# szellmann/icon-ray-tracing

Measured on AMD Instinct MI355X. Metric: Mray/s + ms/frame at 1024², R2B07 ICON grid, 1/2/4/8 MI355X vs host CPU, higher is better.
Workload: dtype f32; 1 GPU; C3: R2B07 (1,310,720 cells) x 90 levels, 1024x1024, framing camera --camera 0 0 1.4e7 0 0 0 0 1 0 -fovy 60, 8 consecutive progressive frames (accumID) per step, woodcockTrackingWithAccel, default TF; records=3932160, width=1024, height=1024, transfer_function=default, sampler=user, accel=sphere, parallelism=single GPU, frames_per_launch=8, slot_table_bytes=0

## Files before the change

icon-ray-tracing_amd/csrc/irt_context.h:

```cpp
#pragma once

#include <hip/hip_runtime.h>

#include <cmath>
#include <vector>

#include "irt_internal.h"
#include "irt_kernels.h"

int irt_hip_failed(const char *call, hipError_t e, const char *file, int line);

#define IRT_HIP(call)                                                           \
  do {                                                                          \
    hipError_t e_ = (call);                                                     \
    if (e_ != hipSuccess) return irt_hip_failed(#call, e_, __FILE__, __LINE__); \
  } while (0)

struct LaunchSlot {
  hipEvent_t ev0 = nullptr, ev1 = nullptr;
  hipEvent_t evDone = nullptr;
  bool pending = false;
  bool marked = false;
  bool timed = false;
  bool block = false;
  hipStream_t stream = nullptr;
  long long launch = 0;
  size_t numWG = 0;
  long long costsOf = -1;
};

struct irt_context {
  int device = 0;
  hipStream_t stream = nullptr;
  irt_volume_info info{};
  uint32_t n = 0;
  int G = 0;
  uint4 *d_binHdr = nullptr;
  float4 *d_fat = nullptr;
  float4 *d_blocks = nullptr;
  irt::SlotTable slot;
  bool slotAlways = false;
  bool slotLazy = false;
  bool slotTried = false;
  bool slotSparse = false;
  double tfSamples = 0.0;
  double *d_tfStat = nullptr;
  size_t binEntries = 0;
  uint32_t numSph = 0;
  uint32_t numSphRec = 0;
  float *d_sphR = nullptr;
  uint32_t *d_sphOff = nullptr;
  uint2 *d_sphRec = nullptr;
  uint32_t *d_sphBits = nullptr;
  uint32_t *h_wgCounts = nullptr, *dh_wgCounts = nullptr;
  size_t wgCap = 0;
  bool lastBlock = false;
  bool wgCountsOn = true;
  bool statsOff = false;
  int countersProbe = 0;
  uint32_t *d_probeCounts = nullptr;
  size_t probeCap = 0;
  float4 *d_samples = nullptr;
  size_t sampleCap = 0;
  float *d_srgb = nullptr;
  float *d_valueRanges = nullptr;
  float *d_maxOp = nullptr;
  ushort4 *d_rects = nullptr;
  unsigned long long *d_updStat = nullptr;
  hipEvent_t evUpd = nullptr;
  bool updPending = false;
  bool gridBuilt = false;
  uint32_t *d_meta = nullptr;
  float *d_gridVR = nullptr;
  float *d_gridMaxOp = nullptr;
  uint32_t *d_gridBits = nullptr;
  int wG = 0;
  uint32_t *d_wOff = nullptr, *d_wRec = nullptr;
  float4 *d_wBox = nullptr, *d_wTrig = nullptr;
  size_t numMCs = 0;
  float4 *d_lut = nullptr;
  int lutCap = 0;
  int lutSize = 0;
  float tfLo = 0.f, tfHi = 1.f, opScale = 1.f;
  bool tfSet = false;
  static constexpr int kSlots = 32;
  static constexpr int kDoneEvery = 8;
  LaunchSlot ring[kSlots];
  long long launches = 0;
  static constexpr size_t kWgCountsMax = size_t(1) << 18;
  size_t wgCountsMax = kWgCountsMax;
  unsigned long long *d_counters = nullptr;
  unsigned long long *d_counterBuckets = nullptr;
  unsigned long long *h_counters = nullptr;
  unsigned long long *dh_counters = nullptr;
  hipStream_t lastStream = nullptr;
  int timingEvery = 8;
  float lastMs = 0.f;
  double timedMs = 0.0;
  long long timedLaunches = 0;
  irt_render_stats stats{};
  unsigned long long h_last[16] = {};
  irt_render_stats total{};
  long long totalLaunches = 0;
  size_t bytes = 0;
  int variant = irt::kDefaultVariant;
  uint32_t *d_schedOrder = nullptr, *d_schedCost = nullptr;
  uint32_t *h_schedCost = nullptr, *h_schedOrder = nullptr;
  uint32_t schedSplit[2] = {0, 0};
  uint32_t lastNumSplit = 0;
  int splitLg = 2;
  float splitFactor = 1.f;
  bool splitFixed = false;
  int schedBuf = 0;
  long long schedSwitch = 0;
  size_t schedCap = 0;
  bool schedOn = false;
  bool schedFixed = false;
  int coopMaxLg = 0;
  int coopRamp = 1;
  int probeExit = 0;
  uint32_t *wgTrace = nullptr;
  bool chainOn = true;
  uint32_t *d_chainFlag = nullptr;
  size_t chainCap = 0;
  uint32_t chainEpoch = 1;
  uint32_t *h_chainFail = nullptr, *dh_chainFail = nullptr;
  long long chainFailLaunches = 0;
  uint32_t chainSpins = 0;
  int chainWithhold = -1;
  float4 *d_frameCams = nullptr;
  float4 *h_frameCams = nullptr;
  size_t frameCamCap = 0;
  bool queueOn = false;
  uint32_t *d_queue = nullptr;
  int numCU = 0;
  int queuePerCU = 0;
  int lastQueueWG = 0;
  int schedPolicy = 2;
  bool schedOrderValid = false;
  bool schedLastApplied = false;
  long long schedApplied = 0;
  long long schedKey[8] = {};
  long long schedSrc = -1;
  long long schedLastCopy = -1000;
  bool building = false;
  size_t expected = 0, received = 0;
  float bottomMin = INFINITY, bottomMax = -INFINITY;
  bool voids = false;
  bool variantFixed = false;
  irt_icon_cell *d_cells = nullptr;
  float4 *d_trig = nullptr;
  irt::VolumeAcc vacc{};
  size_t numRuns = 0;
  irt_icon_cell last{};
  struct Sphere {
    float r;
    uint32_t rec;
    int32_t nl;
  };
  std::vector<Sphere> sph;
  struct TileTable {
    std::vector<int32_t> ids;
    int32_t *dev;
  };
  std::vector<TileTable> tileTables;
};

template <typename T>
int dalloc(irt_context *c, T **p, size_t count) {
  *p = nullptr;
  if (count == 0) count = 1;
  IRT_HIP(hipMalloc((void **)p, count * sizeof(T)));
  c->bytes += count * sizeof(T);
  return IRT_OK;
}

template <typename T>
int upload(irt_context *c, T **p, const T *src, size_t count) {
  int rc = dalloc(c, p, count);
  if (rc) return rc;
  if (count) IRT_HIP(hipMemcpyAsync(*p, src, count * sizeof(T), hipMemcpyHostToDevice, c->stream));
  return IRT_OK;
}

int update_pending(const char *what);
int ensure_grid(irt_context *c);
hipError_t wait_slot(irt_context *c, int i);
int finish_slot(irt_context *c, int i);
int finish_stats(irt_context *c);
int tile_table(irt_context *c, const int32_t *ids, size_t n, int lo, int total, const int32_t **out);
```

icon-ray-tracing_amd/csrc/irt_context.hip:

```cpp

#include <hip/hip_runtime.h>
#include <string.h>

#include <algorithm>
#include <cfloat>
#include <chrono>
#include <cstdio>
#include <thread>
#include <vector>

#include "irt_build.h"
#include "irt_context.h"

using namespace irt;

int irt_hip_failed(const char *call, hipError_t e, const char *file, int line) {
  set_error("%s failed: %s (%s:%d)", call, hipGetErrorString(e), file, line);
  return IRT_E_HIP;
}

constexpr float kSplitFactorHoles = 0.35f;
constexpr double kSparseTfSamples = 8.0;

namespace {

void free_all(irt_context *c) {
  if (c->device >= 0) (void)hipSetDevice(c->device);
  if (c->stream) (void)hipStreamSynchronize(c->stream);
  void *ptrs[] = {c->d_binHdr, c->d_fat, c->slot.slots, c->d_blocks, c->d_sphR, c->d_sphOff, c->d_sphRec,
                  c->d_sphBits, c->d_samples, c->d_maxOp, c->d_gridVR, c->d_gridMaxOp, c->d_gridBits, c->d_wOff, c->d_wRec, c->d_wBox, c->d_wTrig, c->d_schedOrder, c->d_schedCost, c->d_srgb, c->d_valueRanges,
                  c->d_lut, c->d_counters, c->d_counterBuckets, c->d_meta, c->d_queue, c->d_chainFlag,
                  c->d_frameCams, c->d_tfStat, c->d_rects, c->d_updStat, c->d_probeCounts};
  for (void *p : ptrs)
    if (p) (void)hipFree(p);
  if (c->d_cells) (void)hipFree(c->d_cells);
  if (c->d_trig) (void)hipFree(c->d_trig);
  if (c->h_counters) (void)hipHostFree(c->h_counters);
  if (c->h_wgCounts) (void)hipHostFree(c->h_wgCounts);
  if (c->h_schedCost) (void)hipHostFree(c->h_schedCost);
  if (c->h_schedOrder) (void)hipHostFree(c->h_schedOrder);
  if (c->h_frameCams) (void)hipHostFree(c->h_frameCams);
  if (c->h_chainFail) (void)hipHostFree(c->h_chainFail);
  for (LaunchSlot &r : c->ring) {
    if (r.ev0) (void)hipEventDestroy(r.ev0);
    if (r.ev1) (void)hipEventDestroy(r.ev1);
    if (r.evDone) (void)hipEventDestroy(r.evDone);
  }
  if (c->evUpd) (void)hipEventDestroy(c->evUpd);
  for (auto &t : c->tileTables) (void)hipFree(t.dev);
  c->tileTables.clear();
  if (c->stream) (void)hipStreamDestroy(c->stream);
}

}

int update_pending(const char *what) {
  set_error("%s: a value update is pending (irt_update_values_end commits it)", what);
  return IRT_E_INVALID;
}

int ensure_grid(irt_context *c) {
  if (c->gridBuilt) return IRT_OK;
  const size_t gridMCs = (size_t)kGridDim * kGridDim * kGridDim;
  int rc;
  if (!c->d_gridVR && (rc = dalloc(c, &c->d_gridVR, 2 * gridMCs))) return rc;
  if (!c->d_gridMaxOp && (rc = dalloc(c, &c->d_gridMaxOp, gridMCs))) return rc;
  if (!c->d_gridBits && (rc = dalloc(c, &c->d_gridBits, (size_t)kGridBitWords))) return rc;
  IRT_HIP(hipMemsetAsync(c->d_gridBits, 0, kGridBitWords * sizeof(uint32_t), c->stream));
  launch_shell_init(c->d_gridVR, gridMCs, c->stream);
  IRT_HIP(hipMemsetAsync(c->d_gridMaxOp, 0, gridMCs * sizeof(float), c->stream));
  if (c->n) {
    const irt_box3f &vb = c->info.bounds;
    launch_grid_build(c->d_blocks, c->d_meta, c->d_trig, c->n, make_float3(vb.lower.x, vb.lower.y, vb.lower.z),
                      make_float3(vb.upper.x, vb.upper.y, vb.upper.z), c->d_gridVR, c->stream);
  }
  if (c->tfSet) {
    launch_max_opacities(c->d_gridVR, gridMCs, c->d_lut, c->lutSize, c->tfLo, c->tfHi, c->d_gridMaxOp,
                         c->stream);
    launch_grid_bits(c->d_gridMaxOp, c->d_gridBits, c->stream);
  }
  IRT_HIP(hipGetLastError());
  IRT_HIP(hipStreamSynchronize(c->stream));
  c->gridBuilt = true;
  c->info.deviceBytes = c->bytes;
  return IRT_OK;
}

extern "C" {

int irt_create_begin(size_t numCells, int device, irt_context **out) {
  if (!out) {
    set_error("irt_create: null argument");
    return IRT_E_INVALID;
  }
  *out = nullptr;
  if (numCells > 0xFFFFFFF0ull) {
    set_error("too many cells (%zu)", numCells);
    return IRT_E_INVALID;
  }
  int ndev = 0;
  if (hipGetDeviceCount(&ndev) != hipSuccess || ndev <= 0) {
    set_error("irt_create: no HIP device visible (this product has no CPU fallback)");
    return IRT_E_HIP;
  }
  if (device < 0 || device >= ndev) {
    set_error("irt_create: device %d out of range (%d devices)", device, ndev);
    return IRT_E_INVALID;
  }
  irt_context *c = new irt_context();
  c->device = device;
  if (const char *v = getenv("IRT_RENDER_VARIANT")) {
    const int var = atoi(v);
    if (render_variant_available(var)) {
      c->variant = var;
      c->variantFixed = true;
    }
  }
  auto fail = [&](int code) {
    free_all(c);
    delete c;
    return code;
  };
  if (hipSetDevice(device) != hipSuccess || hipStreamCreateWithFlags(&c->stream, hipStreamNonBlocking) != hipSuccess) {
    set_error("irt_create: cannot initialise device %d", device);
    return fail(IRT_E_HIP);
  }
  if (const char *e = getenv("IRT_SPLIT_LG")) c->splitLg = std::min(3, std::max(0, atoi(e)));
  if (const char *e = getenv("IRT_SPLIT_FACTOR")) {
    c->splitFactor = (float)atof(e);
    c->splitFixed = true;
  }
  if (const char *e = getenv("IRT_SCHED")) {
    c->schedOn = atoi(e) != 0;
    c->schedPolicy = atoi(e);
    c->schedFixed = true;
  }
  if (hipMalloc((void **)&c->d_cells, std::max<size_t>(numCells, 1) * sizeof(irt_icon_cell) + 16) != hipSuccess ||
      hipMalloc((void **)&c->d_trig, std::max<size_t>(numCells, 1) * 3 * sizeof(float4)) != hipSuccess) {
    set_error("irt_create: cannot allocate %zu cells in HBM", numCells);
    return fail(IRT_E_HIP);
  }
  volume_acc_init(c->vacc);
  c->expected = numCells;
  c->building = true;
  *out = c;
  return IRT_OK;
}

namespace {
int append_chunk(irt_context *c, const irt_icon_cell *cells, size_t n, float *trigPinned) {
  const size_t base = c->received;
  std::vector<float> trigHeap;
  float *trig = trigPinned;
  if (!trig) {
    trigHeap.resize(n * 12);
    trig = trigHeap.data();
  }
  const int threads = n < 4096 ? 1 : default_threads();
  const size_t slice = (n + threads - 1) / threads;
  struct Part {
    VolumeAcc acc;
    size_t runs = 0, bad = SIZE_MAX;
    std::vector<irt_context::Sphere> sph;
    float bottomMin = INFINITY, bottomMax = -INFINITY;
    bool gap = false;
  };
  std::vector<Part> part(threads);
  auto work = [&](int t) {
    Part &P = part[t];
    volume_acc_init(P.acc);
    const size_t b = (size_t)t * slice, e = std::min(n, b + slice);
    for (size_t i = b; i < e; ++i) {
      const irt_icon_cell &x = cells[i];
      bool ok = x.numLayers >= 0 && x.numLayers <= 31;
      for (int k = 0; ok && k < 3; ++k) ok = std::isfinite(x.lat[k]) && std::isfinite(x.lon[k]);
      for (int j = 0; ok && j <= x.numLayers; ++j) ok = std::isfinite(x.height[j]);
      if (!ok) {
        P.bad = i;
        return;
      }
      float *tr = &trig[12 * i];
      if (i > b && same_corners(x.lat, x.lon, cells[i - 1].lat, cells[i - 1].lon))
        memcpy(tr, tr - 12, 12 * sizeof(float));
      else
        corner_trig(x, tr);
      float lo[3], hi[3];
      cell_bounds(x, tr, lo, hi);
      volume_acc_add(P.acc, x, lo, hi);
      const irt_icon_cell &prev = i ? cells[i - 1] : c->last;
      if (base + i == 0 || !same_corners(x.lat, x.lon, prev.lat, prev.lon)) {
        ++P.runs;
        P.bottomMin = std::min(P.bottomMin, x.height[0]);
        P.bottomMax = std::max(P.bottomMax, x.height[0]);
      } else if (!(x.height[0] == prev.height[prev.numLayers])) {
        P.gap = true;
      }
      if (!(x.height[0] <= x.height[x.numLayers])) P.gap = true;
      if (x.height[0] == x.height[x.numLayers])
        P.sph.push_back({x.height[0], (uint32_t)(base + i), x.numLayers});
    }
  };
  if (threads == 1) {
    work(0);
  } else {
    std::vector<std::thread> ts;
    for (int t = 0; t < threads; ++t) ts.emplace_back(work, t);
    for (auto &t : ts) t.join();
  }
  size_t bad = SIZE_MAX;
  for (const Part &P : part) bad = std::min(bad, P.bad);
  if (bad != SIZE_MAX) {
    const irt_icon_cell &x = cells[bad];
    if (x.numLayers < 0 || x.numLayers > 31)
      set_error("cell %zu: numLayers %d outside [0,31] (MAX_LAYERS 32, ICONGrid.h:57)", base + bad, x.numLayers);
    else
      set_error("cell %zu: non-finite lat/lon/height", base + bad);
    return IRT_E_DATA;
  }
  for (const Part &P : part) {
    volume_acc_merge(c->vacc, P.acc);
    c->numRuns += P.runs;
    c->sph.insert(c->sph.end(), P.sph.begin(), P.sph.end());
    c->bottomMin = std::min(c->bottomMin, P.bottomMin);
    c->bottomMax = std::max(c->bottomMax, P.bottomMax);
    c->voids = c->voids || P.gap;
  }
  IRT_HIP(hipSetDevice(c->device));
  if (trigPinned) {
    IRT_HIP(hipMemcpyAsync(c->d_cells + base, cells, n * sizeof(irt_icon_cell), hipMemcpyHostToDevice, c->stream));
    IRT_HIP(hipMemcpyAsync(c->d_trig + 3 * base, trig, n * 12 * sizeof(float), hipMemcpyHostToDevice, c->stream));
  } else {
    IRT_HIP(hipMemcpy(c->d_cells + base, cells, n * sizeof(irt_icon_cell), hipMemcpyHostToDevice));
    IRT_HIP(hipMemcpy(c->d_trig + 3 * base, trig, n * 12 * sizeof(float), hipMemcpyHostToDevice));
  }
  c->last = cells[n - 1];
  c->received += n;
  return IRT_OK;
}
}

int irt_create_append(irt_context *c, const irt_icon_cell *cells, size_t n) {
  if (!c || !c->building || (n && !cells)) {
    set_error("irt_create_append: no context being created, or null cells");
    return IRT_E_INVALID;
  }
  if (n > c->expected - c->received) {
    set_error("irt_create_append: %zu more cells than irt_create_begin announced", n - (c->expected - c->received));
    return IRT_E_INVALID;
  }
  if (n == 0) return IRT_OK;
  return append_chunk(c, cells, n, nullptr);
}

int build_slot_table(irt_context *c, bool forced) {
  c->slotTried = true;
  const bool indexable = (uint64_t)6 * c->G * c->G * kSubCells * kSubCells < ((uint64_t)1 << 32);
  int slotSubs = 0;
  if (const char *v = getenv("IRT_SLOT_SUBS")) slotSubs = atoi(v);
  const size_t hdrBytes = (size_t)6 * c->G * c->G * kBinHdrWords * 4;
  const size_t sceneBytes = hdrBytes + c->binEntries * kFatStride4 * 16 + (size_t)c->n * kBlk4 * 16;
  size_t fr = 0, tot = 0;
  IRT_HIP(hipMemGetInfo(&fr, &tot));
  size_t cap = fr > ((size_t)16 << 30) ? fr - ((size_t)16 << 30) : 0;
  cap = std::min(cap, tot / 2);
  if (const char *g = getenv("IRT_SLOTS_MAX_GB")) cap = std::min(cap, (size_t)(atof(g) * (double)(1ull << 30)));
  if (!indexable) {
    c->slot = SlotTable{};
    c->slot.skipped = "the cube map has 2^28 cells or more (32-bit slot index)";
  } else if (int rc = build_slots_device(reinterpret_cast<const uint32_t *>(c->d_binHdr), c->d_fat, 6u * c->G * c->G,
                                         cap, slotSubs, sceneBytes, c->stream, c->slot)) {
    return rc;
  }
  c->bytes += c->slot.bytes;
  c->info.deviceBytes = c->bytes;
  if (c->slot.bytes)
    fprintf(stderr, "icon_rt_hip: slot table built on device %d: %.1f GB of HBM, %d sub-cells per slot (IRT_SLOTS=0: none)\n",
            c->device, c->slot.bytes / 1e9, c->slot.subs);
  else if (forced)
    fprintf(stderr, "icon_rt_hip: IRT_SLOTS=1 but no slot table was built: %s\n",
            c->slot.skipped ? c->slot.skipped : "unknown reason");
  return IRT_OK;
}

namespace {
int choose_slot_table(irt_context *c) {
  int rc;
  const char *e = getenv("IRT_SLOTS");
  const bool forced = e && atoi(e) != 0;
  const char *sp = getenv("IRT_SLOTS_SPARSE_TF");
  c->slotLazy = !e && (!sp || atoi(sp) != 0);
  const size_t hdrBytes = (size_t)6 * c->G * c->G * kBinHdrWords * 4;
  if (e ? forced : hdrBytes > kSlotAutoHdrBytes) {
    if ((rc = build_slot_table(c, forced))) return rc;
    c->slotAlways = c->slot.slots != nullptr;
  }
  return IRT_OK;
}

int upload_sphere_table(irt_context *c) {
  int rc;
  std::sort(c->sph.begin(), c->sph.end(), [](const irt_context::Sphere &a, const irt_context::Sphere &b) {
    return a.r < b.r || (a.r == b.r && a.rec < b.rec);
  });
  std::vector<float> R;
  std::vector<uint32_t> off(1, 0u), bits(kSphBitWords, 0u);
  std::vector<uint2> rec;
  for (size_t k = 0; k < c->sph.size(); ++k) {
    if (k == 0 || c->sph[k].r != c->sph[k - 1].r) {
      if (k) off.push_back((uint32_t)rec.size());
      R.push_back(c->sph[k].r);
    }
    rec.push_back(make_uint2(c->sph[k].rec, (uint32_t)c->sph[k].nl));
  }
  if (!c->sph.empty()) off.push_back((uint32_t)rec.size());
  for (float r : R) {
    const uint32_t h = sph_hash(r);
    bits[h >> 5] |= 1u << (h & 31);
  }
  c->numSph = (uint32_t)R.size();
  c->numSphRec = (uint32_t)rec.size();
  if ((rc = upload(c, &c->d_sphR, R.data(), R.size())) || (rc = upload(c, &c->d_sphOff, off.data(), off.size())) ||
      (rc = upload(c, &c->d_sphRec, rec.data(), rec.size())) ||
      (rc = upload(c, &c->d_sphBits, bits.data(), bits.size())))
    return rc;
  IRT_HIP(hipStreamSynchronize(c->stream));
  std::vector<irt_context::Sphere>().swap(c->sph);
  return IRT_OK;
}

int create_launch_state(irt_context *c) {
  int rc;
  if ((rc = dalloc(c, &c->d_counters, 16 * irt_context::kSlots))) return rc;
  if ((rc = dalloc(c, &c->d_counterBuckets, (size_t)kCounterBuckets * 8 * irt_context::kSlots))) return rc;
  IRT_HIP(hipMemsetAsync(c->d_counterBuckets, 0, (size_t)kCounterBuckets * 8 * irt_context::kSlots * sizeof(unsigned long long),
                         c->stream));
  IRT_HIP(hipHostMalloc((void **)&c->h_counters, 16 * irt_context::kSlots * sizeof(unsigned long long)));
  for (LaunchSlot &r : c->ring) {
    IRT_HIP(hipEventCreate(&r.ev0));
    IRT_HIP(hipEventCreate(&r.ev1));
    IRT_HIP(hipEventCreateWithFlags(&r.evDone, hipEventDisableTiming));
  }
  memset(c->h_counters, 0, 16 * irt_context::kSlots * sizeof(unsigned long long));
  if (const char *e = getenv("IRT_COUNTERS")) {
    c->wgCountsOn = strcmp(e, "atomic") != 0;
    c->countersProbe = strcmp(e, "off") == 0 ? 1 : (strcmp(e, "device") == 0 ? 2 : 0);
// ... 482 lines not shown
```

icon-ray-tracing_amd/csrc/irt_debug_hooks.hip:

```cpp

#include <hip/hip_runtime.h>
#include <string.h>

#include <algorithm>

#include "icon_rt_hip_debug.h"
#include "irt_context.h"
#include "irt_device.h"

using namespace irt;

namespace {
__global__ void k_debug_math(const float *a, const float *y, const float *x, int n, float *oa,
                             float *ot) {
  const int i = blockIdx.x * blockDim.x + threadIdx.x;
  if (i >= n) return;
  oa[i] = glibc_asinf(a[i]);
  ot[i] = glibc_atan2f(y[i], x[i]);
}
}

extern "C" int irt_debug_device_math(int device, const float *a, const float *y, const float *x,
                                     int n, float *oa, float *ot) {
  if (n <= 0 || !a || !y || !x || !oa || !ot) {
    set_error("irt_debug_device_math: bad argument");
    return IRT_E_INVALID;
  }
  IRT_HIP(hipSetDevice(device));
  float *d = nullptr;
  IRT_HIP(hipMalloc((void **)&d, 5 * (size_t)n * sizeof(float)));
  hipError_t e = hipSuccess;
  e = e == hipSuccess ? hipMemcpy(d, a, n * sizeof(float), hipMemcpyHostToDevice) : e;
  e = e == hipSuccess ? hipMemcpy(d + n, y, n * sizeof(float), hipMemcpyHostToDevice) : e;
  e = e == hipSuccess ? hipMemcpy(d + 2 * (size_t)n, x, n * sizeof(float), hipMemcpyHostToDevice) : e;
  if (e == hipSuccess) {
    hipLaunchKernelGGL(k_debug_math, dim3((n + 255) / 256), dim3(256), 0, 0, d, d + n,
                       d + 2 * (size_t)n, n, d + 3 * (size_t)n, d + 4 * (size_t)n);
    e = hipGetLastError();
  }
  e = e == hipSuccess ? hipMemcpy(oa, d + 3 * (size_t)n, n * sizeof(float), hipMemcpyDeviceToHost) : e;
  e = e == hipSuccess ? hipMemcpy(ot, d + 4 * (size_t)n, n * sizeof(float), hipMemcpyDeviceToHost) : e;
  (void)hipFree(d);
  if (e != hipSuccess) {
    set_error("irt_debug_device_math: %s", hipGetErrorString(e));
    return IRT_E_HIP;
  }
  return IRT_OK;
}

namespace {
__device__ __forceinline__ void wave_max_out(unsigned long long *out, double v) {
  unsigned long long b = __double_as_longlong(v);
  for (int off = 32; off > 0; off >>= 1) {
    const unsigned long long o = __shfl_xor(b, off, 64);
    b = o > b ? o : b;
  }
  if (__lane_id() == 0) atomicMax(out, b);
}
__global__ void __launch_bounds__(256) k_fast_math_bounds(unsigned long long *out) {
  const uint32_t t = blockIdx.x * blockDim.x + threadIdx.x, stride = gridDim.x * blockDim.x;
  double m0 = 0.0, m1 = 0.0, m2 = 0.0, m3 = 0.0;
  for (uint32_t u = t; u <= 0x3f800000u; u += stride) {
    const float x = __uint_as_float(u);
    const double a = fabs((double)fast_asin(x) - (double)glibc_asinf(x));
    const double b = fabs((double)fast_asin(-x) - (double)glibc_asinf(-x));
    m0 = fmax(m0, fmax(a, b));
    if (!(a == a) || !(b == b)) m0 = __longlong_as_double(0x7ff8000000000000ll);
  }
  for (uint32_t u = t; u <= 0x5d000000u; u += stride) {
    const float q = __uint_as_float(u);
    const double ref = atan((double)q);
    const double a = fabs((double)fast_atan(q) - ref), b = fabs((double)glibc_atanf(q) - ref);
    m1 = (a == a) ? fmax(m1, a) : __longlong_as_double(0x7ff8000000000000ll);
    m2 = (b == b) ? fmax(m2, b) : __longlong_as_double(0x7ff8000000000000ll);
  }
  for (uint32_t u = 0x0d800000u + t; u <= 0x71800000u; u += stride) {
    const float b = __uint_as_float(u);
    m3 = fmax(m3, fabs((double)__builtin_amdgcn_rcpf(b) * (double)b - 1.0));
  }
  wave_max_out(out + 0, m0);
  wave_max_out(out + 1, m1);
  wave_max_out(out + 2, m2);
  wave_max_out(out + 3, m3);
}
}

extern "C" int irt_debug_fast_math_bounds(int device, double *out4) {
  if (!out4) {
    set_error("irt_debug_fast_math_bounds: null argument");
    return IRT_E_INVALID;
  }
  IRT_HIP(hipSetDevice(device));
  unsigned long long *d = nullptr;
  IRT_HIP(hipMalloc((void **)&d, 4 * sizeof(unsigned long long)));
  hipError_t e = hipMemset(d, 0, 4 * sizeof(unsigned long long));
  if (e == hipSuccess) {
    hipLaunchKernelGGL(k_fast_math_bounds, dim3(8192), dim3(256), 0, 0, d);
    e = hipGetLastError();
  }
  if (e == hipSuccess) e = hipMemcpy(out4, d, 4 * sizeof(double), hipMemcpyDeviceToHost);
  (void)hipFree(d);
  if (e != hipSuccess) {
    set_error("irt_debug_fast_math_bounds: %s", hipGetErrorString(e));
    return IRT_E_HIP;
  }
  return IRT_OK;
}

extern "C" void irt_debug_fast_spherical_consts(float *out2) {
  out2[0] = kLatErr;
  out2[1] = kLonErr;
}

namespace {
__global__ void k_debug_wlog(float *out) {
  __shared__ LogfTab t[16];
  if (threadIdx.x < 16) t[threadIdx.x] = kLogfTab[threadIdx.x];
  __syncthreads();
  const uint32_t j = blockIdx.x * blockDim.x + threadIdx.x;
  out[j] = woodcock_log(j, t);
}
}

extern "C" int irt_debug_device_woodcock_log(int device, float *out) {
  if (!out) {
    set_error("irt_debug_device_woodcock_log: null argument");
    return IRT_E_INVALID;
  }
  IRT_HIP(hipSetDevice(device));
  float *d = nullptr;
  const size_t n = (size_t)1 << 24;
  IRT_HIP(hipMalloc((void **)&d, n * sizeof(float)));
  hipLaunchKernelGGL(k_debug_wlog, dim3((unsigned)(n / 256)), dim3(256), 0, 0, d);
  hipError_t e = hipGetLastError();
  if (e == hipSuccess) e = hipMemcpy(out, d, n * sizeof(float), hipMemcpyDeviceToHost);
  (void)hipFree(d);
  if (e != hipSuccess) {
    set_error("irt_debug_device_woodcock_log: %s", hipGetErrorString(e));
    return IRT_E_HIP;
  }
  return IRT_OK;
}

namespace {
__global__ void k_debug_srgb(const float *th, const float *x, uint32_t *out, int n) {
  __shared__ float s_th[256];
  s_th[threadIdx.x] = th[threadIdx.x];
  __syncthreads();
  const int j = blockIdx.x * 256 + threadIdx.x;
  if (j < n) out[j] = srgb_byte(s_th, x[j]);
}
}

extern "C" int irt_debug_device_srgb(int device, const float *x, uint32_t *out, int n) {
  if (!x || !out || n < 0) {
    set_error("irt_debug_device_srgb: bad argument");
    return IRT_E_INVALID;
  }
  IRT_HIP(hipSetDevice(device));
  float th[256];
  srgb_thresholds(th);
  float *d = nullptr;
  const size_t m = 256 + 2 * (size_t)n;
  IRT_HIP(hipMalloc((void **)&d, m * sizeof(float)));
  hipError_t e = hipMemcpy(d, th, sizeof(th), hipMemcpyHostToDevice);
  e = e == hipSuccess ? hipMemcpy(d + 256, x, n * sizeof(float), hipMemcpyHostToDevice) : e;
  if (e == hipSuccess && n > 0) {
    hipLaunchKernelGGL(k_debug_srgb, dim3((n + 255) / 256), dim3(256), 0, 0, d, d + 256,
                       reinterpret_cast<uint32_t *>(d + 256 + n), n);
    e = hipGetLastError();
  }
  e = e == hipSuccess ? hipMemcpy(out, d + 256 + n, n * sizeof(uint32_t), hipMemcpyDeviceToHost) : e;
  (void)hipFree(d);
  if (e != hipSuccess) {
    set_error("irt_debug_device_srgb: %s", hipGetErrorString(e));
    return IRT_E_HIP;
  }
  return IRT_OK;
}

static int debug_locate(irt_context *c, const float *xyz, int n, int *found, float *value, bool wave) {
  if (!c || !xyz || !found || !value || n < 0) {
    set_error("irt_debug_locate: bad argument");
    return IRT_E_INVALID;
  }
  IRT_HIP(hipSetDevice(c->device));
  RenderArgs A;
  memset(&A, 0, sizeof(A));
  A.numCells = c->n;
  A.G = c->G;
  A.binHdr = c->d_binHdr;
  A.fat = c->d_fat;
  A.blocks = c->d_blocks;
  A.slots = c->slot.slots;
  A.slotBins = c->slot.bins;
  A.slotSubs = c->slot.subs;
  for (int k = 0; k < 3; ++k) A.slotEdge[k] = c->slot.edges[k];
  A.numSph = c->numSph;
  A.sphR = c->d_sphR;
  A.sphOff = c->d_sphOff;
  A.sphRec = c->d_sphRec;
  A.sphBits = c->d_sphBits;
  float *d = nullptr;
  IRT_HIP(hipMalloc((void **)&d, (size_t)std::max(n, 1) * 5 * sizeof(float)));
  hipError_t e = hipMemcpy(d, xyz, (size_t)n * 3 * sizeof(float), hipMemcpyHostToDevice);
  int *dFound = reinterpret_cast<int *>(d + 3 * (size_t)n);
  float *dValue = d + 4 * (size_t)n;
  if (e == hipSuccess) {
    launch_debug_locate(A, d, n, dFound, dValue, 0, wave);
    e = hipGetLastError();
  }
  e = e == hipSuccess ? hipMemcpy(found, dFound, (size_t)n * sizeof(int), hipMemcpyDeviceToHost) : e;
  e = e == hipSuccess ? hipMemcpy(value, dValue, (size_t)n * sizeof(float), hipMemcpyDeviceToHost) : e;
  (void)hipFree(d);
  if (e != hipSuccess) {
    set_error("irt_debug_locate: %s", hipGetErrorString(e));
    return IRT_E_HIP;
  }
  return IRT_OK;
}

extern "C" int irt_debug_locate(irt_context *c, const float *xyz, int n, int *found, float *value) {
  return debug_locate(c, xyz, n, found, value, false);
}

extern "C" int irt_debug_locate_wave(irt_context *c, const float *xyz, int n, int *found, float *value) {
  return debug_locate(c, xyz, n, found, value, true);
}

extern "C" int irt_debug_locate_sampler(irt_context *c, int mode, const float *xyz, int n, int *found,
                                        float *value) {
  if (!c || c->building || n < 0 || (n && (!xyz || !found || !value))) {
    set_error("irt_debug_locate_sampler: bad argument");
    return IRT_E_INVALID;
  }
  if (mode != IRT_MODE_CUBQL && mode != IRT_MODE_TRIANGLES) {
    set_error("irt_debug_locate_sampler: sampler mode %d is neither IRT_MODE_CUBQL nor IRT_MODE_TRIANGLES", mode);
    return IRT_E_INVALID;
  }
  if (c->updPending) return update_pending("irt_debug_locate_sampler");
  if (c->wG == 0 && c->n != 0) {
    set_error("irt_debug_locate_sampler: sampler mode %d needs irt_build_wedge_accel first", mode);
    return IRT_E_INVALID;
  }
  if (n == 0) return IRT_OK;
  IRT_HIP(hipSetDevice(c->device));
  RenderArgs A;
  memset(&A, 0, sizeof(A));
  A.numCells = c->n;
  A.sampler = mode;
  A.wG = c->wG;
  A.wOff = c->d_wOff;
  A.wRec = c->d_wRec;
  A.wBox = c->d_wBox;
  A.wTrig = c->d_wTrig;
  A.blocks = c->d_blocks;
  float *d = nullptr;
  IRT_HIP(hipMalloc((void **)&d, (size_t)n * 5 * sizeof(float)));
  hipError_t e = hipMemcpy(d, xyz, (size_t)n * 3 * sizeof(float), hipMemcpyHostToDevice);
  int *dFound = reinterpret_cast<int *>(d + 3 * (size_t)n);
  float *dValue = d + 4 * (size_t)n;
  if (e == hipSuccess) {
    launch_debug_locate_sampler(A, d, n, dFound, dValue, 0);
    e = hipGetLastError();
  }
  e = e == hipSuccess ? hipMemcpy(found, dFound, (size_t)n * sizeof(int), hipMemcpyDeviceToHost) : e;
  e = e == hipSuccess ? hipMemcpy(value, dValue, (size_t)n * sizeof(float), hipMemcpyDeviceToHost) : e;
  (void)hipFree(d);
  if (e != hipSuccess) {
    set_error("irt_debug_locate_sampler: %s", hipGetErrorString(e));
    return IRT_E_HIP;
  }
  return IRT_OK;
}

extern "C" int irt_debug_sched(irt_context *c, int *policy, int *lastApplied, long long *applied) {
  if (!c || !policy || !lastApplied || !applied) {
    set_error("irt_debug_sched: null argument");
    return IRT_E_INVALID;
  }
  *policy = c->schedOn ? c->schedPolicy : 0;
  *lastApplied = c->schedLastApplied ? 1 : 0;
  *applied = c->schedApplied;
  return IRT_OK;
}

extern "C" int irt_debug_counters(irt_context *c, unsigned long long *out16) {
  if (!c || !out16) {
    set_error("irt_debug_counters: null argument");
    return IRT_E_INVALID;
  }
  int rc = finish_stats(c);
  if (rc) return rc;
  memcpy(out16, c->h_last, 16 * sizeof(unsigned long long));
  return IRT_OK;
}

extern "C" int irt_debug_default_variant(void) { return kDefaultVariant; }
extern "C" int irt_debug_slot_use(const irt_context *c, double *tfSamples) {
  if (!c) return -1;
  if (tfSamples) *tfSamples = c->tfSamples;
  return c->slot.slots && (c->slotAlways || c->slotSparse) ? 1 : 0;
}

extern "C" int irt_debug_context_array(const irt_context *c, int which, void *dst, size_t capacity,
                                       size_t *bytes) {
  if (!c || !bytes || c->building) {
    set_error("irt_debug_context_array: null argument or context not built");
    return IRT_E_INVALID;
  }
  const void *src = nullptr;
  size_t n = 0;
  switch (which) {
    case IRT_DEBUG_ARRAY_BIN_HDR: src = c->d_binHdr; n = (size_t)6 * c->G * c->G * kBinHdrWords * 4; break;
    case IRT_DEBUG_ARRAY_FAT: src = c->d_fat; n = c->binEntries * kFatStride4 * 16; break;
    case IRT_DEBUG_ARRAY_BLOCKS: src = c->d_blocks; n = (size_t)c->n * kBlk4 * 16; break;
    case IRT_DEBUG_ARRAY_SPH_R: src = c->d_sphR; n = (size_t)c->numSph * 4; break;
    case IRT_DEBUG_ARRAY_SPH_OFF: src = c->d_sphOff; n = c->numSph ? ((size_t)c->numSph + 1) * 4 : 4; break;
    case IRT_DEBUG_ARRAY_SPH_REC: src = c->d_sphRec; n = (size_t)c->numSphRec * 8; break;
    case IRT_DEBUG_ARRAY_SPH_BITS: src = c->d_sphBits; n = (size_t)kSphBitWords * 4; break;
    case IRT_DEBUG_ARRAY_SLOTS: src = c->slot.slots; n = c->slot.bytes; break;
    case IRT_DEBUG_ARRAY_GRID_BITS: src = c->d_gridBits; n = c->gridBuilt ? (size_t)kGridBitWords * 4 : 0; break;
    default:
      set_error("irt_debug_context_array: unknown array %d", which);
      return IRT_E_INVALID;
  }
  *bytes = n;
  if (dst && capacity >= n && n) {
    IRT_HIP(hipSetDevice(c->device));
    IRT_HIP(hipStreamSynchronize(c->stream));
    IRT_HIP(hipMemcpy(dst, src, n, hipMemcpyDeviceToHost));
  }
  return IRT_OK;
}

extern "C" int irt_debug_get_variant(const irt_context *c) { return c ? c->variant : -1; }

extern "C" int irt_debug_variants(int *out, int capacity) { return render_variants(out, capacity); }

extern "C" int irt_debug_set_queue(irt_context *c, int on) {
  if (!c) {
    set_error("irt_debug_set_queue: null context");
    return IRT_E_INVALID;
  }
  if (on && !render_queue_compiled()) {
    set_error("irt_debug_set_queue: persistent launches are compiled into the A/B library only "
              "(make VARIANTS=all, libicon_rt_hip_all.so)");
    return IRT_E_INVALID;
  }
  c->queueOn = on != 0;
  return IRT_OK;
}

extern "C" int irt_debug_set_wg_trace(irt_context *c, uint32_t *trace) {
  if (!c) {
    set_error("irt_debug_set_wg_trace: null context");
    return IRT_E_INVALID;
  }
  c->wgTrace = trace;
  return IRT_OK;
}

extern "C" long long irt_debug_launch_workgroups(const irt_context *c, int numTiles, int numFrames) {
  if (!c || numTiles < 0 || numFrames < 1) {
    set_error("irt_debug_launch_workgroups: bad argument");
    return -1;
  }
  RenderArgs A;
  memset(&A, 0, sizeof(A));
  const int per = render_wg_per_block(A, c->variant);
  const size_t extra = c->schedOn && numFrames == 1 && per == 4 ? (size_t)kMaxSplit : 0;
  return (long long)((size_t)numTiles * 16 * per * numFrames + extra);
}

extern "C" int irt_debug_sched_split(const irt_context *c, int *numSplit, int *splitLg) {
  if (!c || !numSplit || !splitLg) {
    set_error("irt_debug_sched_split: null argument");
    return IRT_E_INVALID;
  }
  *numSplit = (int)c->lastNumSplit;
  *splitLg = c->splitLg;
  return IRT_OK;
}

extern "C" int irt_debug_set_chain(irt_context *c, int on) {
  if (!c) {
    set_error("irt_debug_set_chain: null context");
    return IRT_E_INVALID;
  }
  c->chainOn = on != 0;
  return IRT_OK;
}

extern "C" int irt_debug_chain_errors(irt_context *c) {
  if (!c) {
    set_error("irt_debug_chain_errors: null context");
    return -1;
  }
  for (long long j = c->launches - irt_context::kSlots; j < c->launches; ++j) {
    if (j < 0) continue;
    const int rc = finish_slot(c, (int)(j % irt_context::kSlots));
    if (rc && rc != IRT_E_CHAIN) return -1;
  }
  return (int)c->chainFailLaunches;
}

extern "C" int irt_debug_set_chain_fault(irt_context *c, uint32_t spins, int withholdFrame) {
  if (!c) {
    set_error("irt_debug_set_chain_fault: null context");
    return IRT_E_INVALID;
  }
  c->chainSpins = spins;
  c->chainWithhold = withholdFrame;
  return IRT_OK;
}

extern "C" int irt_debug_get_queue(const irt_context *c) { return c ? (c->queueOn ? 1 : 0) : -1; }

extern "C" int irt_debug_queue_wgs(const irt_context *c) { return c ? c->lastQueueWG : -1; }

extern "C" int irt_debug_set_variant(irt_context *c, int variant) {
  if (!c || !render_variant_available(variant)) {
    set_error("irt_debug_set_variant: variant %d not compiled", variant);
    return IRT_E_INVALID;
  }
  c->variant = variant;
  return IRT_OK;
}
```

icon-ray-tracing_amd/csrc/irt_internal.h:

```cpp
#pragma once

#include <stddef.h>
#include <stdint.h>

#include <string>
#include <vector>

#include "icon_rt_hip.h"
#include "irt_common.h"

namespace irt {

void set_error(const char *fmt, ...) __attribute__((format(printf, 1, 2)));
void clear_error();


struct HostScene {
  size_t n = 0;
  irt_volume_info info{};
  std::vector<float> hv;
  std::vector<float> trig;
  std::vector<float> planes;
  std::vector<float> rng;
  std::vector<uint32_t> meta;
  std::vector<float> blocks;
  int G = 0;
  std::vector<uint32_t> offsets;
  std::vector<uint32_t> entryRec;
  std::vector<uint32_t> entrySub;
  std::vector<uint32_t> binHdr;
  std::vector<float> fat;
  size_t binEntries = 0;
  std::vector<float> sphR;
  std::vector<uint32_t> sphOff, sphRec, sphBits;
};

int build_bins(HostScene &S, int threads);
int locator_resolution(size_t numRuns);
float record_value_host(const HostScene &s, uint32_t rec, uint32_t path, float r);
int locate_bins_host(const HostScene &s, float px, float py, float pz, float &value,
                     uint32_t *record, uint32_t *tested);

int build_scene(const irt_icon_cell *cells, size_t n, HostScene &out, int threads = 0);


void compute_volume_info(const irt_icon_cell *cells, size_t n, irt_volume_info &info);
struct VolumeAcc {
  float vlo[3], vhi[3], slo[3], shi[3], dlo, dhi;
  size_t n;
};
void corner_trig(const irt_icon_cell &c, float *t12);
void cell_bounds(const irt_icon_cell &c, const float *t12, float lo[3], float hi[3]);
void volume_acc_init(VolumeAcc &a);
void volume_acc_add(VolumeAcc &a, const irt_icon_cell &c, const float blo[3], const float bhi[3]);
void volume_acc_merge(VolumeAcc &a, const VolumeAcc &b);
void volume_acc_finish(const VolumeAcc &a, irt_volume_info &info);

const std::vector<float> &logf_table();

void srgb_thresholds(float th[256]);

int sample_host(const HostScene &s, uint32_t rec, float px, float py, float pz, float &value);
int locate_host(const HostScene &s, float px, float py, float pz, float &value,
                uint32_t *record);

struct WedgeScene {
  int G = 0;
  std::vector<float> trig;
  std::vector<float> box;
  std::vector<uint32_t> offsets;
  std::vector<uint32_t> recs;
};
int build_wedges(const irt_icon_cell *cells, size_t n, WedgeScene &W, int threads = 0);
bool wedge_locate_host(const WedgeScene &W, const irt_icon_cell *cells, float px, float py,
                       float pz, float &value);
bool triangle_locate_host(const WedgeScene &W, const irt_icon_cell *cells, float px, float py,
                          float pz, float &value, uint32_t *record);

int default_threads();

inline bool update_range_ok(size_t first, size_t n, size_t numCells) {
  return first <= numCells && n <= numCells - first;
}

uint32_t sched_order(const uint32_t *cost, int numBlocks, int tilesX, int tileStride, int policy,
                     int splitLg, float splitFactor, int numCU, bool wavewg, size_t cap,
                     uint32_t maxSplit, uint32_t *out);

int synth_open(int rootN, int bisections, int levels, float topHeight, float noise, uint32_t seed,
               float terrainHeight,
               void **gen, size_t *total);
void synth_fill(const void *gen, size_t first, size_t count, irt_icon_cell *out);
void synth_close(void *gen);

}
```

icon-ray-tracing_amd/csrc/irt_kernels.h:

```cpp
#pragma once

#include <hip/hip_runtime.h>
#include <stdint.h>

#include "icon_rt_hip.h"

namespace irt {

struct RenderArgs {
  float3 org, dir00, du, dv;
  int accumID;
  float accumW;
  float3 amb;
  float ambRad;
  float unitDistance;
  int raygen;
  float3 bmin, bmax;
  int3 dims;
  float3 sbLo, sbHi;
  const float *maxOp;
  int accelMode;
  const float *gridMaxOp;
  const uint32_t *gridBits;
  int sampler;
  int wG;
  const uint32_t *wOff, *wRec;
  const float4 *wBox;
  const float4 *wTrig;
  float tfLo, tfHi, opacityScale;
  double invTf;
  double invSb[3];
  const float4 *lut;
  int lutSize;
  uint32_t numCells;
  int G;
  const float *srgbTh;
  int W, H;
  uint32_t *fb;
  float4 *accum;
  int packed;
  int tileBegin, tileStride, numTiles, tilesX;
  const int32_t *tileList;
  unsigned long long *counters;
  unsigned long long *counterBuckets;
  const uint4 *binHdr;
  const float4 *fat;
  const float4 *blocks;
  uint32_t numSph;
  const float *sphR;
  const uint32_t *sphOff;
  const uint2 *sphRec;
  const uint32_t *sphBits;
  uint32_t *wgCounts;
  int numSamples;
  const uint32_t *schedOrder;
  uint32_t *schedCost;
  float4 *sampleBuf;
  int coopMaxLg;
  int coopRamp;
  int probeExit;
  uint32_t *queue;
  uint32_t numPackets;
  int chain;
  const float4 *frameCams;
  uint32_t chainEpoch;
  uint32_t *chainFlag;
  uint32_t *chainFail;
  uint32_t chainSpins;
  int chainWithhold;

  uint32_t *wgTrace;
  const uint32_t *splitList;
  const uint32_t *splitMask;
  uint32_t numSplit;
  const float4 *slots;
  float slotEdge[3];
  int slotBins;
  int slotSubs;
};
constexpr int kQueueLine = 32;
constexpr uint32_t kChainSpinsDefault = 1u << 20;
constexpr int kQueueWords = 9 * kQueueLine;

constexpr int kCnt = 8;

enum : int {
  OPT_WEDGE = 16384,
  OPT_GRID = 8192,
  OPT_STATS = 32768,
  OPT_SERIAL = 65536,
  OPT_SCAN1 = 131072,
  OPT_TIMING = 524288,
  OPT_WAVEWG = 4194304,
  OPT_LEAN = 2097152,
  OPT_QUEUE = 16777216,
  OPT_FASTSPH = 33554432,
  OPT_SPLIT = 8,
  OPT_DPPSCAN = 32,
  OPT_DMATAB = 67108864,
  OPT_NOMISS = 262144,
  OPT_VOIDLOC = 1073741824,
  OPT_NOVOIDRUN = 2,
  OPT_NOHOLESKIP = 4,
  OPT_SLOT = 128,
};
constexpr int OPT_MONO = 4096;
constexpr int kDefaultVariant = 73405728;
constexpr int kNoMissBit = OPT_NOMISS;
constexpr uint32_t kMaxSplit = 4096;
constexpr int kVoidLocBit = OPT_VOIDLOC;
constexpr int kSamplerVariant = ((kDefaultVariant & ~OPT_MONO) & ~(0xF00 | OPT_WAVEWG | OPT_LEAN)) | OPT_WEDGE;
inline int scene_variant(bool holes) { return holes ? kDefaultVariant | kVoidLocBit : kDefaultVariant | kNoMissBit; }
bool render_variant_available(int variant);
int render_variants(int *out, int cap);
int render_wg_per_block(const RenderArgs &A, int variant);
bool render_queue_ok(const RenderArgs &A, int variant);
bool render_queue_compiled();
bool render_split_ok(const RenderArgs &A, int variant);
int render_queue_wgs(const RenderArgs &A, int variant, int numCU, int numBlocks);
void launch_render(const RenderArgs &A, int numBlocks, hipStream_t s, int variant);
void prewarm_render(int variant, hipStream_t s);
void launch_debug_locate(const RenderArgs &A, const float *xyz, int n, int *found, float *value,
                         hipStream_t s, bool wave);
void launch_debug_locate_sampler(const RenderArgs &A, const float *xyz, int n, int *found, float *value,
                                 hipStream_t s);
void launch_shell_init(float *valueRanges, size_t numMCs, hipStream_t s);
void launch_shell_build(const irt_icon_cell *cells, size_t n, int3 dims, float3 lo, float3 hi,
                        float *valueRanges, ushort4 *rects, hipStream_t s);
void launch_value_scatter(const float *d_values, size_t first, size_t n, float4 *blocks, hipStream_t s);
void launch_shell_rebuild(const float4 *blocks, const uint32_t *meta, const ushort4 *rects, size_t n,
                          int3 dims, float *valueRanges, unsigned long long *stat, hipStream_t s);
void launch_grid_build(const float4 *blocks, const uint32_t *meta, const float4 *trig, size_t n,
                       float3 lo, float3 hi, float *valueRanges, hipStream_t s);
void launch_grid_bits(const float *maxOp, uint32_t *bits, hipStream_t s);
void launch_accept_stat(const float *valueRanges, const float *maxOp, size_t numMCs, const float4 *lut, int size,
                        float lo, float hi, double *out, hipStream_t s);
void launch_max_opacities(const float *valueRanges, size_t numMCs, const float4 *lut, int size,
                          float lo, float hi, float *maxOp, hipStream_t s);
void launch_clear(uint32_t *fb, float4 *accum, size_t n, hipStream_t s);
constexpr int kCounterBuckets = 64;
void launch_stats_out(const unsigned long long *cur, unsigned long long *host,
                      unsigned long long *next, unsigned long long *buckets, hipStream_t s);
void launch_copy_u32(const uint32_t *src, uint32_t *dst, size_t n, hipStream_t s);
struct DeviceScene {
  float4 *blocks = nullptr;
  uint32_t *meta = nullptr;
  uint4 *binHdr = nullptr;
  float4 *fat = nullptr;
  size_t entries = 0, binEntries = 0, bigCells = 0, bytes = 0;
};
int build_scene_device(const irt_icon_cell *d_cells, const float4 *d_trig, size_t n, size_t numRuns,
                       int G, hipStream_t s, DeviceScene &out);
struct SlotTable {
  float4 *slots = nullptr;
  int bins = 0;
  int subs = 0;
  float edges[3] = {0.f, 0.f, 0.f};
  size_t bytes = 0;
  const char *skipped = nullptr;
};
constexpr size_t kSlotAutoHdrBytes = (size_t)256 << 20;
int build_slots_device(const uint32_t *hdr, const float4 *fat, uint32_t numCells, size_t maxBytes, int subs,
                       size_t autoBytes, hipStream_t s, SlotTable &out);
void launch_unpack(const uint32_t *gathered, int numRanks, int maxTiles, int W, int H,
                   uint32_t *fb, hipStream_t s, const int32_t *table = nullptr);

}
```

icon-ray-tracing_amd/csrc/irt_launch.hip:

```cpp

#include <hip/hip_runtime.h>
#include <string.h>

#include <algorithm>
#include <initializer_list>

#include "irt_context.h"

using namespace irt;


int tile_table(irt_context *c, const int32_t *ids, size_t n, int lo, int total, const int32_t **out) {
  for (size_t k = 0; k < n; ++k)
    if (ids[k] < lo || ids[k] >= total) {
      set_error("tile id %d at %zu outside [%d, %d)", ids[k], k, lo, total);
      return IRT_E_INVALID;
    }
  for (auto &t : c->tileTables)
    if (t.ids.size() == n && std::equal(t.ids.begin(), t.ids.end(), ids)) {
      *out = t.dev;
      return IRT_OK;
    }
  if (c->tileTables.size() >= 64) {
    IRT_HIP(hipDeviceSynchronize());
// ... 184 lines not shown
    const LaunchSlot &r = c->ring[i];
    if (r.costsOf > c->schedSrc && r.costsOf >= c->schedSwitch && r.costsOf > best &&
        (!r.pending || (r.marked && hipEventQuery(r.evDone) == hipSuccess))) {
      best = r.costsOf;
      bestSlot = i;
    }
  }
  if (bestSlot < 0) return IRT_OK;
  const int nb = c->schedOrderValid ? 1 - c->schedBuf : c->schedBuf;
  const size_t stride = sched_stride(c->schedCap);
  uint32_t *h = c->h_schedOrder + (size_t)nb * stride;
  c->schedSplit[nb] = sched_order(c->h_schedCost + (size_t)bestSlot * 4 * c->schedCap, numBlocks, (W + 63) / 64,
                                  tileStride, c->schedPolicy, c->splitLg, c->splitFactor, c->numCU, wavewg,
                                  c->schedCap, kMaxSplit, h);
  uint32_t *dh = nullptr;
  IRT_HIP(hipHostGetDevicePointer((void **)&dh, h, 0));
  launch_copy_u32(dh, c->d_schedOrder + (size_t)nb * stride, stride, s);
  IRT_HIP(hipGetLastError());
  c->schedBuf = nb;
  c->schedSwitch = c->launches;
  c->schedOrderValid = true;
  c->schedSrc = best;
  return IRT_OK;
}


struct RenderRequest {
  int W, H;
  int packed;
  int tileBegin, tileStride;
  const int32_t *tileList;
  int listCount;
  int numFrames;
  const irt_launch_params *seq;
};

struct Launch {
  RenderArgs A;
  hipStream_t s;
  int slot;
  int numTiles;
  bool queued;
  int queueWG;
  bool copyCosts;
  size_t numWG;
};

bool whole_kernel(const irt_context *c) { return c->probeExit == 0 || c->probeExit >= 16; }

bool chain_capable(const irt_context *c, bool queue) {
  return c->chainOn && !queue && whole_kernel(c) && (c->variant & OPT_SERIAL) == 0;
}

bool stats_variant(const irt_context *c) { return (c->variant & (OPT_STATS | OPT_TIMING)) != 0; }

int validate(const irt_context *c, const irt_launch_params *lp, const RenderRequest &r, const uint32_t *fb,
             const irt_vec4f *accum) {
  if (!c || !lp || r.W <= 0 || r.H <= 0 || !fb || !accum || r.tileStride <= 0 || r.tileBegin < 0 ||
      r.numFrames < 1 || r.numFrames > 65535 || r.listCount < 0 || (r.listCount > 0 && !r.tileList)) {
    set_error("irt_render: bad argument");
    return IRT_E_INVALID;
  }
  if (c->updPending) return update_pending("irt_render");
  if (!c->tfSet) {
    set_error("irt_render: no transfer function set (irt_set_transfunc)");
    return IRT_E_INVALID;
  }
  if (lp->raygen != IRT_RAYGEN_WITH_ACCEL && lp->raygen != IRT_RAYGEN_AE) {
    set_error("irt_render: unknown raygen %d", lp->raygen);
    return IRT_E_INVALID;
  }
  if (lp->accelMode != IRT_ACCEL_SPHERE && lp->accelMode != IRT_ACCEL_GRID) {
    set_error("irt_render: unknown accelMode %d", lp->accelMode);
    return IRT_E_INVALID;
  }
  if (lp->mode != IRT_MODE_USER_GEOM && lp->mode != IRT_MODE_CUBQL &&
      lp->mode != IRT_MODE_TRIANGLES) {
    set_error("irt_render: unknown sampler mode %d", lp->mode);
    return IRT_E_INVALID;
  }
  if (lp->mode != IRT_MODE_USER_GEOM && c->wG == 0 && c->n != 0) {
    set_error("irt_render: sampler mode %d needs irt_build_wedge_accel first (buildCuBQLAccel / "
              "buildTriangleAccel, hostCode.cu:557-649, 440-484)", lp->mode);
    return IRT_E_INVALID;
  }
  return IRT_OK;
}

int resolve_tiles(irt_context *c, const RenderRequest &r, Launch &L) {
  RenderArgs &A = L.A;
  A.tilesX = (r.W + 63) / 64;
  const int total = A.tilesX * ((r.H + 63) / 64);
  L.numTiles = r.tileBegin < total ? (total - r.tileBegin + r.tileStride - 1) / r.tileStride : 0;
  if (r.tileList) {
    L.numTiles = r.listCount;
    if (r.listCount > 0) {
      int rc = tile_table(c, r.tileList, (size_t)r.listCount, 0, total, &A.tileList);
      if (rc) return rc;
    }
  }
  A.W = r.W;
  A.H = r.H;
  A.packed = r.packed;
  A.tileBegin = r.tileBegin;
  A.tileStride = r.tileStride;
  A.numTiles = L.numTiles;
  return IRT_OK;
}

void fill_args(const irt_context *c, const irt_launch_params *lp, uint32_t *fb, irt_vec4f *accum, Launch &L) {
  RenderArgs &A = L.A;
  A.org = make_float3(lp->org.x, lp->org.y, lp->org.z);
  A.dir00 = make_float3(lp->dir_00.x, lp->dir_00.y, lp->dir_00.z);
  A.du = make_float3(lp->dir_du.x, lp->dir_du.y, lp->dir_du.z);
  A.dv = make_float3(lp->dir_dv.x, lp->dir_dv.y, lp->dir_dv.z);
  A.accumID = lp->accumID;
  A.accumW = 1.f / (float)(lp->accumID + 1);
  A.amb = make_float3(lp->ambientColor.x, lp->ambientColor.y, lp->ambientColor.z);
  A.ambRad = lp->ambientRadiance;
  A.unitDistance = lp->unitDistance;
  A.raygen = lp->raygen;
  const irt_volume_info &I = c->info;
  A.bmin = make_float3(I.bounds.lower.x, I.bounds.lower.y, I.bounds.lower.z);
  A.bmax = make_float3(I.bounds.upper.x, I.bounds.upper.y, I.bounds.upper.z);
  A.dims = make_int3(I.shellDims[0], I.shellDims[1], I.shellDims[2]);
  A.sbLo = make_float3(I.sphericalBounds.lower.x, I.sphericalBounds.lower.y, I.sphericalBounds.lower.z);
  A.sbHi = make_float3(I.sphericalBounds.upper.x, I.sphericalBounds.upper.y, I.sphericalBounds.upper.z);
  A.maxOp = c->d_maxOp;
  A.accelMode = lp->accelMode;
  A.gridMaxOp = c->d_gridMaxOp;
  A.gridBits = c->d_gridBits;
  A.sampler = lp->mode;
  A.wG = c->wG;
  A.wOff = c->d_wOff;
  A.wRec = c->d_wRec;
  A.wBox = c->d_wBox;
  A.wTrig = c->d_wTrig;
  A.tfLo = c->tfLo;
  A.tfHi = c->tfHi;
  {
    const float tfSize = c->tfHi - c->tfLo;
    A.invTf = 1.0 / (double)tfSize;
    const float sz[3] = {I.sphericalBounds.upper.x - I.sphericalBounds.lower.x,
                         I.sphericalBounds.upper.y - I.sphericalBounds.lower.y,
                         I.sphericalBounds.upper.z - I.sphericalBounds.lower.z};
    for (int k = 0; k < 3; ++k) A.invSb[k] = 1.0 / (double)sz[k];
  }
  A.opacityScale = c->opScale;
  A.lut = c->d_lut;
  A.lutSize = c->lutSize;
  A.coopMaxLg = c->coopMaxLg;
  A.coopRamp = c->coopRamp;
  A.probeExit = c->probeExit;
  A.wgTrace = c->wgTrace;
  A.numCells = c->n;
  A.G = c->G;
  A.srgbTh = c->d_srgb;
  A.fb = fb;
  A.accum = (float4 *)accum;
  A.counters = c->d_counters + 16 * L.slot;
  A.binHdr = c->d_binHdr;
  A.fat = c->d_fat;
  A.blocks = c->d_blocks;
  A.slots = c->slotAlways || c->slotSparse ? c->slot.slots : nullptr;
  A.slotBins = c->slot.bins;
  A.slotSubs = c->slot.subs;
  for (int k = 0; k < 3; ++k) A.slotEdge[k] = c->slot.edges[k];
  A.numSph = c->numSph;
  A.sphR = c->d_sphR;
  A.sphOff = c->d_sphOff;
  A.sphRec = c->d_sphRec;
  A.sphBits = c->d_sphBits;
}

int claim_slot(irt_context *c, Launch &L) {
  for (int i = 0; i < kSlots; ++i)
    if (c->ring[i].pending && c->h_chainFail[i]) {
      int rc = finish_slot(c, i);
      if (rc) return rc;
    }
  if (c->ring[L.slot].pending) {
    int rc = finish_slot(c, L.slot);
    if (rc) return rc;
  }
  hipStream_t s = L.s;
  if (c->launches > 0 && s != c->lastStream) {
    const int prev = (int)((c->launches - 1) % kSlots);
    if (c->ring[prev].pending) {
      const hipEvent_t e = done_event(c, prev);
      if (e) IRT_HIP(hipStreamWaitEvent(s, e, 0));
    }
  }
  c->lastStream = s;
  return IRT_OK;
}

void decide_queue(irt_context *c, int numFrames, Launch &L) {
  RenderArgs &A = L.A;
  L.queued = c->queueOn && L.numTiles > 0 && whole_kernel(c) && render_queue_ok(A, c->variant);
  L.queueWG = 0;
  if (!L.queued) return;
  A.queue = c->d_queue + (size_t)kQueueWords * L.slot;
  A.numPackets = (uint32_t)L.numTiles * 64u * (uint32_t)numFrames;
  L.queueWG = c->queuePerCU > 0 ? std::min(c->queuePerCU * c->numCU, L.numTiles * 16 * numFrames)
                                : render_queue_wgs(A, c->variant, c->numCU, L.numTiles * 16 * numFrames);
  c->lastQueueWG = L.queueWG;
}

int decide_sched(irt_context *c, const irt_launch_params *lp, const RenderRequest &r, Launch &L) {
  RenderArgs &A = L.A;
  const int numBlocks = L.numTiles * 16;
  L.copyCosts = false;
  if (!(c->schedOn && r.numFrames == 1 && numBlocks > 0 && !A.tileList && !L.queued)) return IRT_OK;
  int rc = sched_prepare(c, numBlocks, r.W, r.H, r.packed, r.tileBegin, r.tileStride, L.numTiles, lp,
                         render_split_ok(A, c->variant), L.s);
  if (rc) return rc;
  const uint32_t *ob = c->d_schedOrder + (size_t)c->schedBuf * sched_stride(c->schedCap);
  A.schedOrder = c->schedOrderValid ? ob : nullptr;
  if (c->schedOrderValid && c->schedSplit[c->schedBuf] && render_split_ok(A, c->variant) && whole_kernel(c)) {
    A.splitList = ob + c->schedCap;
    A.splitMask = ob + c->schedCap + kMaxSplit;
    A.numSplit = c->schedSplit[c->schedBuf];
  }
  L.copyCosts = c->launches - c->schedLastCopy >= 8;
  if (L.copyCosts) {
    uint32_t *dh = nullptr;
    IRT_HIP(hipHostGetDevicePointer((void **)&dh, c->h_schedCost + (size_t)L.slot * 4 * c->schedCap, 0));
    A.schedCost = dh;
  } else {
    A.schedCost = c->d_schedCost;
  }
  return IRT_OK;
}

void count_workgroups(const irt_context *c, const RenderRequest &r, Launch &L) {
  RenderArgs &A = L.A;
  const uint64_t outPixels = r.packed ? (uint64_t)L.numTiles * 4096u : (uint64_t)r.W * (uint64_t)r.H;
  A.chain = r.numFrames > 1 && chain_capable(c, L.queued) && outPixels * 16u <= 0x7FFFFFFFull ? 1 : 0;
  A.numSamples = r.numFrames;
  L.numWG = L.queued ? (size_t)L.queueWG
                     : (size_t)L.numTiles * 16 * (size_t)render_wg_per_block(A, c->variant) * (size_t)r.numFrames +
                           (size_t)A.numSplit;
}

int choose_counters(irt_context *c, Launch &L) {
  RenderArgs &A = L.A;
  const bool useWG = c->wgCountsOn && L.numWG <= c->wgCountsMax;
  if (useWG && L.numWG > c->wgCap) {
    bool failed = false;
    int rc = grow(c, Retire::Slots, L.s, &c->wgCap, L.numWG,
                  {{(void **)&c->h_wgCounts, [](size_t n) { return n * kSlots * kCnt * sizeof(uint32_t); }, true}},
                  &failed);
    if (rc) return rc;
    if (!failed && hipHostGetDevicePointer((void **)&c->dh_wgCounts, c->h_wgCounts, 0) != hipSuccess) {
      (void)hipGetLastError();
      (void)hipHostFree(c->h_wgCounts);
      c->h_wgCounts = nullptr;
      c->wgCap = 0;
      failed = true;
    }
    if (failed) {
      c->dh_wgCounts = nullptr;
      c->wgCountsOn = false;
    }
  }
  A.wgCounts = useWG && c->wgCountsOn ? c->dh_wgCounts + (size_t)L.slot * c->wgCap * kCnt : nullptr;
  if (c->countersProbe == 1 || c->statsOff) {
    A.wgCounts = nullptr;
    if (!stats_variant(c)) A.counters = nullptr;
  } else if (c->countersProbe == 2) {
    if (L.numWG > c->probeCap) {
      int rc = grow(c, Retire::Stream, L.s, &c->probeCap, L.numWG,
                    {{(void **)&c->d_probeCounts, [](size_t n) { return n * kCnt * sizeof(uint32_t); }, false}}, nullptr);
      if (rc) return rc;
    }
    A.wgCounts = c->d_probeCounts;
  }
  return IRT_OK;
}

int setup_chain(irt_context *c, int numFrames, Launch &L) {
  RenderArgs &A = L.A;
  if (!A.chain) return IRT_OK;
  const size_t words = (size_t)L.numTiles * 16 * 4;
  if (words > c->chainCap || c->chainEpoch > 0xF0000000u - (uint32_t)numFrames) {
    if (words > c->chainCap) {
      int rc = grow(c, Retire::SlotsThenStream, L.s, &c->chainCap, words,
                    {{(void **)&c->d_chainFlag, [](size_t n) { return n * sizeof(uint32_t); }, false}}, nullptr);
      if (rc) return rc;
    }
    IRT_HIP(hipMemsetAsync(c->d_chainFlag, 0, c->chainCap * sizeof(uint32_t), L.s));
    c->chainEpoch = 1;
  }
  A.chainFlag = c->d_chainFlag;
  c->h_chainFail[L.slot] = 0;
  A.chainFail = c->dh_chainFail + L.slot;
  A.chainSpins = c->chainSpins ? c->chainSpins : kChainSpinsDefault;
  A.chainWithhold = c->chainWithhold;
  A.chainEpoch = c->chainEpoch;
  c->chainEpoch += (uint32_t)numFrames;
  return IRT_OK;
}

int stage_sequence(irt_context *c, const RenderRequest &r, Launch &L) {
  RenderArgs &A = L.A;
  if (!r.seq) return IRT_OK;
  if (!A.chain) {
    set_error("irt_render_sequence: needs chained frames (a cooperative variant, IRT_CHAIN on)");
    return IRT_E_INVALID;
  }
  const int numFrames = r.numFrames;
  if ((size_t)numFrames > c->frameCamCap) {
    int rc = grow(c, Retire::SlotsThenStream, L.s, &c->frameCamCap, (size_t)numFrames,
                  {{(void **)&c->d_frameCams, [](size_t n) { return n * 4 * sizeof(float4); }, false},
                   {(void **)&c->h_frameCams, [](size_t n) { return kSlots * n * 4 * sizeof(float4); }, true}},
                  nullptr);
    if (rc) return rc;
  }
  float4 *h = c->h_frameCams + (size_t)L.slot * c->frameCamCap * 4;
  for (int k = 0; k < numFrames; ++k) {
    const irt_launch_params &q = r.seq[k];
    h[4 * k + 0] = make_float4(q.org.x, q.org.y, q.org.z, __builtin_bit_cast(float, q.accumID));
    h[4 * k + 1] = make_float4(q.dir_00.x, q.dir_00.y, q.dir_00.z, 0.f);
    h[4 * k + 2] = make_float4(q.dir_du.x, q.dir_du.y, q.dir_du.z, 0.f);
    h[4 * k + 3] = make_float4(q.dir_dv.x, q.dir_dv.y, q.dir_dv.z, 0.f);
  }
  IRT_HIP(hipMemcpyAsync(c->d_frameCams, h, (size_t)numFrames * 4 * sizeof(float4), hipMemcpyHostToDevice, L.s));
  A.frameCams = c->d_frameCams;
  return IRT_OK;
}

int ensure_samples(irt_context *c, int numFrames, Launch &L) {
  if (numFrames > 1 && !L.A.chain) {
    const size_t need = (size_t)L.numTiles * 4096 * (size_t)numFrames;
    if (need > c->sampleCap) {
      int rc = grow(c, Retire::Stream, L.s, &c->sampleCap, need,
                    {{(void **)&c->d_samples, [](size_t n) { return n * sizeof(float4); }, false}}, nullptr);
      if (rc) return rc;
    }
  }
  L.A.sampleBuf = c->d_samples;
  return IRT_OK;
}

int launch_and_commit(irt_context *c, Launch &L) {
  RenderArgs &A = L.A;
  hipStream_t s = L.s;
  LaunchSlot &r = c->ring[L.slot];
  c->schedLastApplied = A.schedOrder != nullptr;
  c->lastNumSplit = A.numSplit;
  c->schedApplied += c->schedLastApplied ? 1 : 0;
  A.counterBuckets = A.counters && !A.wgCounts ? c->d_counterBuckets + (size_t)L.slot * kCounterBuckets * 8 : nullptr;
  const bool block = A.counters && (!A.wgCounts || stats_variant(c));
  if (block && !c->lastBlock) IRT_HIP(hipMemsetAsync(A.counters, 0, 16 * sizeof(unsigned long long), s));
  r.timed = c->launches % c->timingEvery == 0;
  if (r.timed) IRT_HIP(hipEventRecord(r.ev0, s));
  if (L.numTiles > 0) {
    launch_render(A, L.queued ? L.queueWG : L.numTiles * 16, s, c->variant);
  }
  IRT_HIP(hipGetLastError());
  if (r.timed) IRT_HIP(hipEventRecord(r.ev1, s));
  if (block) {
    launch_stats_out(A.counters, c->dh_counters + 16 * L.slot,
                     c->d_counters + 16 * ((c->launches + 1) % kSlots), A.counterBuckets, s);
    IRT_HIP(hipGetLastError());
  }
  r.block = block;
  c->lastBlock = block;
  r.numWG = (A.wgCounts && c->countersProbe == 0 && !c->statsOff && L.numTiles > 0) ? L.numWG : 0;
  r.costsOf = -1;
  if (L.copyCosts) {
    r.costsOf = c->launches;
    c->schedLastCopy = c->launches;
  }
  r.stream = s;
  r.launch = c->launches;
  r.marked = c->launches % irt_context::kDoneEvery == irt_context::kDoneEvery - 1 || L.copyCosts;
  if (r.marked) IRT_HIP(hipEventRecord(r.evDone, s));
  r.pending = true;
  ++c->launches;
  return IRT_OK;
}

int render_impl(irt_context *c, const irt_launch_params *lp, const RenderRequest &r, uint32_t *fb,
                irt_vec4f *accum, int *numTilesOut, void *stream) {
  int rc = validate(c, lp, r, fb, accum);
  if (rc) return rc;
  IRT_HIP(hipSetDevice(c->device));
  if (lp->accelMode == IRT_ACCEL_GRID && (rc = ensure_grid(c))) return rc;
  Launch L;
  memset(&L.A, 0, sizeof(L.A));
  L.s = (hipStream_t)stream;
  L.slot = (int)(c->launches % kSlots);
  if ((rc = resolve_tiles(c, r, L))) return rc;
  if (numTilesOut) *numTilesOut = L.numTiles;
  fill_args(c, lp, fb, accum, L);
  if ((rc = claim_slot(c, L))) return rc;
  decide_queue(c, r.numFrames, L);
  if ((rc = decide_sched(c, lp, r, L))) return rc;
  count_workgroups(c, r, L);
  if ((rc = choose_counters(c, L)) || (rc = setup_chain(c, r.numFrames, L)) || (rc = stage_sequence(c, r, L)) ||
      (rc = ensure_samples(c, r.numFrames, L)))
    return rc;
  return launch_and_commit(c, L);
}

RenderRequest whole_frame(int W, int H, int numFrames) { return {W, H, 0, 0, 1, nullptr, 0, numFrames, nullptr}; }
RenderRequest strided_tiles(int W, int H, int tileBegin, int tileStride, int numFrames) {
  return {W, H, 1, tileBegin, tileStride, nullptr, 0, numFrames, nullptr};
}
RenderRequest listed_tiles(int W, int H, const int32_t *tiles, int numTiles, int numFrames) {
  static const int32_t none = 0;
  return {W, H, 1, 0, 1, numTiles > 0 ? tiles : &none, numTiles, numFrames, nullptr};
}

int render_sequence(irt_context *c, const irt_launch_params *lps, int numFrames, int W, int H,
                    const int32_t *tiles, int numTiles, uint32_t *fb, irt_vec4f *accum, void *stream) {
  if (!c || !lps || numFrames < 1 || numTiles < 0 || (numTiles > 0 && !tiles)) {
    set_error("irt_render_sequence: bad argument");
    return IRT_E_INVALID;
  }
  const size_t fixed = offsetof(irt_launch_params, ambientColor);
  for (int k = 1; k < numFrames; ++k)
    if (memcmp((const char *)&lps[k] + fixed, (const char *)&lps[0] + fixed, sizeof(irt_launch_params) - fixed)) {
      set_error("irt_render_sequence: frame %d differs from frame 0 in more than the camera and accumID", k);
      return IRT_E_INVALID;
    }
  const bool chainable = chain_capable(c, c->queueOn);
  RenderRequest r = tiles ? listed_tiles(W, H, tiles, numTiles, 1) : whole_frame(W, H, 1);
  if (numFrames == 1 || !chainable) {
    for (int k = 0; k < numFrames; ++k) {
      int rc = render_impl(c, &lps[k], r, fb, accum, nullptr, stream);
      if (rc) return rc;
    }
    return IRT_OK;
  }
  r.numFrames = numFrames;
  r.seq = lps;
  return render_impl(c, &lps[0], r, fb, accum, nullptr, stream);
}

}


extern "C" {

int irt_clear_frame(irt_context *c, uint32_t *fb, irt_vec4f *accum, size_t n, void *stream) {
  if (!c) {
    set_error("irt_clear_frame: null context");
    return IRT_E_INVALID;
  }
  IRT_HIP(hipSetDevice(c->device));
  launch_clear(fb, (float4 *)accum, n, (hipStream_t)stream);
  IRT_HIP(hipGetLastError());
  return IRT_OK;
}

int irt_render(irt_context *c, const irt_launch_params *lp, int W, int H, uint32_t *fb,
               irt_vec4f *accum, void *stream) {
  return render_impl(c, lp, whole_frame(W, H, 1), fb, accum, nullptr, stream);
}

int irt_render_tiles(irt_context *c, const irt_launch_params *lp, int W, int H, int tileBegin,
                     int tileStride, uint32_t *fb, irt_vec4f *accum, int *numTiles,
                     void *stream) {
  return render_impl(c, lp, strided_tiles(W, H, tileBegin, tileStride, 1), fb, accum, numTiles, stream);
}

int irt_render_accumulate(irt_context *c, const irt_launch_params *lp, int W, int H,
                          int numFrames, uint32_t *fb, irt_vec4f *accum, void *stream) {
  return render_impl(c, lp, whole_frame(W, H, numFrames), fb, accum, nullptr, stream);
}

int irt_render_sequence(irt_context *c, const irt_launch_params *lps, int numFrames, int W, int H,
                        uint32_t *fb, irt_vec4f *accum, void *stream) {
  return render_sequence(c, lps, numFrames, W, H, nullptr, 0, fb, accum, stream);
}

int irt_render_tile_list_sequence(irt_context *c, const irt_launch_params *lps, int numFrames, int W, int H,
                                  const int32_t *tiles, int numTiles, uint32_t *fb, irt_vec4f *accum,
                                  void *stream) {
  if (numTiles < 0 || (numTiles > 0 && !tiles)) {
    set_error("irt_render_tile_list_sequence: bad tile list");
    return IRT_E_INVALID;
  }
  static const int32_t none = 0;
  return render_sequence(c, lps, numFrames, W, H, numTiles > 0 ? tiles : &none, numTiles, fb, accum, stream);
}

int irt_render_tiles_accumulate(irt_context *c, const irt_launch_params *lp, int W, int H,
                                int tileBegin, int tileStride, int numFrames, uint32_t *fb,
                                irt_vec4f *accum, int *numTiles, void *stream) {
  return render_impl(c, lp, strided_tiles(W, H, tileBegin, tileStride, numFrames), fb, accum, numTiles, stream);
}

int irt_unpack_tiles(irt_context *c, const uint32_t *g, int numRanks, int maxTiles, int W, int H,
                     uint32_t *fb, void *stream) {
  if (!c || !g || !fb || numRanks <= 0 || maxTiles < 0 || W <= 0 || H <= 0) {
    set_error("irt_unpack_tiles: bad argument");
    return IRT_E_INVALID;
  }
  IRT_HIP(hipSetDevice(c->device));
  if (maxTiles > 0) launch_unpack(g, numRanks, maxTiles, W, H, fb, (hipStream_t)stream);
  IRT_HIP(hipGetLastError());
  return IRT_OK;
}

int irt_render_tile_list(irt_context *c, const irt_launch_params *lp, int W, int H,
                         const int32_t *tiles, int numTiles, int numFrames, uint32_t *fb,
                         irt_vec4f *accum, void *stream) {
  if (numTiles < 0 || (numTiles > 0 && !tiles)) {
    set_error("irt_render_tile_list: bad tile list");
    return IRT_E_INVALID;
  }
  return render_impl(c, lp, listed_tiles(W, H, tiles, numTiles, numFrames), fb, accum, nullptr, stream);
}

int irt_unpack_tile_table(irt_context *c, const uint32_t *g, int numRanks, int maxTiles,
                          const int32_t *table, int W, int H, uint32_t *fb, void *stream) {
  if (!c || !g || !fb || !table || numRanks <= 0 || maxTiles < 0 || W <= 0 || H <= 0) {
    set_error("irt_unpack_tile_table: bad argument");
    return IRT_E_INVALID;
  }
  IRT_HIP(hipSetDevice(c->device));
  if (maxTiles == 0) return IRT_OK;
  const int total = irt_num_tiles(W, H);
  const int32_t *d = nullptr;
  int rc = tile_table(c, table, (size_t)numRanks * (size_t)maxTiles, -1, total, &d);
  if (rc) return rc;
  launch_unpack(g, numRanks, maxTiles, W, H, fb, (hipStream_t)stream, d);
  IRT_HIP(hipGetLastError());
  return IRT_OK;
}

int irt_get_render_stats(const irt_context *cc, irt_render_stats *st) {
  irt_context *c = const_cast<irt_context *>(cc);
  if (!c || !st) {
    set_error("irt_get_render_stats: null argument");
    return IRT_E_INVALID;
  }
  int rc = finish_stats(c);
  if (rc) return rc;
  *st = c->stats;
  return IRT_OK;
}

int irt_get_render_stats_total(const irt_context *cc, irt_render_stats *total, long long *launches) {
  irt_context *c = const_cast<irt_context *>(cc);
  if (!c || !total) {
    set_error("irt_get_render_stats_total: null argument");
    return IRT_E_INVALID;
  }
  int rc = finish_stats(c);
  if (rc) return rc;
  *total = c->total;
  total->kernelMs = c->timedLaunches
                        ? (float)(c->timedMs / (double)c->timedLaunches * (double)c->totalLaunches)
                        : 0.f;
  if (launches) *launches = c->totalLaunches;
  return IRT_OK;
}

int irt_set_timing_interval(irt_context *c, int every) {
  if (!c || every < 1) {
    set_error("irt_set_timing_interval: null context or interval < 1");
    return IRT_E_INVALID;
  }
  c->timingEvery = every;
  return IRT_OK;
}

int irt_set_statistics(irt_context *c, int on) {
  if (!c) {
    set_error("irt_set_statistics: null context");
    return IRT_E_INVALID;
  }
  c->statsOff = on == 0;
  return IRT_OK;
}

int irt_reset_render_stats_total(irt_context *c) {
  if (!c) {
    set_error("irt_reset_render_stats_total: null context");
    return IRT_E_INVALID;
  }
  int rc = finish_stats(c);
  if (rc) return rc;
  c->total = irt_render_stats{};
  c->totalLaunches = 0;
  c->timedMs = 0.0;
  c->timedLaunches = 0;
  return IRT_OK;
}

}
```

icon-ray-tracing_amd/csrc/irt_raygen.h:

```cpp
#pragma once

#include "irt_tracer.h"

namespace irt {

struct Pixel {
  int x, y;
  size_t outIdx;
  bool active;
};
__device__ __forceinline__ Pixel pixel_of(const RenderArgs &A, uint32_t blkU, int tid) {
  const int blk = (int)__builtin_amdgcn_readfirstlane(blkU);
  const int k = blk >> 4, sub = blk & 15;
  const int wave = tid >> 6, lane = tid & 63;
  const int lx = ((sub & 3) << 4) | ((wave & 1) << 3) | (lane & 7);
  const int ly = ((sub >> 2) << 4) | ((wave >> 1) << 3) | (lane >> 3);
  const int tileId = !A.tileList ? A.tileBegin + k * A.tileStride : (k < A.numTiles ? (int)scalar_word(A.tileList, (uint32_t)k) : 0);
  const int tx = tileId % A.tilesX, ty = tileId / A.tilesX;
  Pixel p;
  p.x = tx * 64 + lx;
  p.y = ty * 64 + ly;
  p.active = k < A.numTiles && p.x < A.W && p.y < A.H;
  p.outIdx = A.packed ? (size_t)k * 4096 + ly * 64 + lx : (size_t)p.x + (size_t)A.W * p.y;
  return p;
}

__device__ __forceinline__ void gen_ray(const RenderArgs &A, int accumID, int x, int y, uint32_t &st,
                                        float &dx, float &dy, float &dz, int frame = 0) {
  st = lcg_seed((uint32_t)accumID * (uint32_t)A.W * (uint32_t)A.H + (uint32_t)x, (uint32_t)y);
  st = lcg_next(st);
  const float jv = lcg_float(st);
  st = lcg_next(st);
  const float ju = lcg_float(st);
  const float su = (float)x + .5f, sv = (float)y + .5f;
  const float a = su + ju, b = sv + jv;
  float3 d00 = A.dir00, du = A.du, dv = A.dv;
  if (A.frameCams) {
    const float4 w1 = cam_word(A, frame, 1), w2 = cam_word(A, frame, 2), w3 = cam_word(A, frame, 3);
    d00 = make_float3(w1.x, w1.y, w1.z);
    du = make_float3(w2.x, w2.y, w2.z);
    dv = make_float3(w3.x, w3.y, w3.z);
  }
  dx = (d00.x + a * du.x) + b * dv.x;
  dy = (d00.y + a * du.y) + b * dv.y;
  dz = (d00.z + a * du.z) + b * dv.z;
  const float len = sqrtf(dot3(dx, dy, dz, dx, dy, dz));
  if (recip_ok(len)) {
    const double r = recip_d(len);
    dx = div_recip(dx, r);
    dy = div_recip(dy, r);
    dz = div_recip(dz, r);
  } else {
    dx = dx / len;
    dy = dy / len;
    dz = dz / len;
  }
  if (fabsf(dx) < 1e-5f) dx = 1e-5f;
  if (fabsf(dy) < 1e-5f) dy = 1e-5f;
  if (fabsf(dz) < 1e-5f) dz = 1e-5f;
}

template <bool nt = false>
__device__ __forceinline__ void write_pixel(const RenderArgs &A, size_t outIdx, float cr, float cg,
                                            float cb, float alpha, const float *s_th, float4 old) {
  const float w = A.accumW;
  float4 nv;
  nv.x = w * cr + (1.f - w) * old.x;
  nv.y = w * cg + (1.f - w) * old.y;
  nv.z = w * cb + (1.f - w) * old.z;
  nv.w = w * alpha + (1.f - w) * old.w;
  const uint32_t rgba = srgb_byte(s_th, nv.x) + (srgb_byte(s_th, nv.y) << 8) +
                        (srgb_byte(s_th, nv.z) << 16) + (make_8bit(nv.w) << 24);
  if constexpr (nt) {
    typedef float f4v __attribute__((ext_vector_type(4)));
    const f4v t = {nv.x, nv.y, nv.z, nv.w};
    __builtin_nontemporal_store(t, reinterpret_cast<f4v *>(&A.accum[outIdx]));
    __builtin_nontemporal_store(rgba, &A.fb[outIdx]);
  } else {
    A.accum[outIdx] = nv;
    A.fb[outIdx] = rgba;
  }
}
__device__ __forceinline__ void write_pixel(const RenderArgs &A, size_t outIdx, float cr, float cg,
                                            float cb, float alpha, const float *s_th) {
  write_pixel(A, outIdx, cr, cg, cb, alpha, s_th, A.accum[outIdx]);
}

typedef uint32_t u32x4 __attribute__((ext_vector_type(4)));
__device__ __forceinline__ uint32_t out_pixels(const RenderArgs &A) {
  return A.packed ? (uint32_t)A.numTiles * 4096u : (uint32_t)A.W * (uint32_t)A.H;
}
__device__ __forceinline__ void chain_wait(const RenderArgs &A, uint32_t blk, int pwave, int frame) {
  uint32_t *f = A.chainFlag + (size_t)blk * 4u + (uint32_t)pwave;
  const uint32_t want = A.chainEpoch + (uint32_t)frame;
  for (uint32_t spins = 0;; ++spins) {
    const uint32_t v = __builtin_amdgcn_readfirstlane(__hip_atomic_load(f, __ATOMIC_RELAXED, __HIP_MEMORY_SCOPE_AGENT));
    if (v == want) break;
    if (spins >= A.chainSpins) {
      if (__lane_id() == (unsigned)(__ffsll((long long)__ballot(1)) - 1))
        __hip_atomic_store(A.chainFail, 1u, __ATOMIC_RELAXED, __HIP_MEMORY_SCOPE_SYSTEM);
      break;
    }
    __builtin_amdgcn_s_sleep(2);
  }
  __builtin_amdgcn_fence(__ATOMIC_ACQUIRE, "wavefront");
}
__device__ __forceinline__ float4 chain_load_accum(const RenderArgs &A, size_t outIdx) {
  const __amdgpu_buffer_rsrc_t r = __builtin_amdgcn_make_buffer_rsrc((void *)A.accum, 0, (int)(out_pixels(A) * 16u), 0x00020000);
  return __builtin_bit_cast(float4, __builtin_amdgcn_raw_buffer_load_b128(r, (int)(outIdx * 16u), 0, 16));
}
__device__ __forceinline__ bool chain_skips_fb(const RenderArgs &A, int frame) {
  return A.chain && !A.frameCams && frame < A.numSamples - 1;
}
__device__ __forceinline__ bool chain_last_fb(const RenderArgs &A, int frame) {
  return A.chain && !A.frameCams && frame == A.numSamples - 1;
}
__device__ __forceinline__ void chain_replay_fb(const RenderArgs &KA, uint32_t blk, int ptid, int frame,
                                                const float *s_th) {
  const RenderArgs *vp = &KA;
  asm volatile("" : "+v"(vp));
  const RenderArgs &A = *vp;
  const Pixel p = pixel_of(A, blk, ptid);
  if (!p.active) return;
  int g = frame;
  asm volatile("" : "+v"(g));
  bool seen = false;
#pragma nounroll
  while (--g >= 0 && !seen) {
    uint32_t st;
    float dx, dy, dz, t0, t1;
    gen_ray(A, A.accumID + g, p.x, p.y, st, dx, dy, dz);
    const Ray ray = {A.org.x, A.org.y, A.org.z, 0.f, dx, dy, dz, 1e10f};
    seen = box_test(ray, A, t0, t1);
  }
  if (!seen) return;
  const float *ap = reinterpret_cast<const float *>(A.accum + p.outIdx);
  float a[4];
#pragma unroll
  for (int k = 0; k < 4; ++k) a[k] = __hip_atomic_load(ap + k, __ATOMIC_RELAXED, __HIP_MEMORY_SCOPE_AGENT);
  const uint32_t rgba = srgb_byte(s_th, a[0]) + (srgb_byte(s_th, a[1]) << 8) + (srgb_byte(s_th, a[2]) << 16) +
                        (make_8bit(a[3]) << 24);
  __builtin_nontemporal_store(rgba, &A.fb[p.outIdx]);
}
__device__ __forceinline__ void write_pixel_chain(const RenderArgs &A, size_t outIdx, float cr, float cg, float cb,
                                                  float alpha, float w, const float *s_th, float4 old, bool publish,
                                                  bool toFb) {
  float4 nv;
  nv.x = w * cr + (1.f - w) * old.x;
  nv.y = w * cg + (1.f - w) * old.y;
  nv.z = w * cb + (1.f - w) * old.z;
  nv.w = w * alpha + (1.f - w) * old.w;
  if (!toFb) {
    if (publish) {
      const __amdgpu_buffer_rsrc_t ra =
          __builtin_amdgcn_make_buffer_rsrc((void *)A.accum, 0, (int)(out_pixels(A) * 16u), 0x00020000);
      __builtin_amdgcn_raw_buffer_store_b128(__builtin_bit_cast(u32x4, nv), ra, (int)(outIdx * 16u), 0, 16);
    } else {
      typedef float f4v __attribute__((ext_vector_type(4)));
      const f4v t = {nv.x, nv.y, nv.z, nv.w};
      __builtin_nontemporal_store(t, reinterpret_cast<f4v *>(&A.accum[outIdx]));
    }
    return;
  }
  const uint32_t rgba = srgb_byte(s_th, nv.x) + (srgb_byte(s_th, nv.y) << 8) +
                        (srgb_byte(s_th, nv.z) << 16) + (make_8bit(nv.w) << 24);
#ifdef IRT_PROBE_BUILD
  if (publish && A.probeExit == 17) {
    A.accum[outIdx] = nv;
    A.fb[outIdx] = rgba;
    return;
  }
#endif
  if (publish) {
    const uint32_t n = out_pixels(A);
    const __amdgpu_buffer_rsrc_t ra = __builtin_amdgcn_make_buffer_rsrc((void *)A.accum, 0, (int)(n * 16u), 0x00020000);
    const __amdgpu_buffer_rsrc_t rf = __builtin_amdgcn_make_buffer_rsrc((void *)A.fb, 0, (int)(n * 4u), 0x00020000);
    __builtin_amdgcn_raw_buffer_store_b128(__builtin_bit_cast(u32x4, nv), ra, (int)(outIdx * 16u), 0, 16);
    __builtin_amdgcn_raw_buffer_store_b32(rgba, rf, (int)(outIdx * 4u), 0, 16);
  } else {
    typedef float f4v __attribute__((ext_vector_type(4)));
    const f4v t = {nv.x, nv.y, nv.z, nv.w};
    __builtin_nontemporal_store(t, reinterpret_cast<f4v *>(&A.accum[outIdx]));
    __builtin_nontemporal_store(rgba, &A.fb[outIdx]);
  }
}

__device__ __forceinline__ void flush_counters(const RenderArgs &A, const uint32_t *s_cnt, int lane) {
  if (A.wgCounts) {
    const size_t wg = (size_t)blockIdx.y * gridDim.x + blockIdx.x;
    if (lane < kCnt) A.wgCounts[wg * kCnt + lane] = s_cnt[lane];
  } else if (lane < 5 && s_cnt[lane]) {
    const size_t wg = (size_t)blockIdx.y * gridDim.x + blockIdx.x;
    unsigned long long *dst = A.counterBuckets ? A.counterBuckets + (wg % kCounterBuckets) * 8 : A.counters;
    atomicAdd(&dst[lane], (unsigned long long)s_cnt[lane]);
  }
}

constexpr float kNoSample = -1.f;

template <int OPT>
__device__ __forceinline__ void render_grid(const RenderArgs &A, Tracer<OPT> &T, const Ray &ray,
                                            float rtmin, float rtmax, uint32_t &st, float &cr,
                                            float &cg, float &cb, float &alpha) {
  const int D = kGridDim;
  const float ox = ray.ox + rtmin * ray.dx, oy = ray.oy + rtmin * ray.dy, oz = ray.oz + rtmin * ray.dz;
  const float tmax = rtmax - rtmin;
  const float rx = 1.f / ray.dx, ry = 1.f / ray.dy, rz = 1.f / ray.dz;
  const float lx = (A.bmin.x - ox) * rx, ly = (A.bmin.y - oy) * ry, lz = (A.bmin.z - oz) * rz;
  const float hx = (A.bmax.x - ox) * rx, hy = (A.bmax.y - oy) * ry, hz = (A.bmax.z - oz) * rz;
  float nx = fminf(lx, hx), ny = fminf(ly, hy), nz = fminf(lz, hz);
  const float fx = fmaxf(lx, hx), fy = fmaxf(ly, hy), fz = fmaxf(lz, hz);
  if (ray.dx == 0.f) nx = IRT_FLT_MAX;
  if (ray.dy == 0.f) ny = IRT_FLT_MAX;
  if (ray.dz == 0.f) nz = IRT_FLT_MAX;
  int cx = project_on_grid(ox, A.bmin.x, A.bmax.x, D);
  int cy = project_on_grid(oy, A.bmin.y, A.bmax.y, D);
  int cz = project_on_grid(oz, A.bmin.z, A.bmax.z, D);
  const float dx = fmaxf(0.f, (fx - nx) / (float)D), dy = fmaxf(0.f, (fy - ny) / (float)D),
              dz = fmaxf(0.f, (fz - nz) / (float)D);
  const int sx = ray.dx > 0.f ? 1 : -1, sy = ray.dy > 0.f ? 1 : -1, sz = ray.dz > 0.f ? 1 : -1;
  const int ex = ray.dx > 0.f ? D : -1, ey = ray.dy > 0.f ? D : -1, ez = ray.dz > 0.f ? D : -1;
  float tnx = ray.dx > 0.f ? nx + (float)(cx + 1) * dx : nx + (float)(D - cx) * dx;
  float tny = ray.dy > 0.f ? ny + (float)(cy + 1) * dy : ny + (float)(D - cy) * dy;
  float tnz = ray.dz > 0.f ? nz + (float)(cz + 1) * dz : nz + (float)(D - cz) * dz;
  float tc0 = 0.f;
  for (int iter = 0; iter < 4 * D + 16; ++iter) {
    const float tmn = fminf(fminf(tnx, tny), tnz);
    const float tc1 = dda3_min_quirk(tmn, tmax);
    const float w0 = rtmin + tc0, w1 = rtmin + tc1;
    constexpr int NB = kGridDim / kGridBlock;
    const bool inGrid = (unsigned)cx < (unsigned)D && (unsigned)cy < (unsigned)D && (unsigned)cz < (unsigned)D;
    const uint32_t gb = inGrid ? ((uint32_t)(cz / kGridBlock) * NB + (uint32_t)(cy / kGridBlock)) * NB +
                                     (uint32_t)(cx / kGridBlock)
                               : 0u;
    if (!inGrid || ((T.s_gbits[gb >> 5] >> (gb & 31)) & 1u)) {
      const float maj = A.gridMaxOp[(size_t)cz * D * D + (size_t)cy * D + cx];
      float4 s = make_float4(0.f, 0.f, 0.f, 0.f);
      const float tw = T.woodcock(ray.dx, ray.dy, ray.dz, w0, w1, st, maj, s, !(w0 == w1));
      if (tw > w0 && tw < w1) {
        cr = s.x * A.amb.x * A.ambRad;
        cg = s.y * A.amb.y * A.ambRad;
        cb = s.z * A.amb.z * A.ambRad;
        alpha = s.w > 0.f ? 1.f : 0.f;
        return;
      }
    }
    if (tnx == tmn) {
      tnx += dx;
      cx += sx;
      if (cx == ex) return;
    }
    if (tny == tmn) {
      tny += dy;
      cy += sy;
      if (cy == ey) return;
    }
    if (tnz == tmn) {
      tnz += dz;
      cz += sz;
      if (cz == ez) return;
    }
    tc0 = tc1;
  }
}

template <int OPT>
__device__ __forceinline__ void render_pixel(const RenderArgs &A, Tracer<OPT> &T, const Pixel &px,
                                             const float *s_th, int4 *s_dda, float4 *s_entry,
                                             int tid, int accumID, float4 *sampleOut) {
  uint32_t st;
  float dx, dy, dz;
  gen_ray(A, accumID, px.x, px.y, st, dx, dy, dz);
  const Ray ray = {A.org.x, A.org.y, A.org.z, 0.f, dx, dy, dz, 1e10f};
  float t0, t1;
  if (!box_test(ray, A, t0, t1)) {
    if (sampleOut) *sampleOut = make_float4(0.f, 0.f, 0.f, kNoSample);
    return;
  }
  T.count(1);
  float cr = 0.f, cg = 0.f, cb = 0.f, alpha = 0.f;
  const bool ae = A.raygen == 1;
  float rlo0 = t0, rhi0 = t1, rlo1 = __builtin_inff(), rhi1 = -__builtin_inff();
  int numRanges = 1;
  if (!ae) {
    float st1 = 0.f, st2 = 0.f, st3 = 0.f, st4 = 0.f;
    const bool s1 = intersect_sphere(ray, A.sbHi.x, st1, st4);
    const bool s2 = intersect_sphere(ray, A.sbLo.x, st2, st3);
    numRanges = 0;
    if ((s1 || s2) && !(st4 < t0)) {
      numRanges = 2;
      if (s1 && !s2) {
        rlo0 = st1; rhi0 = st4;
      } else if (t0 < st2) {
        rlo0 = st1; rhi0 = st2;
        rlo1 = st3; rhi1 = st4;
      } else {
        rlo0 = st3; rhi0 = st4;
      }
    }
  }
  if constexpr ((OPT & OPT_GRID) != 0) {
    if (!ae) {
      render_grid(A, T, ray, t0, t1, st, cr, cg, cb, alpha);
      numRanges = 0;
    }
  }
  const float sceneEPS = A.sbLo.x * 1e-6f;
  for (int i = 0; i < numRanges; ++i) {
    const float lower = i ? rlo1 : rlo0, upper = i ? rhi1 : rhi0;
    if (upper <= lower) break;
    const bool lastRange = ae || i == 1 || rhi1 <= rlo1;
    int cx = 0, cy = 0, cz = 0;
    if (!ae) {
      const float e1 = lower + sceneEPS;
      float r1, la1, lo1;
      to_spherical(ray.ox + ray.dx * e1, ray.oy + ray.dy * e1, ray.oz + ray.dz * e1, r1, la1, lo1);
      cx = project_axis(r1, A.sbLo.x, A.sbHi.x, A.dims.x);
      cy = project_axis(la1, A.sbLo.y, A.sbHi.y, A.dims.y);
      cz = project_axis(lo1, A.sbLo.z, A.sbHi.z, A.dims.z);
      if (!lastRange) lds_st16(&s_entry[tid], make_float4(r1, la1, lo1, 0.f));
    }
    const float tnx = upper, tny = 0.f, tnz = 0.f;
    float t = lower;
    for (int iter = 0; iter < (1 << 22); ++iter) {
      float tt1 = IRT_FLT_MAX;
      if (ae) {
        tt1 = upper;
      } else {
        if (tnx < tt1 && tnx >= t) tt1 = tnx;
        if (tny < tt1 && tny >= t) tt1 = tny;
        if (tnz < tt1 && tnz >= t) tt1 = tnz;
      }
      const bool zeroLen = tt1 == t;
      if (zeroLen && lastRange) break;
      if constexpr ((OPT & OPT_STATS) != 0) T.cnt.deg += zeroLen ? 1u : 0u;
      float maj = 1.f;
      if (!ae) {
        const uint32_t leaf = (uint32_t)wrap_coord(cz, A.dims.z) * (uint32_t)A.dims.x * (uint32_t)A.dims.y +
                              (uint32_t)wrap_coord(cy, A.dims.y) * (uint32_t)A.dims.x +
                              (uint32_t)wrap_coord(cx, A.dims.x);
        maj = A.maxOp[leaf];
      }
      bool fast = false;
      if (zeroLen) {
        const float q = maj / A.unitDistance;
        const uint32_t nx = lcg_next(st);
        if (!(maj > 0.f)) {
          fast = true;
        } else if (q > 0.f && q <= 1e30f && (nx & 0x00FFFFFFu) != 0u) {
          st = nx;
          fast = true;
        }
      }
      if (!fast) {
        float4 s = make_float4(0.f, 0.f, 0.f, 0.f);
        const bool counted = !zeroLen;
        const float tw = T.woodcock(ray.dx, ray.dy, ray.dz, t, tt1, st, maj, s, counted);
        if (!zeroLen && (ae || (tw > t && tw < tt1))) {
          cr = s.x * A.amb.x * A.ambRad;
          cg = s.y * A.amb.y * A.ambRad;
          cb = s.z * A.amb.z * A.ambRad;
          alpha = s.w > 0.f ? 1.f : 0.f;
          i = 2;
          break;
        }
      }
      if (lastRange) break;
      int4 dd;
      if (iter == 0) {
        const float e2 = upper - sceneEPS;
        float r2, la2, lo2;
        to_spherical(ray.ox + ray.dx * e2, ray.oy + ray.dy * e2, ray.oz + ray.dz * e2, r2, la2, lo2);
        const float4 en = lds_ld16(&s_entry[tid]);
        const float r1 = en.x, la1 = en.y, lo1 = en.z;
        const int sx = r1 < r2 ? 1 : -1, sy = la1 < la2 ? 1 : -1, sz = lo1 < lo2 ? 1 : -1;
        dd.x = (sx > 0 ? 1 : 0) | (sy > 0 ? 2 : 0) | (sz > 0 ? 4 : 0);
        dd.y = (int)((uint32_t)project_axis(r2, A.sbLo.x, A.sbHi.x, A.dims.x) + (uint32_t)sx);
        dd.z = (int)((uint32_t)project_axis(la2, A.sbLo.y, A.sbHi.y, A.dims.y) + (uint32_t)sy);
        dd.w = (int)((uint32_t)project_axis(lo2, A.sbLo.z, A.sbHi.z, A.dims.z) + (uint32_t)sz);
        s_dda[tid] = dd;
      } else {
        dd = s_dda[tid];
      }
      const float t_closest = fminf(fminf(tnx, tny), tnz);
      if (tnx == t_closest) {
        cx += (dd.x & 1) ? 1 : -1;
        if (cx == dd.y) break;
      }
      if (tny == t_closest) {
        cy += (dd.x & 2) ? 1 : -1;
        if (cy == dd.z) break;
      }
      if (tnz == t_closest) {
        cz += (dd.x & 4) ? 1 : -1;
        if (cz == dd.w) break;
      }
      t = t_closest;
    }
  }
  if (sampleOut)
    *sampleOut = make_float4(cr, cg, cb, alpha);
  else
    write_pixel(A, px.outIdx, cr, cg, cb, alpha, s_th);
}

__device__ __forceinline__ bool spherical_fast(const RenderArgs &A, float x, float y, float z, float &r, float &la,
                                               float &lo, int &cy, int &cz) {
  r = sqrtf(dot3(x, y, z, x, y, z));
  la = fast_asin(z / r);
  const bool okLon = fast_atan2(y, x, lo);
  const bool okY = cell_certified(la, kLatErr, A.sbLo.y, A.invSb[1], A.dims.y, cy);
  const bool okZ = cell_certified(lo, kLonErr, A.sbLo.z, A.invSb[2], A.dims.z, cz);
  return okY && okZ && okLon;
}


template <int OPT>
__device__ __forceinline__ void render_pixel_coop(const RenderArgs &A, Tracer<OPT> &T, const Pixel &px,
                                                  const float *s_th, int4 *s_dda, float4 *s_entry,
                                                  float4 *s_acc, CoopWave &W, ScanWave *SW, const uint2 *jmp,
                                                  int tid, int accumID, uint32_t blk, int pwave, int frame,
                                                  int partSel = -1) {
  constexpr bool kRecompute = ((OPT >> 8) & 15) >= 5;
  const int ptid = pwave * 64 + (tid & 63);
  const int wbase = __builtin_amdgcn_readfirstlane(tid) & ~63;
  auto tid_late = [&]() { return kRecompute ? (opaque_u(wbase) | (int)__lane_id()) : tid; };
  auto ptid_late = [&]() {
    if constexpr (!kRecompute) return ptid;
    int lane = (int)__lane_id();
    asm volatile("" : "+v"(lane));
    if (partSel >= 0) {
      const int ps = opaque_u(partSel), pn = 64 >> (ps & 255);
      lane = ((ps >> 8) * pn) | (lane & (pn - 1));
    }
    return (opaque_u(pwave) << 6) | lane;
  };
  const bool toSample = A.numSamples > 1 && !A.chain;
  const bool chainLate = A.chain && frame > 0;
  uint32_t chainSeen = 0u;
  if (chainLate)
    chainSeen = __hip_atomic_load(A.chainFlag + (size_t)blk * 4u + (uint32_t)pwave, __ATOMIC_RELAXED,
                                  __HIP_MEMORY_SCOPE_AGENT);
  float4 *const slot0 = kRecompute || !toSample
                            ? nullptr
                            : A.sampleBuf + (size_t)frame * A.numTiles * 4096u + (size_t)blk * 256u + (size_t)ptid;
  auto sample_slot = [&]() {
    if constexpr (!kRecompute) return slot0;
    return A.sampleBuf + (size_t)opaque_u(frame) * opaque_u(A.numTiles) * 4096u + (size_t)opaque_u((int)blk) * 256u +
           (size_t)ptid_late();
  };
  enum : int { kRange, kLeaf, kWait, kDone, kGrid, kGridNext };
  constexpr bool kFastSph = (OPT & OPT_FASTSPH) != 0;
  constexpr bool grid = (OPT & OPT_GRID) != 0;
  const bool ae = A.raygen == 1;
  uint32_t st = 0;
  float dx = 1.f, dy = 1.f, dz = 1.f;
  float rlo0 = 0.f, rhi0 = 0.f, rlo1 = __builtin_inff(), rhi1 = -__builtin_inff();
  int numRanges = 0, phase = kDone;
  bool inBox = false;
  float t0box = 0.f, t1box = 0.f;
  if (px.active) {
    gen_ray(A, accumID, px.x, px.y, st, dx, dy, dz, frame);
    const float3 O = cam_org(A, frame);
    const Ray ray = {O.x, O.y, O.z, 0.f, dx, dy, dz, 1e10f};
    float t0, t1;
    const bool boxHit = box_test(ray, A, t0, t1);
#ifdef IRT_PROBE_BUILD
    if (A.probeExit == 30) {
#pragma nounroll
      for (int k = 0; k < 50; ++k) asm volatile("v_nop\n v_nop\n v_nop\n v_nop" ::: "memory");
    }
#endif
    if (A.probeExit == 3) {
      if (boxHit && t0 == -1.2345f) A.fb[0] = 0u;
      return;
    }
    if (boxHit) {
      inBox = true;
      phase = kRange;
      t0box = t0;
      t1box = t1;
      if (!toSample && !chainLate && (OPT & OPT_LEAN) == 0)
        __builtin_amdgcn_global_load_lds((const void *)(A.accum + px.outIdx),
                                         (__attribute__((address_space(3))) void *)(s_acc + (tid & ~63)),
                                         16, 0, kRecompute ? 2 : 0);
      rlo0 = t0;
      rhi0 = t1;
      numRanges = 1;
      if (!ae) {
        float st1 = 0.f, st2 = 0.f, st3 = 0.f, st4 = 0.f;
        bool s1, s2;
        intersect_spheres(ray, A.sbHi.x, A.sbLo.x, s1, st1, st4, s2, st2, st3);
        numRanges = 0;
        if ((s1 || s2) && !(st4 < t0)) {
          numRanges = 2;
          if (s1 && !s2) {
            rlo0 = st1; rhi0 = st4;
          } else if (t0 < st2) {
// ... 388 lines not shown
```

icon-ray-tracing_amd/csrc/irt_render.hip:

```cpp

#include "irt_raygen.h"

namespace irt {

constexpr int kQueueXcds = 8;
struct QueueCursor {
  int cur;
  uint32_t dead;
};
__device__ __forceinline__ uint32_t queue_take(uint32_t *Q, uint32_t numBlocksAll, QueueCursor &c) {
  while (c.dead != (1u << kQueueXcds) - 1u) {
    const uint32_t x = (uint32_t)c.cur;
    const uint32_t limit = numBlocksAll > x ? 4u * ((numBlocksAll - x + kQueueXcds - 1) / kQueueXcds) : 0u;
    uint32_t v = 0xFFFFFFFFu;
    if (__lane_id() == 0) {
      uint32_t *q = Q + (size_t)x * kQueueLine;
      if (__hip_atomic_load(q, __ATOMIC_RELAXED, __HIP_MEMORY_SCOPE_AGENT) < limit) v = atomicAdd(q, 1u);
    }
    v = __builtin_amdgcn_readfirstlane(v);
    if (v < limit) return ((v >> 2) * kQueueXcds + x) * 4u + (v & 3u);
    c.dead |= 1u << x;
    c.cur = (c.cur + 1) & (kQueueXcds - 1);
  }
  return 0xFFFFFFFFu;
}
__device__ __forceinline__ void queue_done(uint32_t *Q) {
  if (__lane_id() == 0) {
    __threadfence();
    const uint32_t waves = gridDim.x * (blockDim.x >> 6);
    if (atomicAdd(&Q[kQueueXcds * kQueueLine], 1u) == waves - 1u) {
      for (int x = 0; x <= kQueueXcds; ++x)
        __hip_atomic_store(&Q[(size_t)x * kQueueLine], 0u, __ATOMIC_RELAXED, __HIP_MEMORY_SCOPE_AGENT);
    }
  }
}

template <int OPT>
__global__ void __launch_bounds__((OPT & OPT_WAVEWG) ? 64 : 256,
                                  ((OPT >> 8) & 15) ? ((OPT >> 8) & 15) : 1)
    k_render(RenderArgs A) {
  constexpr bool lean = (OPT & OPT_LEAN) != 0;
  constexpr bool wavewg = (OPT & OPT_WAVEWG) != 0;
  constexpr int kWpg = wavewg ? 1 : 4;
  constexpr bool split = kWpg < 4;
  static_assert(!split || (lean && Tracer<OPT>::kCoop), "one-wave workgroups: lean, cooperative kernels");
  constexpr int kT = 64 * kWpg;
  constexpr int kW = kT / 64;
  __shared__ float s_th[lean ? 1 : 256];
  __shared__ uint32_t s_cnt[kCnt];
  __shared__ LogfTab s_logf[16];
  __shared__ uint32_t s_sph[lean ? 1 : kSphBitWords];
  __shared__ int4 s_dda[split ? 1 : 256];
  __shared__ float4 s_entry[kT];
  __shared__ CoopWave s_coop[kW];
  __shared__ ScanWave s_scan[Tracer<OPT>::kWaveScan ? kW : 1];
  __shared__ float4 s_acc[lean ? 1 : 256];
  __shared__ uint2 s_jmp[kLcgJumps];
  const int tid = threadIdx.x;
  if (A.wgTrace && tid == 0) {
    uint32_t *w = A.wgTrace + 4 * (blockIdx.y * gridDim.x + blockIdx.x);
    w[0] = (uint32_t)__builtin_amdgcn_s_memrealtime();
    w[2] = __builtin_amdgcn_s_getreg((31 << 11) | 4);
    w[3] = __builtin_amdgcn_s_getreg((15 << 11) | 20);
  }
  if (A.probeExit == 1) return;
  uint64_t tStart = 0;
  if constexpr ((OPT & OPT_TIMING) != 0) tStart = __builtin_amdgcn_s_memtime();
  constexpr bool dmaTab = (OPT & OPT_DMATAB) != 0 && kT == 64 && Tracer<OPT>::kCoop;
  if constexpr (dmaTab) {
    typedef __attribute__((address_space(3))) void *LdsPtr;
    const char *jt = reinterpret_cast<const char *>(&kLcgJumpTab.ma[0][0]);
    static_assert(sizeof(kLcgJumpTab.ma) == kLcgJumps * 8 && kLcgJumps * 8 <= 64 * 16 + 16, "jump table: 65 chunks");
    __builtin_amdgcn_global_load_lds((const void *)(jt + 16 * tid), (LdsPtr)s_jmp, 16, 0, 0);
    if (tid == 0)
      __builtin_amdgcn_global_load_lds((const void *)(jt + 1024), (LdsPtr)(reinterpret_cast<char *>(s_jmp) + 1024), 16, 0, 0);
    static_assert(sizeof(LogfTab) == 16, "logf table: one chunk per entry");
    if (tid < 16) __builtin_amdgcn_global_load_lds((const void *)(kLogfTab + tid), (LdsPtr)s_logf, 16, 0, 0);
  }
  const float th = lean ? 0.f : A.srgbTh[tid];
  const LogfTab lt = dmaTab ? LogfTab{0.0, 0.0} : kLogfTab[tid & 15];
  uint32_t sph[kSphBitWords / 256];
  if (!lean && A.numSph) {
#pragma unroll
    for (int k = 0; k < kSphBitWords / 256; ++k) sph[k] = A.sphBits[tid + 256 * k];
  }
  uint2 jmpv[(kLcgJumps + kT - 1) / kT];
#pragma unroll
  for (int k = 0; k < (kLcgJumps + kT - 1) / kT; ++k) {
    const int j = tid + kT * k;
    jmpv[k] = make_uint2(0u, 0u);
    if (!dmaTab && Tracer<OPT>::kCoop && j < kLcgJumps) jmpv[k] = make_uint2(kLcgJumpTab.ma[j][0], kLcgJumpTab.ma[j][1]);
  }
#pragma unroll
  for (int k = 0; k < (kLcgJumps + kT - 1) / kT; ++k) {
    const int j = tid + kT * k;
    if (!dmaTab && Tracer<OPT>::kCoop && j < kLcgJumps) *reinterpret_cast<uvec2 *>(&s_jmp[j]) = __builtin_bit_cast(uvec2, jmpv[k]);
  }
  if constexpr (!lean) s_th[tid] = th;
  if (!dmaTab && tid < 16) s_logf[tid] = lt;
  if (!lean && A.numSph) {
#pragma unroll
    for (int k = 0; k < kSphBitWords / 256; ++k) s_sph[tid + 256 * k] = sph[k];
  }
  if (tid < kCnt) s_cnt[tid] = 0;
  __shared__ uint32_t s_done;
  if (tid == 0) s_done = 0;
  __shared__ uint32_t s_gbits[(OPT & OPT_GRID) ? kGridBitWords : 1];
  if constexpr ((OPT & OPT_GRID) != 0) {
#pragma unroll
    for (int k = 0; k < kGridBitWords / 256; ++k) s_gbits[tid + 256 * k] = A.gridBits[tid + 256 * k];
  }
  if constexpr (dmaTab)
    __builtin_amdgcn_wave_barrier();
  else
    __syncthreads();
  if (A.probeExit == 2) return;
  Tracer<OPT> T{{}, A, s_logf, lean ? A.sphBits : s_sph, s_cnt, {0, 0, 0, 0, 0, 0, 0}};
  T.s_gbits = s_gbits;
  const float *th_p = lean ? A.srgbTh : s_th;
  constexpr uint32_t kNwb = 4 / kWpg;
  uint32_t bx = blockIdx.x;
  int partSel = -1;
  uint32_t splitP = 0u;
  bool emptyItem = false;
  constexpr bool splitOk = wavewg && (OPT & OPT_SPLIT) != 0;
  if constexpr (splitOk) {
    if (bx < A.numSplit) {
      const uint32_t item = scalar_word(A.splitList, bx);
      emptyItem = item == ~0u;
      partSel = emptyItem ? 0 : (int)((((item >> 4) & 15u) << 8) | (item & 15u));
      splitP = emptyItem ? 0u : item >> 8;
    } else {
      bx -= A.numSplit;
    }
  }
  const uint32_t wg = split ? (((bx >> 3) / kNwb) << 3) | (bx & 7u) : bx;
  const int wwave = partSel >= 0 ? (int)(splitP & 3u)
                                  : split ? (int)(((bx >> 3) % kNwb) * kWpg) : 0;
  const int ptid = split ? wwave * 64 + tid : tid;
  if constexpr ((OPT & OPT_TIMING) != 0) {
    T.tLast = tStart;
    T.tmark(0);
  }
  const uint64_t c0 = A.schedCost ? wall_clock64() : 0;
  const uint32_t blk = partSel >= 0 ? splitP >> 2 : A.schedOrder ? scalar_word(A.schedOrder, wg) : wg;
  const uint32_t pkt = blk * 4u + (uint32_t)wwave;
  const bool splitAway = splitOk && partSel < 0 && ((scalar_word(A.splitMask, pkt >> 5) >> (pkt & 31u)) & 1u);
  uint32_t launched = 0u;
  bool pxActive = false;
  if constexpr (Tracer<OPT>::kCoop) {
    constexpr bool queued = (OPT & OPT_QUEUE) != 0;
    static_assert(!queued || (!split && (OPT & (OPT_STATS | OPT_TIMING)) == 0),
                  "persistent launches: 256-thread workgroups, no per-wave statistics");
    const uint32_t perFrame = (uint32_t)A.numTiles * 16u;
    const uint32_t blocksAll = perFrame * (uint32_t)A.numSamples;
    QueueCursor qc = {(int)(blockIdx.x & (kQueueXcds - 1)), 0u};
    uint32_t p = queued ? queue_take(A.queue, blocksAll, qc) : 0u;
    bool more = !queued || p != 0xFFFFFFFFu;
    while (more) {
      uint32_t pblk = blk, nx = 0u;
      int pw = wwave + (tid >> 6), frame = (int)blockIdx.y;
      if constexpr (queued) {
        const uint32_t g = p >> 2;
        frame = A.numSamples > 1 ? (int)(g / perFrame) : 0;
        pblk = g - (uint32_t)frame * perFrame;
        pw = (int)(p & 3u);
      }
      pblk = __builtin_amdgcn_readfirstlane(pblk);
      pw = __builtin_amdgcn_readfirstlane(pw);
      frame = __builtin_amdgcn_readfirstlane(frame);
      int ltid = tid;
      if constexpr (queued) {
        asm volatile("" : "+v"(ltid));
        typedef const __attribute__((address_space(4))) RenderArgs *KArgs;
        KArgs kp = (KArgs)__builtin_amdgcn_kernarg_segment_ptr();
        asm volatile("" : "+s"(kp));
        const RenderArgs &AL = *(const RenderArgs *)kp;
        Tracer<OPT> TL{{}, AL, s_logf, lean ? AL.sphBits : s_sph, s_cnt, {0, 0, 0, 0, 0, 0, 0}};
        TL.s_gbits = s_gbits;
        const Pixel ppx = pixel_of(AL, pblk, pw * 64 + (ltid & 63));
        launched += (uint32_t)__popcll(__ballot(ppx.active));
        render_pixel_coop<OPT>(AL, TL, ppx, lean ? AL.srgbTh : s_th, s_dda, s_entry, s_acc, s_coop[ltid >> 6],
                               &s_scan[Tracer<OPT>::kWaveScan ? ltid >> 6 : 0], s_jmp, ltid, AL.accumID + frame,
                               pblk, pw, frame);
        TL.flush_coop();
      } else {
        const int pl = partSel & 255, pn = 64 >> pl;
        Pixel ppx = pixel_of(A, pblk, pw * 64 + (partSel < 0 ? (ltid & 63) : ((partSel >> 8) * pn) | (ltid & (pn - 1))));
        if (partSel >= 0) ppx.active = ppx.active && (ltid & 63) < pn;
        if (splitAway || emptyItem) ppx.active = false;
        launched += (uint32_t)__popcll(__ballot(ppx.active));
        T.frame = frame;
        render_pixel_coop<OPT>(A, T, ppx, th_p, s_dda, s_entry, s_acc, s_coop[ltid >> 6],
                               &s_scan[Tracer<OPT>::kWaveScan ? ltid >> 6 : 0], s_jmp, ltid, cam_accum_id(A, frame),
                               pblk, pw, frame, partSel);
        if (A.chain && frame < A.numSamples - 1 && frame != A.chainWithhold) {
#ifdef IRT_PROBE_BUILD
          if (A.probeExit != 16)
#endif
            asm volatile("s_waitcnt vmcnt(0)" ::: "memory");
          if (__lane_id() == 0)
            __hip_atomic_store(A.chainFlag + (size_t)pblk * 4u + (uint32_t)pw, A.chainEpoch + (uint32_t)frame + 1u,
                               __ATOMIC_RELAXED, __HIP_MEMORY_SCOPE_AGENT);
        }
      }
      if constexpr (queued) nx = queue_take(A.queue, blocksAll, qc);
      p = nx;
      more = queued && p != 0xFFFFFFFFu;
    }
    if constexpr (queued) queue_done(A.queue);
    T.flush_coop();
  }
  else {
    const Pixel px = pixel_of(A, blk, ptid);
    float4 *slot = A.numSamples > 1 ? A.sampleBuf + (size_t)blockIdx.y * gridDim.x * blockDim.x + blk * 256u + ptid
                                    : nullptr;
    if (px.active) render_pixel<OPT>(A, T, px, th_p, s_dda, s_entry, tid, A.accumID + (int)blockIdx.y, slot);
    pxActive = px.active;
    launched = (uint32_t)__popcll(__ballot(px.active));
  }
  if constexpr ((OPT & OPT_TIMING) != 0) {
    T.tmark(8);
    if ((tid & 63) == 0) {
      for (int k = 0; k < TimeAccOn::kTimeRegions; ++k)
        atomicAdd(&A.counters[5 + k], (unsigned long long)T.tAcc[k]);
      atomicAdd(&A.counters[14], (unsigned long long)(__builtin_amdgcn_s_memtime() - tStart));
      atomicAdd(&A.counters[15], 1ull);
    }
  }
  if constexpr ((OPT & OPT_STATS) != 0) {
    uint32_t ss = T.cnt.steps, sm = T.cnt.steps, ds = T.cnt.deg, dm = T.cnt.deg;
    for (int off = 32; off > 0; off >>= 1) {
      ss += __shfl_down(ss, off, 64);
      sm = max(sm, (uint32_t)__shfl_down(sm, off, 64));
      ds += __shfl_down(ds, off, 64);
      dm = max(dm, (uint32_t)__shfl_down(dm, off, 64));
    }
    const uint32_t d = T.cnt.steps;
    const int bkt = d == 0 ? 0 : (d <= 2 ? 1 : (d <= 5 ? 2 : 3));
    uint32_t hist[4];
    for (int k = 0; k < 4; ++k)
      hist[k] = T.kCoop ? Tracer<OPT>::wave_sum(T.cnt.candHist[k])
                        : (uint32_t)__popcll(__ballot(pxActive && bkt == k));
    if ((tid & 63) == 0) {
      atomicAdd(&A.counters[5], (unsigned long long)ss);
      atomicAdd(&A.counters[6], (unsigned long long)sm);
      atomicAdd(&A.counters[7], (unsigned long long)(T.kCoop ? T.cnt.hops : ds));
      atomicAdd(&A.counters[8], (unsigned long long)(T.kCoop ? T.cnt.locRounds : dm));
      atomicMax(&A.counters[9], (unsigned long long)sm);
      atomicMax(&A.counters[10], (unsigned long long)dm);
      atomicAdd(&A.counters[11], (unsigned long long)T.cnt.rounds);
      for (int k = 0; k < 4; ++k)
        if (hist[k]) atomicAdd(&A.counters[12 + k], (unsigned long long)hist[k]);
    }
  }
  if (A.counters || A.schedCost || A.wgTrace) {
    const int lane = (int)__lane_id();
    if (A.counters && lane == 0 && launched) atomicAdd(&s_cnt[0], launched);
    uint32_t prev = 0;
    if (lane == 0)
      prev = __hip_atomic_fetch_add(&s_done, 1u, __ATOMIC_ACQ_REL, __HIP_MEMORY_SCOPE_WORKGROUP);
    prev = (uint32_t)__shfl((int)prev, 0, 64);
    if (prev == (blockDim.x >> 6) - 1u) {
      if (A.counters) flush_counters(A, s_cnt, lane);
      if (A.schedCost && lane == 0 && (wavewg || wwave == 0) && !splitAway && !emptyItem) {
        uint64_t dt = wall_clock64() - c0;
        if (partSel >= 0) dt <<= (partSel & 255);
        A.schedCost[pkt] = dt > 0xFFFFFFFFull ? 0xFFFFFFFFu : (uint32_t)dt;
      }
      if (A.wgTrace && lane == 0)
        A.wgTrace[4 * (blockIdx.y * gridDim.x + blockIdx.x) + 1] = (uint32_t)__builtin_amdgcn_s_memrealtime();
    }
  }
}

__global__ void __launch_bounds__(256) k_accumulate(RenderArgs A) {
  __shared__ float s_th[256];
  s_th[threadIdx.x] = A.srgbTh[threadIdx.x];
  __syncthreads();
  const uint32_t gid = blockIdx.x * 256u + threadIdx.x;
  const Pixel px = pixel_of(A, blockIdx.x, (int)threadIdx.x);
  if (!px.active) return;
  const size_t lanes = (size_t)gridDim.x * 256u;
  float4 a = A.accum[px.outIdx];
  bool wrote = false;
  for (int k = 0; k < A.numSamples; ++k) {
    const float4 c = A.sampleBuf[(size_t)k * lanes + gid];
    if (c.w == kNoSample) continue;
    const float w = 1.f / (float)(A.accumID + k + 1);
    a.x = w * c.x + (1.f - w) * a.x;
    a.y = w * c.y + (1.f - w) * a.y;
    a.z = w * c.z + (1.f - w) * a.z;
    a.w = w * c.w + (1.f - w) * a.w;
    wrote = true;
  }
  if (!wrote) return;
  A.accum[px.outIdx] = a;
  A.fb[px.outIdx] = srgb_byte(s_th, a.x) + (srgb_byte(s_th, a.y) << 8) +
                    (srgb_byte(s_th, a.z) << 16) + (make_8bit(a.w) << 24);
}

__global__ void __launch_bounds__(256) k_debug_locate(RenderArgs A, const float *xyz, int n,
                                                      int *found, float *value) {
  __shared__ uint32_t s_sph[kSphBitWords];
  __shared__ uint32_t s_cnt[kCnt];
  for (int i = threadIdx.x; i < kSphBitWords; i += 256) s_sph[i] = A.numSph ? A.sphBits[i] : 0u;
  if (threadIdx.x < kCnt) s_cnt[threadIdx.x] = 0;
  __syncthreads();
  Tracer<kDefaultVariant & ~OPT_MONO> T{{}, A, nullptr, s_sph, s_cnt, {0, 0, 0, 0, 0, 0, 0}};
  const int j = (int)(blockIdx.x * 256 + threadIdx.x);
  if (j < n) {
    float v = 0.f;
    found[j] = T.locate(xyz[3 * j], xyz[3 * j + 1], xyz[3 * j + 2], v) ? 1 : 0;
    value[j] = v;
  }
}

template <int O>
__global__ void __launch_bounds__(256) k_debug_locate_wave(RenderArgs A, const float *xyz, int n,
                                                           int *found, float *value) {
  __shared__ uint32_t s_sph[kSphBitWords];
  __shared__ uint32_t s_cnt[kCnt];
  __shared__ CoopWave s_coop[4];
  __shared__ ScanWave s_scan[4];
  for (int i = threadIdx.x; i < kSphBitWords; i += 256) s_sph[i] = A.numSph ? A.sphBits[i] : 0u;
  if (threadIdx.x < kCnt) s_cnt[threadIdx.x] = 0;
  __syncthreads();
  Tracer<O> T{{}, A, nullptr, s_sph, s_cnt, {0, 0, 0, 0, 0, 0, 0}};
  static_assert(Tracer<O>::kWaveScan, "the default kernel scans wave-wide");
  const int j = (int)(blockIdx.x * 256 + threadIdx.x);
  const bool want = j < n;
  float x = 0.f, y = 0.f, z = 0.f;
  if (want) {
    x = xyz[3 * j];
    y = xyz[3 * j + 1];
    z = xyz[3 * j + 2];
  }
  float v = 0.f;
  const bool f = T.locate_wave(want, x, y, z, v, s_coop[threadIdx.x >> 6], s_scan[threadIdx.x >> 6]);
  if (want) {
    found[j] = f ? 1 : 0;
    value[j] = v;
  }
}

void launch_debug_locate(const RenderArgs &A, const float *xyz, int n, int *found, float *value,
                         hipStream_t s, bool wave) {
  if (n <= 0) return;
  constexpr int D = kDefaultVariant & ~OPT_MONO;
  if (wave && A.slots)
    hipLaunchKernelGGL(k_debug_locate_wave<D | OPT_SLOT>, dim3((n + 255) / 256), dim3(256), 0, s, A, xyz, n, found, value);
  else if (wave)
    hipLaunchKernelGGL(k_debug_locate_wave<D>, dim3((n + 255) / 256), dim3(256), 0, s, A, xyz, n, found, value);
  else
    hipLaunchKernelGGL(k_debug_locate, dim3((n + 255) / 256), dim3(256), 0, s, A, xyz, n, found, value);
}

__global__ void __launch_bounds__(256) k_debug_locate_sampler(RenderArgs A, const float *xyz, int n,
                                                              int *found, float *value) {
  __shared__ uint32_t s_cnt[kCnt];
  if (threadIdx.x < kCnt) s_cnt[threadIdx.x] = 0;
  __syncthreads();
  Tracer<kSamplerVariant> T{{}, A, nullptr, nullptr, s_cnt, {0, 0, 0, 0, 0, 0, 0}};
  const int j = (int)(blockIdx.x * 256 + threadIdx.x);
  if (j < n) {
    float v = 0.f;
    const bool f = T.locate(xyz[3 * j], xyz[3 * j + 1], xyz[3 * j + 2], v);
    found[j] = f ? 1 : 0;
    value[j] = f ? v : 0.f;
  }
}

void launch_debug_locate_sampler(const RenderArgs &A, const float *xyz, int n, int *found, float *value,
                                 hipStream_t s) {
  if (n <= 0) return;
  hipLaunchKernelGGL(k_debug_locate_sampler, dim3((n + 255) / 256), dim3(256), 0, s, A, xyz, n, found, value);
}

static_assert((kDefaultVariant & OPT_MONO) != 0, "variant numbering");

#ifdef IRT_ALL_VARIANTS
#define IRT_VARIANTS(X)                                                                  \
  X(4096) X(5120) X(5376) X(36864) X(70656) X(136192) X(529408)                          \
  X(2102272) X(2102528) X(6296576) X(6296832) X(529664) X(2102784) X(33559808)           \
  X(39851264) X(6297088) X(6558976)                                                      \
  X(73405696) X(73667840) X(73405728) X(73667872) X(73930016) X(74192160)                \
  X(73405732) X(73405730) X(1147147552)                                                  \
  X(107222304) X(106960160) X(73438496) X(73700640)
#else
#define IRT_VARIANTS(X) X(73405728) X(73667872) X(1147147552) X(5376) X(36864)
#endif
static_assert(kDefaultVariant == 73405728 && (kDefaultVariant | kNoMissBit) == 73667872 && kNoMissBit == OPT_NOMISS &&
                  (kDefaultVariant | kVoidLocBit) == 1147147552 && kVoidLocBit == OPT_VOIDLOC,
              "the product build's variant list names the default and its scene forms (scene_variant)");

int render_variants(int *out, int cap) {
  int n = 0;
#define IRT_LIST(N) \
  if (n < cap && out) out[n] = N; \
  ++n;
  IRT_VARIANTS(IRT_LIST)
#undef IRT_LIST
  return n;
}

bool render_variant_available(int v) {
#define IRT_CASE(N) if (v == N) return true;
  IRT_VARIANTS(IRT_CASE)
#undef IRT_CASE
  return false;
}

int render_wg_per_block(const RenderArgs &A, int variant) {
  const int per = (variant & OPT_WAVEWG) ? 4 : 1;
  return render_variant_available(variant) && A.sampler == IRT_MODE_USER_GEOM && A.accelMode != IRT_ACCEL_GRID ? per : 1;
}

constexpr int kNoQueue = OPT_WAVEWG | OPT_SERIAL | OPT_STATS | OPT_TIMING;
bool render_split_ok(const RenderArgs &A, int variant) {
  return (variant == kDefaultVariant || variant == (kDefaultVariant | kNoMissBit) || variant == (kDefaultVariant | OPT_VOIDLOC)) &&
         render_wg_per_block(A, variant) == 4;
}

bool render_queue_compiled() {
#ifdef IRT_ALL_VARIANTS
  return true;
#else
  return false;
#endif
}
bool render_queue_ok(const RenderArgs &A, int variant) {
  return render_queue_compiled() && render_variant_available(variant) && (variant & kNoQueue) == 0 &&
         A.sampler == IRT_MODE_USER_GEOM && A.accelMode != IRT_ACCEL_GRID;
}

typedef void (*RenderKernel)(RenderArgs);
template <int N>
RenderKernel kernel_for(const RenderArgs &A, int &threads) {
  constexpr int K = N & ~OPT_MONO;
  constexpr int D = kDefaultVariant & ~OPT_MONO;
  constexpr int DB = D & ~(0xF00 | OPT_WAVEWG | OPT_LEAN);
  constexpr int DW = DB | OPT_WEDGE | (K & OPT_SERIAL);
  static_assert(DW == (kSamplerVariant | (K & OPT_SERIAL)), "k_debug_locate_sampler runs the samplers' Tracer");
  constexpr int DG = DB | 0x400;
  const bool g = A.accelMode == IRT_ACCEL_GRID;
  threads = 256;
  if (A.sampler != IRT_MODE_USER_GEOM && g) return k_render<DW | OPT_GRID>;
  if (A.sampler != IRT_MODE_USER_GEOM) return k_render<DW>;
  if (g) return k_render<DG | OPT_GRID | (K & OPT_SERIAL)>;
  if ((K & OPT_WAVEWG) != 0) threads = 64;
#ifdef IRT_ALL_VARIANTS
  if constexpr ((K & kNoQueue) == 0)
    if (A.queue) return k_render<K | OPT_QUEUE>;
#endif
  if constexpr (K == (kDefaultVariant & ~OPT_MONO) || K == ((kDefaultVariant | kNoMissBit) & ~OPT_MONO) ||
                K == ((kDefaultVariant | OPT_VOIDLOC) & ~OPT_MONO)) {
    if (A.slots) return A.numSplit ? k_render<K | OPT_SPLIT | OPT_SLOT> : k_render<K | OPT_SLOT>;
    if (A.numSplit) return k_render<K | OPT_SPLIT>;
  }
  return k_render<K>;
}

template <int N>
void launch_variant(const RenderArgs &A, int numBlocks, hipStream_t s) {
  int threads = 256;
  const RenderKernel k = kernel_for<N>(A, threads);
  if (A.queue) {
    hipLaunchKernelGGL(k, dim3(numBlocks), dim3(256), 0, s, A);
    numBlocks = A.numTiles * 16;
  } else {
    const int split = A.numSplit ? (int)A.numSplit : 0;
    hipLaunchKernelGGL(k, dim3(numBlocks * (256 / threads) + split, A.numSamples), dim3(threads), 0, s, A);
  }
  if (A.numSamples > 1 && !A.chain) hipLaunchKernelGGL(k_accumulate, dim3(numBlocks), dim3(256), 0, s, A);
}

template <int N>
int queue_wgs_variant(const RenderArgs &A, int numCU, int numBlocks) {
  int threads = 256;
  const RenderKernel k = kernel_for<N>(A, threads);
  int occ = 0;
  if (hipOccupancyMaxActiveBlocksPerMultiprocessor(&occ, k, threads, 0) != hipSuccess || occ < 1) {
    (void)hipGetLastError();
    occ = 1;
  }
  const long long n = (long long)occ * numCU;
  return (int)(n < numBlocks ? n : numBlocks);
}

int render_queue_wgs(const RenderArgs &A, int variant, int numCU, int numBlocks) {
  switch (variant) {
#define IRT_CASE(N) \
  case N:           \
    return queue_wgs_variant<N>(A, numCU, numBlocks);
    IRT_VARIANTS(IRT_CASE)
#undef IRT_CASE
    default:
      return queue_wgs_variant<kDefaultVariant>(A, numCU, numBlocks);
  }
}

template <int N>
void prewarm_variant(hipStream_t s) {
  RenderArgs A = {};
  A.probeExit = 1;
  A.numSamples = 1;
  int threads = 256;
  const RenderKernel k = kernel_for<N>(A, threads);
  hipLaunchKernelGGL(k, dim3(1), dim3(threads), 0, s, A);
  A.numSplit = 8;
  const RenderKernel ks = kernel_for<N>(A, threads);
  if (ks != k) hipLaunchKernelGGL(ks, dim3(1), dim3(threads), 0, s, A);
  A.slots = reinterpret_cast<const float4 *>(16);
  const RenderKernel kts = kernel_for<N>(A, threads);
  if (kts != ks) hipLaunchKernelGGL(kts, dim3(1), dim3(threads), 0, s, A);
  A.numSplit = 0;
  const RenderKernel kt = kernel_for<N>(A, threads);
  if (kt != k) hipLaunchKernelGGL(kt, dim3(1), dim3(threads), 0, s, A);
  A.slots = nullptr;
  A.queue = reinterpret_cast<uint32_t *>(16);
  const RenderKernel kq = kernel_for<N>(A, threads);
  if (kq != kernel_for<N>(RenderArgs{}, threads)) hipLaunchKernelGGL(kq, dim3(1), dim3(256), 0, s, A);
}

void prewarm_render(int variant, hipStream_t s) {
  switch (variant) {
#define IRT_CASE(N) \
  case N:           \
    prewarm_variant<N>(s); \
    return;
    IRT_VARIANTS(IRT_CASE)
#undef IRT_CASE
    default:
      prewarm_variant<kDefaultVariant>(s);
  }
}

void launch_render(const RenderArgs &A, int numBlocks, hipStream_t s, int variant) {
  switch (variant) {
#define IRT_CASE(N) \
  case N:           \
    launch_variant<N>(A, numBlocks, s); \
    return;
    IRT_VARIANTS(IRT_CASE)
#undef IRT_CASE
    default:
      launch_variant<kDefaultVariant>(A, numBlocks, s);
  }
}

}
```

icon-ray-tracing_amd/host/irt_debug.cpp:

```cpp

#include <math.h>
#include <vector>
#include <string.h>

#include "icon_rt_hip_debug.h"
#include "irt_internal.h"

using namespace irt;

struct irt_debug_scene {
  HostScene s;
  std::vector<irt_icon_cell> cells;
  WedgeScene w;
};

extern "C" {

float irt_debug_asinf(float x) { return glibc_asinf(x); }
float irt_debug_atan2f(float y, float x) { return glibc_atan2f(y, x); }
int irt_debug_f2i(float x) { return f2i_x86(x); }
void irt_debug_lcg_jump(uint32_t n, uint32_t *mul, uint32_t *add) { lcg_jump(n, *mul, *add); }

float irt_debug_logf_entry(uint32_t k) { return logf_table()[k & 0x00FFFFFFu]; }

void irt_debug_srgb_thresholds(float *out256) { srgb_thresholds(out256); }

void irt_debug_host_woodcock_log(float *out) {
  for (uint32_t k = 0; k < (1u << 24); ++k) out[k] = logf(1.f - (float)k / (float)0x01000000);
}

uint32_t irt_debug_logf_mismatches(void) {
  uint32_t bad = 0;
  for (uint32_t k = 0; k < (1u << 24); ++k) {
    const float x = 1.f - (float)k / (float)0x01000000;
    if (f2u(glibc_logf_unit(x, kLogfTab)) != f2u(logf(x))) ++bad;
  }
  return bad;
}

int irt_debug_scene_build(const irt_icon_cell *cells, size_t n, irt_debug_scene **out) {
  if (!out || (n && !cells)) {
    set_error("irt_debug_scene_build: null argument");
    return IRT_E_INVALID;
  }
  irt_debug_scene *d = new irt_debug_scene();
  int rc = build_scene(cells, n, d->s);
  if (rc) {
    delete d;
    return rc;
  }
  *out = d;
  return IRT_OK;
}

int irt_debug_scene_info(const irt_debug_scene *s, irt_volume_info *info) {
  if (!s || !info) return IRT_E_INVALID;
  *info = s->s.info;
  return IRT_OK;
}

int irt_debug_scene_locate(const irt_debug_scene *s, irt_vec3f p, float *value,
                           uint32_t *record) {
  if (!s || !value) return IRT_E_INVALID;
  float v = 0.f;
  uint32_t r = 0;
  int hit = locate_host(s->s, p.x, p.y, p.z, v, &r);
  if (hit) {
    *value = v;
    if (record) *record = r;
  }
  return hit;
}

int irt_debug_scene_locate_binned(const irt_debug_scene *s, irt_vec3f p, float *value,
                                  uint32_t *record, uint32_t *tested) {
  if (!s || !value) return IRT_E_INVALID;
  float v = 0.f;
  uint32_t r = 0;
  int hit = locate_bins_host(s->s, p.x, p.y, p.z, v, &r, tested);
  if (hit) {
    *value = v;
    if (record) *record = r;
  }
  return hit;
}

int irt_debug_scene_values(const irt_debug_scene *s, uint32_t rec, float r, float *out2) {
  if (!s || !out2 || rec >= s->s.n) return IRT_E_INVALID;
  const float *hv = &s->s.hv[(size_t)rec * kHV];
  int32_t nl;
  memcpy(&nl, hv + 63, 4);
  out2[0] = hv[32 + find_height(hv, nl, r)];
  out2[1] = record_value_host(s->s, rec,
                              record_path(s->s.meta[rec], s->s.rng[2 * (size_t)rec],
                                          s->s.rng[2 * (size_t)rec + 1], r), r);
  return IRT_OK;
}

int irt_debug_scene_candidates(const irt_debug_scene *s, irt_vec3f p, uint32_t *records,
                               int capacity) {
  if (!s || s->s.G == 0) return 0;
  const uint32_t cell = cubemap_cell(p.x, p.y, p.z, s->s.G);
  const uint32_t b = s->s.offsets[cell], e = s->s.offsets[cell + 1];
  int k = 0;
  for (uint32_t i = b; i < e; ++i, ++k)
    if (records && k < capacity) records[k] = s->s.entryRec[i];
  return k;
}

int irt_debug_scene_planes(const irt_debug_scene *s, uint32_t record, float *out12) {
  if (!s || !out12 || record >= s->s.n) return IRT_E_INVALID;
  memcpy(out12, &s->s.planes[12 * (size_t)record], 12 * sizeof(float));
  return IRT_OK;
}

void irt_debug_scene_free(irt_debug_scene *s) { delete s; }

int irt_debug_scene_array(const irt_debug_scene *s, int which, void *dst, size_t capacity,
                          size_t *bytes) {
  if (!s || !bytes) {
    set_error("irt_debug_scene_array: null argument");
    return IRT_E_INVALID;
  }
  const HostScene &S = s->s;
  std::vector<uint32_t> rec;
  const void *src = nullptr;
  size_t n = 0;
  switch (which) {
    case IRT_DEBUG_ARRAY_BIN_HDR: src = S.binHdr.data(); n = S.binHdr.size() * 4; break;
    case IRT_DEBUG_ARRAY_FAT: src = S.fat.data(); n = S.fat.size() * 4; break;
    case IRT_DEBUG_ARRAY_BLOCKS: src = S.blocks.data(); n = S.blocks.size() * 4; break;
    case IRT_DEBUG_ARRAY_SPH_R: src = S.sphR.data(); n = S.sphR.size() * 4; break;
    case IRT_DEBUG_ARRAY_SPH_OFF: src = S.sphOff.data(); n = S.sphOff.size() * 4; break;
    case IRT_DEBUG_ARRAY_SPH_REC:
      for (uint32_t r : S.sphRec) {
        int32_t nl;
        memcpy(&nl, &S.hv[(size_t)r * kHV + 63], 4);
        rec.push_back(r);
        rec.push_back((uint32_t)nl);
      }
      src = rec.data();
      n = rec.size() * 4;
      break;
    case IRT_DEBUG_ARRAY_SPH_BITS: src = S.sphBits.data(); n = S.sphBits.size() * 4; break;
    default:
      set_error("irt_debug_scene_array: unknown array %d", which);
      return IRT_E_INVALID;
  }
  *bytes = n;
  if (dst && capacity >= n && n) memcpy(dst, src, n);
  return IRT_OK;
}

int irt_debug_scene_locate_wedge(irt_debug_scene *s, irt_vec3f p, float *value) {
  if (!s || !value) return IRT_E_INVALID;
  if (s->w.G == 0) {
    set_error("irt_debug_scene_locate_wedge: call irt_debug_scene_build_wedges first");
    return IRT_E_INVALID;
  }
  return wedge_locate_host(s->w, s->cells.data(), p.x, p.y, p.z, *value) ? 1 : 0;
}

int irt_debug_scene_build_wedges(irt_debug_scene *s, const irt_icon_cell *cells, size_t n) {
  if (!s || (n && !cells) || n != s->s.n) {
    set_error("irt_debug_scene_build_wedges: cells do not match the scene");
    return IRT_E_INVALID;
  }
  s->cells.assign(cells, cells + n);
  return build_wedges(cells, n, s->w);
}

int irt_debug_scene_locate_triangle(irt_debug_scene *s, irt_vec3f p, float *value,
                                    uint32_t *record) {
  if (!s || !value) return IRT_E_INVALID;
  if (s->w.G == 0) {
    set_error("irt_debug_scene_locate_triangle: call irt_debug_scene_build_wedges first");
    return IRT_E_INVALID;
  }
  return triangle_locate_host(s->w, s->cells.data(), p.x, p.y, p.z, *value, record) ? 1 : 0;
}

int irt_debug_intersect_wedge(const float *v24, irt_vec3f p, float *value) {
  WV4 V[6];
  memcpy(V, v24, sizeof(V));
  float v = 0.f;
  const bool hit = intersect_wedge(v, p.x, p.y, p.z, V);
  if (hit) *value = v;
  return hit ? 1 : 0;
}

int irt_debug_sched_order(const uint32_t *cost, int numBlocks, int tilesX, int tileStride, int policy,
                          int splitLg, float splitFactor, int numCU, int wavewg, size_t capacity,
                          uint32_t maxSplit, uint32_t *out, uint32_t *numSplit) {
  if (!cost || !out || !numSplit || numBlocks < 0 || numBlocks % 16 || (size_t)numBlocks > capacity ||
      splitLg < 0 || splitLg > 3 || maxSplit % 8) {
    set_error("irt_debug_sched_order: bad argument");
    return IRT_E_INVALID;
  }
  *numSplit = sched_order(cost, numBlocks, tilesX, tileStride, policy, splitLg, splitFactor, numCU,
                          wavewg != 0, capacity, maxSplit, out);
  return IRT_OK;
}

}
```

icon-ray-tracing_amd/python/irt.py:

```python
from __future__ import annotations

import ctypes as C
import os
from dataclasses import dataclass

import numpy as np

PKG_DIR = os.path.dirname(os.path.dirname(os.path.abspath(__file__)))
LIB_PATH = os.environ.get("IRT_LIB_PATH") or os.path.join(PKG_DIR, "libicon_rt_hip.so")

CELL_DTYPE = np.dtype(
    [("lat", "<f4", (3,)), ("lon", "<f4", (3,)), ("numLayers", "<i4"),
     ("height", "<f4", (32,)), ("value", "<f4", (32,))], align=False)
assert CELL_DTYPE.itemsize == 284

RAYGEN_WITH_ACCEL = 0
RAYGEN_AE = 1
ACCEL_SPHERE = 0
ACCEL_GRID = 1
MODE_USER_GEOM = 0
MODE_TRIANGLES = 1
MODE_CUBQL = 2
ALL_LIB_PATH = os.path.join(PKG_DIR, "libicon_rt_hip_all.so")


def compiled_variants() -> tuple:
    L = lib()
    n = L.irt_debug_variants(None, 0)
    out = (C.c_int * n)()
    L.irt_debug_variants(out, n)
    return tuple(out)


E_INVALID, E_HIP, E_DATA, E_IO, E_CHAIN = -1, -2, -3, -4, -5


class IrtError(RuntimeError):
    def __init__(self, msg, code=None):
        super().__init__(msg)
        self.code = code


class Vec3(C.Structure):
    _fields_ = [("x", C.c_float), ("y", C.c_float), ("z", C.c_float)]

    def tolist(self):
        return [self.x, self.y, self.z]


class Vec4(C.Structure):
    _fields_ = [("x", C.c_float), ("y", C.c_float), ("z", C.c_float), ("w", C.c_float)]


class Box1(C.Structure):
    _fields_ = [("lower", C.c_float), ("upper", C.c_float)]


class Box3(C.Structure):
    _fields_ = [("lower", Vec3), ("upper", Vec3)]


class LaunchParams(C.Structure):
    _fields_ = [("org", Vec3), ("dir_00", Vec3), ("dir_du", Vec3), ("dir_dv", Vec3),
                ("accumID", C.c_int32), ("ambientColor", Vec3), ("ambientRadiance", C.c_float),
                ("unitDistance", C.c_float), ("raygen", C.c_int32), ("accelMode", C.c_int32),
                ("mode", C.c_int32)]

    def camera12(self) -> np.ndarray:
        return np.array(self.org.tolist() + self.dir_00.tolist() + self.dir_du.tolist()
                        + self.dir_dv.tolist(), dtype=np.float32)


class VolumeInfo(C.Structure):
    _fields_ = [("numCells", C.c_uint64), ("bounds", Box3), ("sphericalBounds", Box3),
                ("dataRange", Box1), ("unitDistance", C.c_float), ("shellDims", C.c_int32 * 3),
                ("locatorFaceRes", C.c_int32), ("locatorEntries", C.c_uint64),
                ("deviceBytes", C.c_uint64)]


class RenderStats(C.Structure):
    _fields_ = [("raysLaunched", C.c_uint64), ("raysInBox", C.c_uint64),
                ("locateCalls", C.c_uint64), ("samplesFound", C.c_uint64),
                ("candidatesTested", C.c_uint64), ("kernelMs", C.c_float)]

    def asdict(self):
        return {f: getattr(self, f) for f, _ in self._fields_}


_lib = None


def lib() -> C.CDLL:
    global _lib
    if _lib is None:
        try:
            import torch
        except ImportError:
            pass
        if not os.path.exists(LIB_PATH):
            raise IrtError(f"{LIB_PATH} not built; run `make -C icon-ray-tracing_amd` "
                           "(or __graft_entry__.build())")
        L = C.CDLL(LIB_PATH)
        P, I, F, S = C.c_void_p, C.c_int, C.c_float, C.c_size_t
        L.irt_last_error.restype = C.c_char_p
        sig = {
            "irt_create": [P, S, I, C.POINTER(P)],
            "irt_create_begin": [S, I, C.POINTER(P)],
            "irt_create_append": [P, P, S],
            "irt_create_end": [P],
            "irt_create_from_file": [C.c_char_p, C.c_long, I, C.POINTER(P)],
            "irt_create_synth": [I, I, I, F, F, C.c_uint32, I, C.POINTER(P)],
            "irt_create_synth_terrain": [I, I, I, F, F, C.c_uint32, F, I, C.POINTER(P)],
            "irt_debug_context_array": [P, I, P, S, C.POINTER(S)],
            "irt_debug_scene_array": [P, I, P, S, C.POINTER(S)],
            "irt_destroy": [P],
            "irt_get_volume_info": [P, C.POINTER(VolumeInfo)],
            "irt_set_transfunc": [P, P, I, Box1, F],
            "irt_update_values": [P, S, S, P],
            "irt_update_values_device": [P, S, S, P, P],
            "irt_update_values_end": [P],
            "irt_clear_frame": [P, P, P, S, P],
            "irt_render": [P, C.POINTER(LaunchParams), I, I, P, P, P],
            "irt_render_tiles": [P, C.POINTER(LaunchParams), I, I, I, I, P, P,
                                 C.POINTER(C.c_int), P],
            "irt_render_accumulate": [P, C.POINTER(LaunchParams), I, I, I, P, P, P],
            "irt_render_sequence": [P, C.POINTER(LaunchParams), I, I, I, P, P, P],
            "irt_render_tiles_accumulate": [P, C.POINTER(LaunchParams), I, I, I, I, I, P, P,
                                            C.POINTER(C.c_int), P],
            "irt_unpack_tiles": [P, P, I, I, I, I, P, P],
            "irt_deal_tiles": [C.POINTER(LaunchParams), C.POINTER(VolumeInfo), I, I, I, F, P, S,
                               C.POINTER(C.c_int)],
            "irt_render_tile_list": [P, C.POINTER(LaunchParams), I, I, P, I, I, P, P, P],
            "irt_unpack_tile_table": [P, P, I, I, P, I, I, P, P],
            "irt_get_render_stats": [P, C.POINTER(RenderStats)],
            "irt_get_render_stats_total": [P, C.POINTER(RenderStats), C.POINTER(C.c_longlong)],
            "irt_reset_render_stats_total": [P],
            "irt_set_timing_interval": [P, C.c_int],
            "irt_get_shell": [P, P, P],
            "irt_get_grid": [P, P, P],
            "irt_build_wedge_accel": [P, P, S],
            "irt_num_tiles": [I, I],
            "irt_load_ic": [C.c_char_p, C.c_long, P, S, C.POINTER(S)],
            "irt_save_ic": [C.c_char_p, P, S],
            "irt_convert_icon": [C.POINTER(ConvertOpts), P, S, C.POINTER(S)],
            "irt_convert_icon_umesh": [C.POINTER(ConvertOpts), C.c_char_p, C.POINTER(S), C.POINTER(S)],
            "irt_filter_cells": [P, S, Box1, Box1, C.POINTER(S)],
            "irt_compute_volume_info": [P, S, C.POINTER(VolumeInfo)],
            "irt_default_transfunc": [Box1, P, C.POINTER(Box1)],
            "irt_resample_lut": [P, I, P, I],
            "irt_camera_view_all": [Box3, F, I, I, C.POINTER(LaunchParams)],
            "irt_camera_look_at": [Vec3, Vec3, Vec3, F, I, I, C.POINTER(LaunchParams)],
            "irt_synth_grid": [I, I, I, F, F, C.c_uint32, P, S, C.POINTER(S)],
            "irt_synth_grid_terrain": [I, I, I, F, F, C.c_uint32, F, P, S, C.POINTER(S)],
            "irt_debug_asinf": [F],
            "irt_debug_atan2f": [F, F],
            "irt_debug_f2i": [F],
            "irt_debug_logf_entry": [C.c_uint32],
            "irt_debug_srgb_thresholds": [P],
            "irt_debug_scene_build": [P, S, C.POINTER(P)],
            "irt_debug_scene_info": [P, C.POINTER(VolumeInfo)],
            "irt_debug_scene_locate": [P, Vec3, C.POINTER(C.c_float), C.POINTER(C.c_uint32)],
            "irt_debug_scene_locate_binned": [P, Vec3, C.POINTER(C.c_float),
                                              C.POINTER(C.c_uint32), C.POINTER(C.c_uint32)],
            "irt_debug_scene_candidates": [P, Vec3, P, I],
            "irt_debug_scene_planes": [P, C.c_uint32, P],
            "irt_debug_scene_values": [P, C.c_uint32, F, P],
            "irt_debug_logf_mismatches": [],
            "irt_debug_host_woodcock_log": [P],
            "irt_debug_device_woodcock_log": [I, P],
            "irt_debug_scene_free": [P],
        }
        for name, args in sig.items():
            fn = getattr(L, name)
            fn.argtypes = args
            if name not in ("irt_last_error",):
                fn.restype = C.c_int
        L.irt_debug_asinf.restype = F
        L.irt_debug_atan2f.restype = F
        L.irt_debug_logf_entry.restype = F
        L.irt_destroy.restype = None
        L.irt_debug_scene_free.restype = None
        L.irt_debug_srgb_thresholds.restype = None
        _lib = L
    return _lib


def _check(rc: int, what: str):
    if rc != 0:
        msg = lib().irt_last_error().decode(errors="replace")
        raise IrtError(f"{what} failed ({rc}): {msg}", rc)


def _ptr(a: np.ndarray) -> C.c_void_p:
    return C.c_void_p(a.ctypes.data)


def vec3(v) -> Vec3:
    return Vec3(float(v[0]), float(v[1]), float(v[2]))


def box1(lo, hi) -> Box1:
    return Box1(float(lo), float(hi))


def default_kernel_id(ctx=None) -> int:
    L = lib()
    if ctx is not None:
        L.irt_debug_get_variant.argtypes = [C.c_void_p]
        v = int(L.irt_debug_get_variant(ctx._h)) & ~4096
        d = int(L.irt_debug_default_variant())
        L.irt_debug_slot_use.argtypes = [C.c_void_p, C.c_void_p]
        if v in ((d & ~4096), (d | 262144) & ~4096, (d | 1073741824) & ~4096) and L.irt_debug_slot_use(ctx._h, None) == 1:
            v |= 128
        return v
    return int(L.irt_debug_default_variant()) & ~4096


def synth_grid(root_n: int, bisections: int, levels: int, top_height: float = 75e3,
               noise: float = 0.0, seed: int = 1234, terrain: float = 0.0) -> np.ndarray:
    n = C.c_size_t()
    _check(lib().irt_synth_grid_terrain(root_n, bisections, levels, top_height, noise, seed, terrain,
                                        None, 0, C.byref(n)), "irt_synth_grid")
    cells = np.zeros(n.value, dtype=CELL_DTYPE)
    _check(lib().irt_synth_grid_terrain(root_n, bisections, levels, top_height, noise, seed, terrain,
                                        _ptr(cells), n.value, C.byref(n)), "irt_synth_grid")
    return cells


def load_ic(path: str, max_num_cells: int = -1) -> np.ndarray:
    n = C.c_size_t()
    _check(lib().irt_load_ic(path.encode(), max_num_cells, None, 0, C.byref(n)), "irt_load_ic")
    cells = np.zeros(n.value, dtype=CELL_DTYPE)
    _check(lib().irt_load_ic(path.encode(), max_num_cells, _ptr(cells), n.value, C.byref(n)),
           "irt_load_ic")
    return cells


class ConvertOpts(C.Structure):
    _fields_ = [("hgridFile", C.c_char_p), ("hsurfFile", C.c_char_p),
                ("hhlFiles", C.POINTER(C.c_char_p)), ("numHhlFiles", C.c_int),
                ("dataFiles", C.POINTER(C.c_char_p)), ("numDataFiles", C.c_int),
                ("varName", C.c_char_p), ("maxLayers", C.c_int)]


def convert_icon(hgrid: str, hsurf: str, hhl: list, data: list, var: str = "pres",
                 max_layers: int = 5) -> np.ndarray:
    hp = (C.c_char_p * max(len(hhl), 1))(*[f.encode() for f in hhl])
    dp = (C.c_char_p * max(len(data), 1))(*[f.encode() for f in data])
    o = ConvertOpts(hgrid.encode(), hsurf.encode(), hp, len(hhl), dp, len(data), var.encode(),
                    max_layers)
    n = C.c_size_t()
    _check(lib().irt_convert_icon(C.byref(o), None, 0, C.byref(n)), "irt_convert_icon")
    cells = np.zeros(n.value, dtype=CELL_DTYPE)
    _check(lib().irt_convert_icon(C.byref(o), _ptr(cells), n.value, C.byref(n)),
           "irt_convert_icon")
    return cells


def convert_icon_umesh(hgrid: str, hsurf: str, hhl: list, data: list, path: str,
                       var: str = "pres", max_layers: int = 5):
    hp = (C.c_char_p * max(len(hhl), 1))(*[f.encode() for f in hhl])
    dp = (C.c_char_p * max(len(data), 1))(*[f.encode() for f in data])
    o = ConvertOpts(hgrid.encode(), hsurf.encode(), hp, len(hhl), dp, len(data), var.encode(),
                    max_layers)
    nv, nw = C.c_size_t(), C.c_size_t()
    _check(lib().irt_convert_icon_umesh(C.byref(o), path.encode(), C.byref(nv), C.byref(nw)),
           "irt_convert_icon_umesh")
    return nv.value, nw.value


def read_umesh(path: str) -> dict:
    raw = open(path, "rb").read()
    pos = 0

    def u64():
        nonlocal pos
        v = int(np.frombuffer(raw, np.uint64, 1, pos)[0])
        pos += 8
        return v

    def arr(dtype, width):
        nonlocal pos
        n = u64()
        a = np.frombuffer(raw, dtype, n * width, pos).reshape(n, width) if width > 1 else \
            np.frombuffer(raw, dtype, n, pos)
        pos += a.nbytes
        return a

    out = {"magic": u64(), "vertices": arr(np.float32, 3), "scalars": arr(np.float32, 1)}
    for name, w in (("triangles", 3), ("quads", 4), ("tets", 4), ("pyrs", 5),
                    ("wedges", 6), ("hexes", 8)):
        out[name] = arr(np.int32, w)
    if pos != len(raw):
        raise ValueError(f"{path}: {len(raw) - pos} trailing bytes")
    return out


def save_ic(path: str, cells: np.ndarray):
    cells = np.ascontiguousarray(cells, dtype=CELL_DTYPE)
    _check(lib().irt_save_ic(path.encode(), _ptr(cells), cells.size), "irt_save_ic")


def filter_cells(cells: np.ndarray, lat_range=(-np.inf, np.inf), lon_range=(-np.inf, np.inf)):
    out = np.array(cells, dtype=CELL_DTYPE, copy=True)
    n = C.c_size_t()
    _check(lib().irt_filter_cells(_ptr(out), out.size, box1(*lat_range), box1(*lon_range),
                                  C.byref(n)), "irt_filter_cells")
    return out[: n.value].copy()


def volume_info(cells: np.ndarray) -> VolumeInfo:
    cells = np.ascontiguousarray(cells, dtype=CELL_DTYPE)
    info = VolumeInfo()
    _check(lib().irt_compute_volume_info(_ptr(cells), cells.size, C.byref(info)),
           "irt_compute_volume_info")
    return info


def default_transfunc(data_range) -> tuple[np.ndarray, tuple[float, float]]:
    lut = np.zeros((300, 4), dtype=np.float32)
    vr = Box1()
    _check(lib().irt_default_transfunc(box1(*data_range), _ptr(lut), C.byref(vr)),
           "irt_default_transfunc")
    return lut, (vr.lower, vr.upper)


def resample_lut(src: np.ndarray, n: int) -> np.ndarray:
    src = np.ascontiguousarray(src, dtype=np.float32).reshape(-1, 4)
    dst = np.zeros((n, 4), dtype=np.float32)
    _check(lib().irt_resample_lut(_ptr(src), src.shape[0], _ptr(dst), n), "irt_resample_lut")
    return dst


def camera_view_all(bounds: Box3, img_w: int, img_h: int, fovy_deg: float = 90.0) -> LaunchParams:
    lp = LaunchParams()
    _check(lib().irt_camera_view_all(bounds, fovy_deg, img_w, img_h, C.byref(lp)),
           "irt_camera_view_all")
    return lp


def camera_look_at(vp, vi, vu, fovy_deg: float, img_w: int, img_h: int) -> LaunchParams:
    lp = LaunchParams()
    _check(lib().irt_camera_look_at(vec3(vp), vec3(vi), vec3(vu), fovy_deg, img_w, img_h,
                                    C.byref(lp)), "irt_camera_look_at")
    return lp


def num_tiles(w: int, h: int) -> int:
    return lib().irt_num_tiles(w, h)


def deal_tiles(lp: LaunchParams, info: VolumeInfo, w: int, h: int, ranks: int,
               rank0_extra: float = 0.0) -> np.ndarray:
    m = C.c_int()
    _check(lib().irt_deal_tiles(C.byref(lp), C.byref(info), w, h, ranks, rank0_extra, None, 0,
                                C.byref(m)), "irt_deal_tiles")
    table = np.full((ranks, m.value), -1, np.int32)
    _check(lib().irt_deal_tiles(C.byref(lp), C.byref(info), w, h, ranks, rank0_extra,
                                _ptr(table), table.size, C.byref(m)), "irt_deal_tiles")
    return table


@dataclass
class FrameSetup:
    lp: LaunchParams
    lut: np.ndarray
    value_range: tuple[float, float]
    opacity_scale: float
    info: VolumeInfo


FRAMING_CAMERA = ((0.0, 0.0, 1.4e7), (0.0, 0.0, 0.0), (0.0, 1.0, 0.0), 60.0)


def setup_frame(cells: np.ndarray, width: int, height: int, camera=None,
                camera_div=None, raygen: int = RAYGEN_WITH_ACCEL, info: VolumeInfo = None) -> FrameSetup:
    if info is None:
        info = volume_info(cells)
    lut, vr = default_transfunc((info.dataRange.lower, info.dataRange.upper))
    dw, dh = camera_div if camera_div is not None else (width, height)
    if camera is None:
        lp = camera_view_all(info.bounds, dw, dh)
    else:
        vp, vi, vu, fovy = camera
        lp = camera_look_at(vp, vi, vu, fovy, dw, dh)
    lp.accumID = 0
    lp.ambientColor = Vec3(1.0, 1.0, 1.0)
    lp.ambientRadiance = 1.0
    lp.unitDistance = info.unitDistance
    lp.raygen = raygen
    return FrameSetup(lp=lp, lut=lut, value_range=vr, opacity_scale=1.0, info=info)


SCENE_ARRAYS = {"bin_hdr": 0, "fat": 1, "blocks": 2, "sph_r": 3, "sph_off": 4, "sph_rec": 5,
                "sph_bits": 6}
CONTEXT_ARRAYS = {"slots": 7, "grid_bits": 8}


def _array(fn, h, name):
    which = SCENE_ARRAYS[name] if name in SCENE_ARRAYS else CONTEXT_ARRAYS[name]
    n = C.c_size_t()
    _check(fn(h, which, None, 0, C.byref(n)), "scene array")
    out = np.zeros(max(n.value, 1), np.uint8)
    _check(fn(h, which, _ptr(out), n.value, C.byref(n)), "scene array")
    return out[:n.value]


def check_update_values(values) -> np.ndarray:
    if not isinstance(values, np.ndarray) or values.dtype != np.float32:
        raise TypeError("update_values: values must be a float32 numpy array")
    if values.ndim != 2 or values.shape[1] != 32:
        raise ValueError(f"update_values: values must have shape (n, 32), not {values.shape}")
    if not values.flags.c_contiguous:
        raise ValueError("update_values: values must be C-contiguous")
    return values


class Context:

    def __init__(self, cells: np.ndarray = None, device: int = 0, _handle=None):
        if _handle is None:
            cells = np.ascontiguousarray(cells, dtype=CELL_DTYPE)
            _handle = C.c_void_p()
            _check(lib().irt_create(_ptr(cells), cells.size, device, C.byref(_handle)),
                   "irt_create")
        self._h = _handle
        self.device = device
        self.info = VolumeInfo()
        _check(lib().irt_get_volume_info(self._h, C.byref(self.info)), "irt_get_volume_info")

    @classmethod
    def synth(cls, root_n: int, bisections: int, levels: int, device: int = 0,
              top_height: float = 75e3, noise: float = 0.0, seed: int = 1234,
              terrain: float = 0.0) -> "Context":
        h = C.c_void_p()
        _check(lib().irt_create_synth_terrain(root_n, bisections, levels, top_height, noise, seed,
                                              terrain, device, C.byref(h)), "irt_create_synth")
        return cls(device=device, _handle=h)

    @classmethod
    def from_file(cls, path: str, max_num_cells: int = -1, device: int = 0) -> "Context":
        h = C.c_void_p()
        _check(lib().irt_create_from_file(path.encode(), max_num_cells, device, C.byref(h)),
               "irt_create_from_file")
        return cls(device=device, _handle=h)

    @classmethod
    def streamed(cls, chunks, num_cells: int, device: int = 0) -> "Context":
        h = C.c_void_p()
        _check(lib().irt_create_begin(num_cells, device, C.byref(h)), "irt_create_begin")
        try:
            for ch in chunks:
                ch = np.ascontiguousarray(ch, dtype=CELL_DTYPE)
                _check(lib().irt_create_append(h, _ptr(ch), ch.size), "irt_create_append")
            _check(lib().irt_create_end(h), "irt_create_end")
        except Exception:
            lib().irt_destroy(h)
            raise
        return cls(device=device, _handle=h)

    def array(self, name: str) -> np.ndarray:
        return _array(lib().irt_debug_context_array, self._h, name)

    def array_bytes(self, name: str) -> int:
        which = SCENE_ARRAYS[name] if name in SCENE_ARRAYS else CONTEXT_ARRAYS[name]
        n = C.c_size_t()
        _check(lib().irt_debug_context_array(self._h, which, None, 0, C.byref(n)), "scene array")
        return n.value

    def close(self):
        if getattr(self, "_h", None):
            lib().irt_destroy(self._h)
            self._h = None

    def __del__(self):
        try:
            self.close()
        except Exception:
            pass

    def __enter__(self):
        return self

    def __exit__(self, *a):
        self.close()

    def set_transfunc(self, lut: np.ndarray, value_range, opacity_scale: float = 1.0):
        lut = np.ascontiguousarray(lut, dtype=np.float32).reshape(-1, 4)
        _check(lib().irt_set_transfunc(self._h, _ptr(lut), lut.shape[0], box1(*value_range),
                                       float(opacity_scale)), "irt_set_transfunc")

    def update_values(self, values: np.ndarray, first: int = 0):
        values = check_update_values(values)
        _check(lib().irt_update_values(self._h, int(first), values.shape[0], _ptr(values)),
               "irt_update_values")

    def update_values_device(self, ptr: int, n: int, first: int = 0, stream: int = 0):
        _check(lib().irt_update_values_device(self._h, int(first), int(n), C.c_void_p(ptr),
                                              C.c_void_p(stream)), "irt_update_values_device")

    def end_update(self):
        _check(lib().irt_update_values_end(self._h), "irt_update_values_end")
        _check(lib().irt_get_volume_info(self._h, C.byref(self.info)), "irt_get_volume_info")

    def set_statistics(self, on: bool):
        L = lib()
        L.irt_set_statistics.argtypes = [C.c_void_p, C.c_int]
        _check(L.irt_set_statistics(self._h, 1 if on else 0), "irt_set_statistics")

    def set_queue(self, on: bool):
        L = lib()
        L.irt_debug_set_queue.argtypes = [C.c_void_p, C.c_int]
        _check(L.irt_debug_set_queue(self._h, 1 if on else 0), "irt_debug_set_queue")

    def set_wg_trace(self, ptr: int):
        L = lib()
        L.irt_debug_set_wg_trace.argtypes = [C.c_void_p, C.c_void_p]
        _check(L.irt_debug_set_wg_trace(self._h, C.c_void_p(ptr or None)), "irt_debug_set_wg_trace")

    def set_chain(self, on: bool):
        L = lib()
        L.irt_debug_set_chain.argtypes = [C.c_void_p, C.c_int]
        _check(L.irt_debug_set_chain(self._h, 1 if on else 0), "irt_debug_set_chain")

    def chain_errors(self) -> int:
        L = lib()
        L.irt_debug_chain_errors.argtypes = [C.c_void_p]
        n = L.irt_debug_chain_errors(self._h)
        if n < 0:
            raise IrtError("irt_debug_chain_errors failed")
        return n

    def set_chain_fault(self, spins: int, withhold_frame: int = -1):
        L = lib()
        L.irt_debug_set_chain_fault.argtypes = [C.c_void_p, C.c_uint32, C.c_int]
        _check(L.irt_debug_set_chain_fault(self._h, spins, withhold_frame), "irt_debug_set_chain_fault")

    def sched_split(self):
        L = lib()
        L.irt_debug_sched_split.argtypes = [C.c_void_p, C.POINTER(C.c_int), C.POINTER(C.c_int)]
        n, lg = C.c_int(), C.c_int()
        _check(L.irt_debug_sched_split(self._h, C.byref(n), C.byref(lg)), "irt_debug_sched_split")
        return n.value, lg.value

    def launch_workgroups(self, num_tiles: int, frames: int = 1) -> int:
        L = lib()
        L.irt_debug_launch_workgroups.argtypes = [C.c_void_p, C.c_int, C.c_int]
        L.irt_debug_launch_workgroups.restype = C.c_longlong
        n = L.irt_debug_launch_workgroups(self._h, num_tiles, frames)
        if n < 0:
            raise IrtError("irt_debug_launch_workgroups failed")
        return n

    def queue(self) -> bool:
        L = lib()
        L.irt_debug_get_queue.argtypes = [C.c_void_p]
        return L.irt_debug_get_queue(self._h) == 1

    def clear(self, fb_ptr: int, accum_ptr: int, num_pixels: int, stream: int = 0):
        _check(lib().irt_clear_frame(self._h, C.c_void_p(fb_ptr), C.c_void_p(accum_ptr),
                                     num_pixels, C.c_void_p(stream)), "irt_clear_frame")

    def render(self, lp: LaunchParams, width: int, height: int, fb_ptr: int, accum_ptr: int,
               stream: int = 0):
        _check(lib().irt_render(self._h, C.byref(lp), width, height, C.c_void_p(fb_ptr),
                                C.c_void_p(accum_ptr), C.c_void_p(stream)), "irt_render")

    def render_tiles(self, lp: LaunchParams, width: int, height: int, tile_begin: int,
                     tile_stride: int, fb_ptr: int, accum_ptr: int, stream: int = 0) -> int:
        n = C.c_int()
        _check(lib().irt_render_tiles(self._h, C.byref(lp), width, height, tile_begin,
                                      tile_stride, C.c_void_p(fb_ptr), C.c_void_p(accum_ptr),
                                      C.byref(n), C.c_void_p(stream)), "irt_render_tiles")
        return n.value

    def render_sequence(self, lps, width: int, height: int, fb_ptr: int, accum_ptr: int,
                        stream: int = 0):
        arr = (LaunchParams * len(lps))(*lps)
        _check(lib().irt_render_sequence(self._h, arr, len(lps), width, height, C.c_void_p(fb_ptr),
                                         C.c_void_p(accum_ptr), C.c_void_p(stream)),
               "irt_render_sequence")

    def render_tile_list_sequence(self, lps, width: int, height: int, tiles, fb_tiles_ptr: int,
                                  accum_tiles_ptr: int, stream: int = 0):
        arr = (LaunchParams * len(lps))(*lps)
        t = np.ascontiguousarray(tiles, dtype=np.int32)
        L = lib()
        L.irt_render_tile_list_sequence.argtypes = [C.c_void_p, C.POINTER(LaunchParams), C.c_int, C.c_int, C.c_int,
                                                    C.c_void_p, C.c_int, C.c_void_p, C.c_void_p, C.c_void_p]
        _check(L.irt_render_tile_list_sequence(self._h, arr, len(lps), width, height, _ptr(t), t.size,
                                               C.c_void_p(fb_tiles_ptr), C.c_void_p(accum_tiles_ptr),
                                               C.c_void_p(stream)), "irt_render_tile_list_sequence")

    def render_accumulate(self, lp: LaunchParams, width: int, height: int, num_frames: int,
                          fb_ptr: int, accum_ptr: int, stream: int = 0):
        _check(lib().irt_render_accumulate(self._h, C.byref(lp), width, height, num_frames,
                                           C.c_void_p(fb_ptr), C.c_void_p(accum_ptr),
                                           C.c_void_p(stream)), "irt_render_accumulate")

    def render_tiles_accumulate(self, lp: LaunchParams, width: int, height: int, tile_begin: int,
                                tile_stride: int, num_frames: int, fb_ptr: int, accum_ptr: int,
                                stream: int = 0) -> int:
        n = C.c_int()
        _check(lib().irt_render_tiles_accumulate(self._h, C.byref(lp), width, height, tile_begin,
                                                 tile_stride, num_frames, C.c_void_p(fb_ptr),
                                                 C.c_void_p(accum_ptr), C.byref(n),
                                                 C.c_void_p(stream)), "irt_render_tiles_accumulate")
        return n.value

    def render_tile_list(self, lp: LaunchParams, width: int, height: int, tiles, num_frames: int,
                         fb_tiles_ptr: int, accum_tiles_ptr: int, stream: int = 0):
        t = np.ascontiguousarray(tiles, dtype=np.int32)
        _check(lib().irt_render_tile_list(self._h, C.byref(lp), width, height, _ptr(t), t.size,
                                          num_frames, C.c_void_p(fb_tiles_ptr),
                                          C.c_void_p(accum_tiles_ptr), C.c_void_p(stream)),
               "irt_render_tile_list")

    def unpack_tile_table(self, gathered_ptr: int, table: np.ndarray, width: int, height: int,
                          fb_ptr: int, stream: int = 0):
        t = np.ascontiguousarray(table, dtype=np.int32)
        _check(lib().irt_unpack_tile_table(self._h, C.c_void_p(gathered_ptr), t.shape[0], t.shape[1],
                                           _ptr(t), width, height, C.c_void_p(fb_ptr),
                                           C.c_void_p(stream)), "irt_unpack_tile_table")

    def unpack_tiles(self, gathered_ptr: int, num_ranks: int, max_tiles: int, width: int,
                     height: int, fb_ptr: int, stream: int = 0):
        _check(lib().irt_unpack_tiles(self._h, C.c_void_p(gathered_ptr), num_ranks, max_tiles,
                                      width, height, C.c_void_p(fb_ptr), C.c_void_p(stream)),
               "irt_unpack_tiles")

    def stats(self) -> RenderStats:
        st = RenderStats()
        _check(lib().irt_get_render_stats(self._h, C.byref(st)), "irt_get_render_stats")
        return st

    def stats_total(self) -> tuple[RenderStats, int]:
        st = RenderStats()
        n = C.c_longlong()
        _check(lib().irt_get_render_stats_total(self._h, C.byref(st), C.byref(n)),
               "irt_get_render_stats_total")
        return st, n.value

    def reset_stats_total(self):
        _check(lib().irt_reset_render_stats_total(self._h), "irt_reset_render_stats_total")

    def set_timing_interval(self, every: int):
        _check(lib().irt_set_timing_interval(self._h, int(every)), "irt_set_timing_interval")

    def build_wedge_accel(self, cells: np.ndarray):
        cells = np.ascontiguousarray(cells, dtype=CELL_DTYPE)
        _check(lib().irt_build_wedge_accel(self._h, _ptr(cells), cells.size),
               "irt_build_wedge_accel")

    def locate_sampler(self, points: np.ndarray, mode: int) -> tuple[np.ndarray, np.ndarray]:
        pts = np.ascontiguousarray(points, dtype=np.float32).reshape(-1, 3)
        found = np.zeros(len(pts), np.int32)
        value = np.zeros(len(pts), np.float32)
        L = lib()
        L.irt_debug_locate_sampler.argtypes = [C.c_void_p, C.c_int, C.c_void_p, C.c_int, C.c_void_p,
                                               C.c_void_p]
        _check(L.irt_debug_locate_sampler(self._h, int(mode), _ptr(pts), len(pts), _ptr(found),
                                          _ptr(value)), "irt_debug_locate_sampler")
        return found, value

    def grid(self) -> tuple[np.ndarray, np.ndarray]:
        n = 256 ** 3
        vr = np.zeros((n, 2), np.float32)
        mo = np.zeros(n, np.float32)
        _check(lib().irt_get_grid(self._h, _ptr(vr), _ptr(mo)), "irt_get_grid")
        return vr, mo

    def shell(self) -> tuple[np.ndarray, np.ndarray]:
        n = int(np.prod(list(self.info.shellDims)))
        vr = np.zeros((n, 2), dtype=np.float32)
        mo = np.zeros(n, dtype=np.float32)
        _check(lib().irt_get_shell(self._h, _ptr(vr), _ptr(mo)), "irt_get_shell")
        return vr, mo


class DebugScene:

    def __init__(self, cells: np.ndarray):
        cells = np.ascontiguousarray(cells, dtype=CELL_DTYPE)
        h = C.c_void_p()
        _check(lib().irt_debug_scene_build(_ptr(cells), cells.size, C.byref(h)),
               "irt_debug_scene_build")
        self._h = h
        self.info = VolumeInfo()
        lib().irt_debug_scene_info(self._h, C.byref(self.info))

    def locate(self, p):
        v = C.c_float()
        r = C.c_uint32()
        hit = lib().irt_debug_scene_locate(self._h, vec3(p), C.byref(v), C.byref(r))
        return (True, v.value, r.value) if hit == 1 else (False, 0.0, None)

    def locate_binned(self, p):
        v = C.c_float()
        r = C.c_uint32()
        t = C.c_uint32()
        hit = lib().irt_debug_scene_locate_binned(self._h, vec3(p), C.byref(v), C.byref(r),
                                                  C.byref(t))
        return (True, v.value, r.value, t.value) if hit == 1 else (False, 0.0, None, t.value)

    def candidates(self, p):
        n = lib().irt_debug_scene_candidates(self._h, vec3(p), None, 0)
        out = np.zeros(max(n, 1), dtype=np.uint32)
        lib().irt_debug_scene_candidates(self._h, vec3(p), _ptr(out), n)
        return out[:n]

    def values(self, rec: int, r: float):
        out = np.zeros(2, dtype=np.float32)
        _check(lib().irt_debug_scene_values(self._h, rec, C.c_float(r), _ptr(out)),
               "irt_debug_scene_values")
        return out

    def array(self, name: str) -> np.ndarray:
        return _array(lib().irt_debug_scene_array, self._h, name)

    def planes(self, rec: int) -> np.ndarray:
        out = np.zeros(12, dtype=np.float32)
        _check(lib().irt_debug_scene_planes(self._h, rec, _ptr(out)), "irt_debug_scene_planes")
        return out.reshape(3, 4)

    def close(self):
        if getattr(self, "_h", None):
            lib().irt_debug_scene_free(self._h)
            self._h = None

    def __del__(self):
        try:
            self.close()
        except Exception:
            pass
```

include/icon_rt_hip_debug.h:

```cpp
#ifndef ICON_RT_HIP_DEBUG_H
#define ICON_RT_HIP_DEBUG_H

#include "icon_rt_hip.h"

#ifdef __cplusplus
extern "C" {
#endif

float irt_debug_asinf(float x);
float irt_debug_atan2f(float y, float x);
int irt_debug_f2i(float x);
void irt_debug_lcg_jump(uint32_t n, uint32_t *mul, uint32_t *add);

float irt_debug_logf_entry(uint32_t k);
void irt_debug_srgb_thresholds(float *out256);

uint32_t irt_debug_logf_mismatches(void);
void irt_debug_host_woodcock_log(float *out);

typedef struct irt_debug_scene irt_debug_scene;
int irt_debug_scene_build(const irt_icon_cell *cells, size_t n, irt_debug_scene **out);
int irt_debug_scene_info(const irt_debug_scene *s, irt_volume_info *info);
int irt_debug_scene_locate(const irt_debug_scene *s, irt_vec3f p, float *value,
                           uint32_t *record);
int irt_debug_scene_locate_binned(const irt_debug_scene *s, irt_vec3f p, float *value,
                                  uint32_t *record, uint32_t *tested);
int irt_debug_scene_values(const irt_debug_scene *s, uint32_t rec, float r, float *out2);
int irt_debug_scene_candidates(const irt_debug_scene *s, irt_vec3f p, uint32_t *records,
                               int capacity);
int irt_debug_scene_planes(const irt_debug_scene *s, uint32_t record, float *out12);
void irt_debug_scene_free(irt_debug_scene *s);
int irt_debug_scene_build_wedges(irt_debug_scene *s, const irt_icon_cell *cells, size_t n);
int irt_debug_scene_locate_wedge(irt_debug_scene *s, irt_vec3f p, float *value);
int irt_debug_scene_locate_triangle(irt_debug_scene *s, irt_vec3f p, float *value,
                                    uint32_t *record);
int irt_debug_intersect_wedge(const float *v24, irt_vec3f p, float *value);

enum {
  IRT_DEBUG_ARRAY_BIN_HDR = 0,
  IRT_DEBUG_ARRAY_FAT = 1,
  IRT_DEBUG_ARRAY_BLOCKS = 2,
  IRT_DEBUG_ARRAY_SPH_R = 3,
  IRT_DEBUG_ARRAY_SPH_OFF = 4,
  IRT_DEBUG_ARRAY_SPH_REC = 5,
  IRT_DEBUG_ARRAY_SPH_BITS = 6,
  IRT_DEBUG_ARRAY_SLOTS = 7,
  IRT_DEBUG_ARRAY_GRID_BITS = 8
};
int irt_debug_context_array(const irt_context *ctx, int which, void *dst, size_t capacity,
                            size_t *bytes);
int irt_debug_scene_array(const irt_debug_scene *s, int which, void *dst, size_t capacity,
                          size_t *bytes);

int irt_debug_set_variant(irt_context *ctx, int variant);
int irt_debug_default_variant(void);
int irt_debug_slot_use(const irt_context *ctx, double *tfSamples);
int irt_debug_get_variant(const irt_context *ctx);
int irt_debug_variants(int *out, int capacity);
int irt_debug_set_queue(irt_context *ctx, int on);
int irt_debug_get_queue(const irt_context *ctx);
int irt_debug_queue_wgs(const irt_context *ctx);
int irt_debug_counters(irt_context *ctx, unsigned long long *out16);

int irt_debug_device_math(int device, const float *a, const float *y, const float *x, int n,
                          float *out_asinf, float *out_atan2f);
int irt_debug_fast_math_bounds(int device, double *out4);
void irt_debug_fast_spherical_consts(float *out2);
int irt_debug_device_woodcock_log(int device, float *out);
int irt_debug_device_srgb(int device, const float *x, uint32_t *out, int n);
int irt_debug_locate(irt_context *ctx, const float *xyz, int n, int *found, float *value);
int irt_debug_locate_wave(irt_context *ctx, const float *xyz, int n, int *found, float *value);
int irt_debug_locate_sampler(irt_context *ctx, int mode, const float *xyz, int n, int *found,
                             float *value);
int irt_debug_sched(irt_context *ctx, int *policy, int *lastApplied, long long *applied);
int irt_debug_set_wg_trace(irt_context *ctx, uint32_t *trace);
long long irt_debug_launch_workgroups(const irt_context *ctx, int numTiles, int numFrames);
int irt_debug_sched_split(const irt_context *ctx, int *numSplit, int *splitLg);
int irt_debug_sched_order(const uint32_t *cost, int numBlocks, int tilesX, int tileStride, int policy,
                          int splitLg, float splitFactor, int numCU, int wavewg, size_t capacity,
                          uint32_t maxSplit, uint32_t *out, uint32_t *numSplit);
int irt_debug_set_chain(irt_context *ctx, int on);
int irt_debug_chain_errors(irt_context *ctx);
int irt_debug_set_chain_fault(irt_context *ctx, uint32_t spins, int withholdFrame);

#ifdef __cplusplus
}
#endif
#endif
```

Baseline: 17200 Mray/s.

## Skip void ray packets with host-computed conservative sphere-miss bitmask

Adds a host-side conservative test that marks 8x8 pixel packets whose rays provably miss the outer bounding sphere. The mask is cached per camera and uploaded to the device, and a new kernel variant reads it. For void packets the kernel writes the blended background accumulation on frame 0 and returns immediately on later frames, so it skips ray generation and traversal for pixels that see only empty space. The cost is an extra kernel specialisation, host geometry computation on camera change, and a small copy to the device. There is also correctness risk if the conservative bound is wrong.

```diff
diff --git a/icon-ray-tracing_amd/csrc/irt_context.h b/icon-ray-tracing_amd/csrc/irt_context.h
--- a/icon-ray-tracing_amd/csrc/irt_context.h
+++ b/icon-ray-tracing_amd/csrc/irt_context.h
@@ -131,6 +131,12 @@
   float4 *d_frameCams = nullptr;
   float4 *h_frameCams = nullptr;
   size_t frameCamCap = 0;
+  irt::VoidCache voidCache;
+  uint32_t *d_voidBits = nullptr;
+  uint32_t *h_voidBits = nullptr;
+  size_t voidCap = 0;
+  long long voidOnDevice = 0;
+  long long lastVoid = 0;
   bool queueOn = false;
   uint32_t *d_queue = nullptr;
   int numCU = 0;
diff --git a/icon-ray-tracing_amd/csrc/irt_context.hip b/icon-ray-tracing_amd/csrc/irt_context.hip
--- a/icon-ray-tracing_amd/csrc/irt_context.hip
+++ b/icon-ray-tracing_amd/csrc/irt_context.hip
@@ -30,7 +30,7 @@
   void *ptrs[] = {c->d_binHdr, c->d_fat, c->slot.slots, c->d_blocks, c->d_sphR, c->d_sphOff, c->d_sphRec,
                   c->d_sphBits, c->d_samples, c->d_maxOp, c->d_gridVR, c->d_gridMaxOp, c->d_gridBits, c->d_wOff, c->d_wRec, c->d_wBox, c->d_wTrig, c->d_schedOrder, c->d_schedCost, c->d_srgb, c->d_valueRanges,
                   c->d_lut, c->d_counters, c->d_counterBuckets, c->d_meta, c->d_queue, c->d_chainFlag,
-                  c->d_frameCams, c->d_tfStat, c->d_rects, c->d_updStat, c->d_probeCounts};
+                  c->d_frameCams, c->d_tfStat, c->d_rects, c->d_updStat, c->d_probeCounts, c->d_voidBits};
   for (void *p : ptrs)
     if (p) (void)hipFree(p);
   if (c->d_cells) (void)hipFree(c->d_cells);
@@ -41,6 +41,7 @@
   if (c->h_schedOrder) (void)hipHostFree(c->h_schedOrder);
   if (c->h_frameCams) (void)hipHostFree(c->h_frameCams);
   if (c->h_chainFail) (void)hipHostFree(c->h_chainFail);
+  if (c->h_voidBits) (void)hipHostFree(c->h_voidBits);
   for (LaunchSlot &r : c->ring) {
     if (r.ev0) (void)hipEventDestroy(r.ev0);
     if (r.ev1) (void)hipEventDestroy(r.ev1);
diff --git a/icon-ray-tracing_amd/csrc/irt_debug_hooks.hip b/icon-ray-tracing_amd/csrc/irt_debug_hooks.hip
--- a/icon-ray-tracing_amd/csrc/irt_debug_hooks.hip
+++ b/icon-ray-tracing_amd/csrc/irt_debug_hooks.hip
@@ -303,6 +303,8 @@
   return c->slot.slots && (c->slotAlways || c->slotSparse) ? 1 : 0;
 }
 
+extern "C" long long irt_debug_void_use(const irt_context *c) { return c ? c->lastVoid : -1; }
+
 extern "C" int irt_debug_context_array(const irt_context *c, int which, void *dst, size_t capacity,
                                        size_t *bytes) {
   if (!c || !bytes || c->building) {
diff --git a/icon-ray-tracing_amd/csrc/irt_internal.h b/icon-ray-tracing_amd/csrc/irt_internal.h
--- a/icon-ray-tracing_amd/csrc/irt_internal.h
+++ b/icon-ray-tracing_amd/csrc/irt_internal.h
@@ -87,6 +87,43 @@
                      int splitLg, float splitFactor, int numCU, bool wavewg, size_t cap,
                      uint32_t maxSplit, uint32_t *out);
 
+struct VoidRequest {
+  float cam[12];
+  float bmin[3], bmax[3];
+  float rOuter, rInner;
+  int W, H, tileBegin, tileStride, numTiles;
+  int raygen, accelMode, mode;
+  const int32_t *tileList;
+};
+inline VoidRequest void_request(const irt_launch_params &lp, const irt_volume_info &info, int W, int H, int tileBegin,
+                                int tileStride, int numTiles, const int32_t *tileList) {
+  VoidRequest q;
+  const irt_vec3f *cam[4] = {&lp.org, &lp.dir_00, &lp.dir_du, &lp.dir_dv};
+  for (int k = 0; k < 4; ++k) {
+    q.cam[3 * k] = cam[k]->x;
+    q.cam[3 * k + 1] = cam[k]->y;
+    q.cam[3 * k + 2] = cam[k]->z;
+  }
+  q.bmin[0] = info.bounds.lower.x, q.bmin[1] = info.bounds.lower.y, q.bmin[2] = info.bounds.lower.z;
+  q.bmax[0] = info.bounds.upper.x, q.bmax[1] = info.bounds.upper.y, q.bmax[2] = info.bounds.upper.z;
+  q.rOuter = info.sphericalBounds.upper.x;
+  q.rInner = info.sphericalBounds.lower.x;
+  q.W = W, q.H = H, q.tileBegin = tileBegin, q.tileStride = tileStride, q.numTiles = numTiles;
+  q.raygen = lp.raygen, q.accelMode = lp.accelMode, q.mode = lp.mode;
+  q.tileList = tileList;
+  return q;
+}
+inline size_t void_words(int numTiles) { return ((size_t)(numTiles > 0 ? numTiles : 0) * 64 + 31) / 32; }
+uint32_t void_packets(const VoidRequest &q, uint32_t *bits);
+struct VoidCache {
+  std::vector<unsigned char> key;
+  std::vector<uint32_t> bits;
+  uint32_t count = 0;
+  bool keyed = false, valid = false;
+  long long generation = 0;
+  bool lookup(const VoidRequest &q, bool defer = false);
+};
+
 int synth_open(int rootN, int bisections, int levels, float topHeight, float noise, uint32_t seed,
                float terrainHeight,
                void **gen, size_t *total);
diff --git a/icon-ray-tracing_amd/csrc/irt_kernels.h b/icon-ray-tracing_amd/csrc/irt_kernels.h
--- a/icon-ray-tracing_amd/csrc/irt_kernels.h
+++ b/icon-ray-tracing_amd/csrc/irt_kernels.h
@@ -77,6 +77,7 @@
   float slotEdge[3];
   int slotBins;
   int slotSubs;
+  const uint32_t *voidBits;
 };
 constexpr int kQueueLine = 32;
 constexpr uint32_t kChainSpinsDefault = 1u << 20;
@@ -103,6 +104,7 @@
   OPT_NOVOIDRUN = 2,
   OPT_NOHOLESKIP = 4,
   OPT_SLOT = 128,
+  OPT_VOID = 16,
 };
 constexpr int OPT_MONO = 4096;
 constexpr int kDefaultVariant = 73405728;
@@ -117,6 +119,7 @@
 bool render_queue_ok(const RenderArgs &A, int variant);
 bool render_queue_compiled();
 bool render_split_ok(const RenderArgs &A, int variant);
+bool render_void_ok(const RenderArgs &A, int variant);
 int render_queue_wgs(const RenderArgs &A, int variant, int numCU, int numBlocks);
 void launch_render(const RenderArgs &A, int numBlocks, hipStream_t s, int variant);
 void prewarm_render(int variant, hipStream_t s);
diff --git a/icon-ray-tracing_amd/csrc/irt_launch.hip b/icon-ray-tracing_amd/csrc/irt_launch.hip
--- a/icon-ray-tracing_amd/csrc/irt_launch.hip
+++ b/icon-ray-tracing_amd/csrc/irt_launch.hip
@@ -510,6 +510,35 @@
   return IRT_OK;
 }
 
+int prepare_void(irt_context *c, const irt_launch_params *lp, const RenderRequest &r, Launch &L) {
+  RenderArgs &A = L.A;
+  c->lastVoid = 0;
+  if (!(A.chain && !r.seq && r.numFrames > 1 && L.numTiles > 0 && c->chainWithhold < 0 && c->probeExit == 0 &&
+        !stats_variant(c) && lp->raygen == IRT_RAYGEN_WITH_ACCEL && lp->accelMode == IRT_ACCEL_SPHERE &&
+        render_void_ok(A, c->variant)))
+    return IRT_OK;
+  c->voidCache.lookup(void_request(*lp, c->info, r.W, r.H, r.tileBegin, r.tileStride, L.numTiles, r.tileList), true);
+  if (!c->voidCache.count) return IRT_OK;
+  const size_t words = void_words(L.numTiles);
+  if (words > c->voidCap) {
+    int rc = grow(c, Retire::SlotsThenStream, L.s, &c->voidCap, words,
+                  {{(void **)&c->d_voidBits, [](size_t n) { return n * sizeof(uint32_t); }, false},
+                   {(void **)&c->h_voidBits, [](size_t n) { return kSlots * n * sizeof(uint32_t); }, true}},
+                  nullptr);
+    c->voidOnDevice = 0;
+    if (rc) return rc;
+  }
+  if (c->voidOnDevice != c->voidCache.generation) {
+    uint32_t *h = c->h_voidBits + (size_t)L.slot * c->voidCap;
+    memcpy(h, c->voidCache.bits.data(), words * sizeof(uint32_t));
+    IRT_HIP(hipMemcpyAsync(c->d_voidBits, h, words * sizeof(uint32_t), hipMemcpyHostToDevice, L.s));
+    c->voidOnDevice = c->voidCache.generation;
+  }
+  A.voidBits = c->d_voidBits;
+  c->lastVoid = c->voidCache.count;
+  return IRT_OK;
+}
+
 int stage_sequence(irt_context *c, const RenderRequest &r, Launch &L) {
   RenderArgs &A = L.A;
   if (!r.seq) return IRT_OK;
@@ -607,7 +636,8 @@
   decide_queue(c, r.numFrames, L);
   if ((rc = decide_sched(c, lp, r, L))) return rc;
   count_workgroups(c, r, L);
-  if ((rc = choose_counters(c, L)) || (rc = setup_chain(c, r.numFrames, L)) || (rc = stage_sequence(c, r, L)) ||
+  if ((rc = choose_counters(c, L)) || (rc = setup_chain(c, r.numFrames, L)) || (rc = prepare_void(c, lp, r, L)) ||
+      (rc = stage_sequence(c, r, L)) ||
       (rc = ensure_samples(c, r.numFrames, L)))
     return rc;
   return launch_and_commit(c, L);
diff --git a/icon-ray-tracing_amd/csrc/irt_raygen.h b/icon-ray-tracing_amd/csrc/irt_raygen.h
--- a/icon-ray-tracing_amd/csrc/irt_raygen.h
+++ b/icon-ray-tracing_amd/csrc/irt_raygen.h
@@ -194,6 +194,45 @@
     unsigned long long *dst = A.counterBuckets ? A.counterBuckets + (wg % kCounterBuckets) * 8 : A.counters;
     atomicAdd(&dst[lane], (unsigned long long)s_cnt[lane]);
   }
+}
+
+__device__ __forceinline__ void void_packet(const RenderArgs &KA, uint32_t blk, int pwave, int frame) {
+  const RenderArgs *vp = &KA;
+  asm volatile("" : "+v"(vp));
+  const RenderArgs &A = *vp;
+  const int lane = (int)__lane_id();
+  const Pixel px = pixel_of(A, blk, pwave * 64 + lane);
+  if (frame == 0 && px.active) {
+    float4 nv = A.accum[px.outIdx];
+    const float c = 0.f;
+#pragma nounroll
+    for (int g = 0; g < A.numSamples; ++g) {
+      const float w = 1.f / (float)(A.accumID + g + 1);
+      nv.x = w * c + (1.f - w) * nv.x;
+      nv.y = w * c + (1.f - w) * nv.y;
+      nv.z = w * c + (1.f - w) * nv.z;
+      nv.w = w * c + (1.f - w) * nv.w;
+    }
+    const float *th = A.srgbTh;
+    const uint32_t rgba = srgb_byte(th, nv.x) + (srgb_byte(th, nv.y) << 8) + (srgb_byte(th, nv.z) << 16) +
+                          (make_8bit(nv.w) << 24);
+    typedef float f4v __attribute__((ext_vector_type(4)));
+    const f4v t = {nv.x, nv.y, nv.z, nv.w};
+    __builtin_nontemporal_store(t, reinterpret_cast<f4v *>(&A.accum[px.outIdx]));
+    __builtin_nontemporal_store(rgba, &A.fb[px.outIdx]);
+  }
+  if (A.counters) {
+    const uint32_t n = (uint32_t)__popcll(__ballot(px.active));
+    const size_t wg = (size_t)blockIdx.y * gridDim.x + blockIdx.x;
+    if (A.wgCounts) {
+      if (lane < kCnt) A.wgCounts[wg * kCnt + lane] = lane < 2 ? n : 0u;
+    } else if (lane < 2 && n) {
+      unsigned long long *dst = A.counterBuckets ? A.counterBuckets + (wg % kCounterBuckets) * 8 : A.counters;
+      atomicAdd(&dst[lane], (unsigned long long)n);
+    }
+  }
+  if (A.wgTrace && lane == 0)
+    A.wgTrace[4 * (blockIdx.y * gridDim.x + blockIdx.x) + 1] = (uint32_t)__builtin_amdgcn_s_memrealtime();
 }
 
 constexpr float kNoSample = -1.f;
diff --git a/icon-ray-tracing_amd/csrc/irt_render.hip b/icon-ray-tracing_amd/csrc/irt_render.hip
--- a/icon-ray-tracing_amd/csrc/irt_render.hip
+++ b/icon-ray-tracing_amd/csrc/irt_render.hip
@@ -64,6 +64,21 @@
     w[3] = __builtin_amdgcn_s_getreg((15 << 11) | 20);
   }
   if (A.probeExit == 1) return;
+  constexpr bool kVoid = (OPT & OPT_VOID) != 0;
+  static_assert(!kVoid || (wavewg && lean && Tracer<OPT>::kCoop &&
+                           (OPT & (OPT_SPLIT | OPT_SLOT | OPT_STATS | OPT_TIMING | OPT_QUEUE | OPT_GRID | OPT_WEDGE)) == 0),
+                "void packets: the default kernels' plain grid form");
+  if constexpr (kVoid) {
+    const RenderArgs &VA = fresh_args();
+    const uint32_t vb = blockIdx.x, vwave = (vb >> 3) & 3u;
+    const uint32_t vblk = ((vb >> 5) << 3) | (vb & 7u), vpkt = vblk * 4u + vwave;
+    uint32_t isVoid = VA.voidBits ? (scalar_word(VA.voidBits, vpkt >> 5) >> (vpkt & 31u)) & 1u : 0u;
+    asm volatile("" : "+s"(isVoid));
+    if (isVoid) {
+      void_packet(VA, vblk, (int)vwave, (int)blockIdx.y);
+      return;
+    }
+  }
   uint64_t tStart = 0;
   if constexpr ((OPT & OPT_TIMING) != 0) tStart = __builtin_amdgcn_s_memtime();
   constexpr bool dmaTab = (OPT & OPT_DMATAB) != 0 && kT == 64 && Tracer<OPT>::kCoop;
@@ -422,6 +437,10 @@
          render_wg_per_block(A, variant) == 4;
 }
 
+bool render_void_ok(const RenderArgs &A, int variant) {
+  return render_split_ok(A, variant) && !A.slots && !A.queue && !A.numSplit && !A.schedOrder;
+}
+
 bool render_queue_compiled() {
 #ifdef IRT_ALL_VARIANTS
   return true;
@@ -455,6 +474,7 @@
 #endif
   if constexpr (K == (kDefaultVariant & ~OPT_MONO) || K == ((kDefaultVariant | kNoMissBit) & ~OPT_MONO) ||
                 K == ((kDefaultVariant | OPT_VOIDLOC) & ~OPT_MONO)) {
+    if (A.voidBits) return k_render<K | OPT_VOID>;
     if (A.slots) return A.numSplit ? k_render<K | OPT_SPLIT | OPT_SLOT> : k_render<K | OPT_SLOT>;
     if (A.numSplit) return k_render<K | OPT_SPLIT>;
   }
@@ -518,6 +538,10 @@
   const RenderKernel kt = kernel_for<N>(A, threads);
   if (kt != k) hipLaunchKernelGGL(kt, dim3(1), dim3(threads), 0, s, A);
   A.slots = nullptr;
+  A.voidBits = reinterpret_cast<const uint32_t *>(16);
+  const RenderKernel kv = kernel_for<N>(A, threads);
+  if (kv != k) hipLaunchKernelGGL(kv, dim3(1), dim3(threads), 0, s, A);
+  A.voidBits = nullptr;
   A.queue = reinterpret_cast<uint32_t *>(16);
   const RenderKernel kq = kernel_for<N>(A, threads);
   if (kq != kernel_for<N>(RenderArgs{}, threads)) hipLaunchKernelGGL(kq, dim3(1), dim3(256), 0, s, A);
diff --git a/icon-ray-tracing_amd/host/irt_debug.cpp b/icon-ray-tracing_amd/host/irt_debug.cpp
--- a/icon-ray-tracing_amd/host/irt_debug.cpp
+++ b/icon-ray-tracing_amd/host/irt_debug.cpp
@@ -12,6 +12,10 @@
   HostScene s;
   std::vector<irt_icon_cell> cells;
   WedgeScene w;
+};
+
+struct irt_debug_void_cache {
+  VoidCache c;
 };
 
 extern "C" {
@@ -202,4 +206,35 @@
   return IRT_OK;
 }
 
-}
+irt_debug_void_cache *irt_debug_void_cache_create(void) { return new irt_debug_void_cache(); }
+void irt_debug_void_cache_free(irt_debug_void_cache *cache) { delete cache; }
+
+int irt_debug_void_packets(irt_debug_void_cache *cache, const irt_launch_params *lp, const irt_volume_info *info,
+                           int W, int H, int tileBegin, int tileStride, const int32_t *tileList, int listCount,
+                           uint32_t *bits, size_t capacity, uint32_t *numVoid, long long *computations) {
+  if (!lp || !info || !numVoid || W <= 0 || H <= 0 || tileBegin < 0 || tileStride <= 0 || listCount < 0) {
+    set_error("irt_debug_void_packets: bad argument");
+    return IRT_E_INVALID;
+  }
+  const int total = ((W + 63) / 64) * ((H + 63) / 64);
+  const int numTiles = tileList ? listCount : tileBegin < total ? (total - tileBegin + tileStride - 1) / tileStride : 0;
+  for (int k = 0; tileList && k < listCount; ++k)
+    if (tileList[k] < 0 || tileList[k] >= total) {
+      set_error("irt_debug_void_packets: tile id %d at %d outside [0, %d)", tileList[k], k, total);
+      return IRT_E_INVALID;
+    }
+  if (void_words(numTiles) > capacity || (!bits && capacity)) {
+    set_error("irt_debug_void_packets: %zu words needed", void_words(numTiles));
+    return IRT_E_INVALID;
+  }
+  const VoidRequest q = void_request(*lp, *info, W, H, tileBegin, tileStride, numTiles, tileList);
+  VoidCache local;
+  VoidCache &vc = cache ? cache->c : local;
+  vc.lookup(q);
+  if (void_words(numTiles)) memcpy(bits, vc.bits.data(), void_words(numTiles) * sizeof(uint32_t));
+  *numVoid = vc.count;
+  if (computations) *computations = vc.generation;
+  return IRT_OK;
+}
+
+}
diff --git a/icon-ray-tracing_amd/host/irt_void.cpp b/icon-ray-tracing_amd/host/irt_void.cpp
--- /dev/null
+++ b/icon-ray-tracing_amd/host/irt_void.cpp
@@ -0,0 +1,159 @@
+
+#include <math.h>
+#include <string.h>
+
+#include <algorithm>
+
+#include "irt_internal.h"
+
+namespace irt {
+
+namespace {
+
+struct V3 {
+  double x, y, z;
+};
+V3 operator+(V3 a, V3 b) { return {a.x + b.x, a.y + b.y, a.z + b.z}; }
+V3 operator*(double s, V3 a) { return {s * a.x, s * a.y, s * a.z}; }
+double dot(V3 a, V3 b) { return a.x * b.x + a.y * b.y + a.z * b.z; }
+double norm(V3 a) { return sqrt(dot(a, a)); }
+double abs1(V3 a) { return fabs(a.x) + fabs(a.y) + fabs(a.z); }
+
+bool hits_box(V3 org, V3 d, const double lo[3], const double hi[3]) {
+  const double o[3] = {org.x, org.y, org.z}, dd[3] = {d.x, d.y, d.z};
+  double t0 = 0.0, t1 = INFINITY;
+  for (int k = 0; k < 3; ++k) {
+    if (dd[k] == 0.0) {
+      if (!(o[k] > lo[k] && o[k] < hi[k])) return false;
+      continue;
+    }
+    const double a = (lo[k] - o[k]) / dd[k], b = (hi[k] - o[k]) / dd[k];
+    t0 = std::max(t0, std::min(a, b));
+    t1 = std::min(t1, std::max(a, b));
+  }
+  return t0 < t1;
+}
+
+struct View {
+  V3 org, d00, du, dv, axis;
+  double uu, vv, uv;
+  double m0, mu, mv;
+  double cosN, sinN;
+  V3 dir(double a, double b) const { return d00 + a * du + b * dv; }
+};
+struct Rect {
+  double a0, a1, b0, b1;
+};
+enum { kUnbounded = -2, kCentreHits = -1, kUndecided = 0, kClear = 1, kAllHit = 2 };
+
+int sphere_rect(const View &v, const Rect &r, double &delta) {
+  const double ha = 0.5 * (r.a1 - r.a0), hb = 0.5 * (r.b1 - r.b0);
+  const V3 c = v.dir(r.a0 + ha, r.b0 + hb);
+  const double lc = norm(c), h = sqrt(ha * ha * v.uu + hb * hb * v.vv + 2.0 * ha * hb * v.uv), dmin = lc - h;
+  if (!(lc > 0.0) || !(h < 0.16 * lc)) return kUnbounded;
+  delta = 8.0 * ldexp(1.0, -24) * (v.m0 + r.a1 * v.mu + r.b1 * v.mv) / dmin + 4e-5;
+  const double ct = dot(c, v.axis) / lc, x0 = 1.01 * h / dmin, x = x0 + delta + 1e-9;
+  if (ct > v.cosN + v.sinN * x0) return kAllHit;
+  if (!(ct < v.cosN)) return kCentreHits;
+  const double L = v.cosN * (1.0 - 0.5 * x * x) - v.sinN * x;
+  return ct < L && ct > -L ? kClear : kUndecided;
+}
+bool sphere_clear(const View &v, const Rect &r, int depth) {
+  double delta;
+  const int res = sphere_rect(v, r, delta);
+  if (res != kUndecided || depth == 3) return res == kClear;
+  const double am = 0.5 * (r.a0 + r.a1), bm = 0.5 * (r.b0 + r.b1);
+  return sphere_clear(v, {r.a0, am, r.b0, bm}, depth + 1) && sphere_clear(v, {am, r.a1, r.b0, bm}, depth + 1) &&
+         sphere_clear(v, {r.a0, am, bm, r.b1}, depth + 1) && sphere_clear(v, {am, r.a1, bm, r.b1}, depth + 1);
+}
+
+}
+
+uint32_t void_packets(const VoidRequest &q, uint32_t *bits) {
+  memset(bits, 0, void_words(q.numTiles) * sizeof(uint32_t));
+  if (q.raygen != IRT_RAYGEN_WITH_ACCEL || q.accelMode != IRT_ACCEL_SPHERE || q.mode != IRT_MODE_USER_GEOM) return 0;
+  if (q.W <= 0 || q.H <= 0 || q.tileStride <= 0 || q.tileBegin < 0) return 0;
+  for (int k = 0; k < 12; ++k)
+    if (!std::isfinite(q.cam[k])) return 0;
+  for (int k = 0; k < 3; ++k)
+    if (!std::isfinite(q.bmin[k]) || !std::isfinite(q.bmax[k])) return 0;
+  const double R = q.rOuter, r = q.rInner;
+  if (!std::isfinite(R) || !std::isfinite(r) || !(r >= 0.0) || !(R >= r) || !(R > 0.0)) return 0;
+  const V3 org = {q.cam[0], q.cam[1], q.cam[2]}, d00 = {q.cam[3], q.cam[4], q.cam[5]},
+           du = {q.cam[6], q.cam[7], q.cam[8]}, dv = {q.cam[9], q.cam[10], q.cam[11]};
+  const double eps = ldexp(1.0, -19);
+  const double P = norm(org);
+  if (!(P > 1.001 * R) || !(eps * P * P <= 0.01 * R * R)) return 0;
+  const double need = asin(sqrt((R / P) * (R / P) + eps));
+  const V3 axis = (-1.0 / P) * org;
+  double T = 0.0;
+  for (int k = 0; k < 8; ++k) {
+    const V3 cnr = {(k & 1) ? q.bmax[0] : q.bmin[0], (k & 2) ? q.bmax[1] : q.bmin[1], (k & 4) ? q.bmax[2] : q.bmin[2]};
+    T = std::max(T, norm(cnr + (-1.0) * org));
+  }
+  if (!(T < 1e9)) return 0;
+  const View v = {org, d00, du, dv, axis, dot(du, du), dot(dv, dv), fabs(dot(du, dv)), abs1(d00), abs1(du), abs1(dv),
+                  cos(need), sin(need)};
+  const int tilesX = (q.W + 63) / 64, total = tilesX * ((q.H + 63) / 64);
+  uint32_t count = 0;
+  auto in_box = [&](double a0, double a1, double b0, double b1, double delta) {
+    const double s = T * (delta + 4e-7);
+    double blo[3], bhi[3];
+    for (int j = 0; j < 3; ++j) {
+      blo[j] = (double)q.bmin[j] + s;
+      bhi[j] = (double)q.bmax[j] - s;
+      if (!(blo[j] < bhi[j])) return false;
+    }
+    return hits_box(org, v.dir(a0, b0), blo, bhi) && hits_box(org, v.dir(a1, b0), blo, bhi) &&
+           hits_box(org, v.dir(a0, b1), blo, bhi) && hits_box(org, v.dir(a1, b1), blo, bhi);
+  };
+  for (int k = 0; k < q.numTiles; ++k) {
+    const int tileId = q.tileList ? q.tileList[k] : q.tileBegin + k * q.tileStride;
+    if (tileId < 0 || tileId >= total) continue;
+    const int tx0 = (tileId % tilesX) * 64, ty0 = (tileId / tilesX) * 64;
+    double delta = 0.0;
+    const Rect tile = {tx0 + 0.5, std::min(tx0 + 64, q.W) + 0.5, ty0 + 0.5, std::min(ty0 + 64, q.H) + 0.5};
+    const int whole = sphere_rect(v, tile, delta);
+    if (whole == kAllHit) continue;
+    const bool tileVoid = whole == kClear && in_box(tile.a0, tile.a1, tile.b0, tile.b1, delta);
+    for (int j = 0; j < 64; ++j) {
+      const size_t p = (size_t)k * 64 + j;
+      const int sub = j >> 2, wave = j & 3;
+      const int x0 = tx0 + (((sub & 3) << 4) | ((wave & 1) << 3)), y0 = ty0 + (((sub >> 2) << 4) | ((wave >> 1) << 3));
+      if (x0 >= q.W || y0 >= q.H) continue;
+      if (!tileVoid) {
+        const Rect r = {x0 + 0.5, std::min(x0 + 8, q.W) + 0.5, y0 + 0.5, std::min(y0 + 8, q.H) + 0.5};
+        double pd = 0.0;
+        if (sphere_rect(v, r, pd) < 0 || pd == 0.0) continue;
+        if (!sphere_clear(v, r, 0) || !in_box(r.a0, r.a1, r.b0, r.b1, pd)) continue;
+      }
+      bits[p >> 5] |= 1u << (p & 31);
+      ++count;
+    }
+  }
+  return count;
+}
+
+bool VoidCache::lookup(const VoidRequest &q, bool defer) {
+  std::vector<unsigned char> k(sizeof(VoidRequest) + (q.tileList ? (size_t)std::max(q.numTiles, 0) * sizeof(int32_t) : 0));
+  VoidRequest flat = q;
+  flat.tileList = q.tileList ? reinterpret_cast<const int32_t *>(1) : nullptr;
+  memcpy(k.data(), &flat, sizeof(flat));
+  if (q.tileList && q.numTiles > 0) memcpy(k.data() + sizeof(flat), q.tileList, (size_t)q.numTiles * sizeof(int32_t));
+  const bool same = keyed && k == key;
+  if (same && valid) return false;
+  if (!same) {
+    key.swap(k);
+    keyed = true;
+    valid = false;
+    count = 0;
+    if (defer) return false;
+  }
+  bits.assign(void_words(q.numTiles), 0u);
+  count = void_packets(q, bits.data());
+  valid = true;
+  ++generation;
+  return true;
+}
+
+}
diff --git a/icon-ray-tracing_amd/python/irt.py b/icon-ray-tracing_amd/python/irt.py
--- a/icon-ray-tracing_amd/python/irt.py
+++ b/icon-ray-tracing_amd/python/irt.py
@@ -212,6 +212,8 @@
         L.irt_debug_slot_use.argtypes = [C.c_void_p, C.c_void_p]
         if v in ((d & ~4096), (d | 262144) & ~4096, (d | 1073741824) & ~4096) and L.irt_debug_slot_use(ctx._h, None) == 1:
             v |= 128
+        elif ctx.void_use() > 0:
+            v |= 16
         return v
     return int(L.irt_debug_default_variant()) & ~4096
 
@@ -359,6 +361,48 @@
     _check(lib().irt_deal_tiles(C.byref(lp), C.byref(info), w, h, ranks, rank0_extra,
                                 _ptr(table), table.size, C.byref(m)), "irt_deal_tiles")
     return table
+
+
+class VoidCache:
+
+    def __init__(self):
+        L = lib()
+        L.irt_debug_void_cache_create.restype = C.c_void_p
+        L.irt_debug_void_cache_free.argtypes = [C.c_void_p]
+        L.irt_debug_void_cache_free.restype = None
+        self._h = C.c_void_p(L.irt_debug_void_cache_create())
+        self.computations = 0
+
+    def packets(self, lp, info, w, h, tile_begin=0, tile_stride=1, tiles=None):
+        out = void_packets(lp, info, w, h, tile_begin, tile_stride, tiles, cache=self)
+        return out
+
+    def __del__(self):
+        if getattr(self, "_h", None):
+            lib().irt_debug_void_cache_free(self._h)
+            self._h = None
+
+
+def void_packets(lp: LaunchParams, info: VolumeInfo, w: int, h: int, tile_begin: int = 0,
+                 tile_stride: int = 1, tiles=None, cache: VoidCache = None) -> np.ndarray:
+    L = lib()
+    L.irt_debug_void_packets.argtypes = [C.c_void_p, C.POINTER(LaunchParams), C.POINTER(VolumeInfo), C.c_int,
+                                         C.c_int, C.c_int, C.c_int, C.c_void_p, C.c_int, C.c_void_p,
+                                         C.c_size_t, C.POINTER(C.c_uint32), C.POINTER(C.c_longlong)]
+    total = num_tiles(w, h)
+    t = None if tiles is None else np.ascontiguousarray(tiles, dtype=np.int32)
+    nt = len(t) if t is not None else (max(0, (total - tile_begin + tile_stride - 1) // tile_stride)
+                                       if tile_begin < total else 0)
+    bits = np.zeros(max(2 * nt, 1), np.uint32)
+    n, comp = C.c_uint32(), C.c_longlong()
+    _check(L.irt_debug_void_packets(cache._h if cache else None, C.byref(lp), C.byref(info), w, h, tile_begin,
+                                    tile_stride, _ptr(t) if t is not None else None, nt if t is not None else 0,
+                                    _ptr(bits), bits.size, C.byref(n), C.byref(comp)), "irt_debug_void_packets")
+    if cache:
+        cache.computations = comp.value
+    out = ((bits[:2 * nt, None] >> np.arange(32, dtype=np.uint32)[None, :]) & 1).astype(bool).reshape(-1)
+    assert int(out.sum()) == n.value
+    return out
 
 
 @dataclass
@@ -543,6 +587,14 @@
         _check(L.irt_debug_sched_split(self._h, C.byref(n), C.byref(lg)), "irt_debug_sched_split")
         return n.value, lg.value
 
+    def void_use(self) -> int:
+        L = lib()
+        if not hasattr(L, "irt_debug_void_use"):
+            return 0
+        L.irt_debug_void_use.argtypes = [C.c_void_p]
+        L.irt_debug_void_use.restype = C.c_longlong
+        return L.irt_debug_void_use(self._h)
+
     def launch_workgroups(self, num_tiles: int, frames: int = 1) -> int:
         L = lib()
         L.irt_debug_launch_workgroups.argtypes = [C.c_void_p, C.c_int, C.c_int]
diff --git a/include/icon_rt_hip_debug.h b/include/icon_rt_hip_debug.h
--- a/include/icon_rt_hip_debug.h
+++ b/include/icon_rt_hip_debug.h
@@ -79,6 +79,13 @@
 int irt_debug_sched_order(const uint32_t *cost, int numBlocks, int tilesX, int tileStride, int policy,
                           int splitLg, float splitFactor, int numCU, int wavewg, size_t capacity,
                           uint32_t maxSplit, uint32_t *out, uint32_t *numSplit);
+typedef struct irt_debug_void_cache irt_debug_void_cache;
+irt_debug_void_cache *irt_debug_void_cache_create(void);
+void irt_debug_void_cache_free(irt_debug_void_cache *cache);
+int irt_debug_void_packets(irt_debug_void_cache *cache, const irt_launch_params *lp, const irt_volume_info *info,
+                           int W, int H, int tileBegin, int tileStride, const int32_t *tileList, int listCount,
+                           uint32_t *bits, size_t capacity, uint32_t *numVoid, long long *computations);
+long long irt_debug_void_use(const irt_context *ctx);
 int irt_debug_set_chain(irt_context *ctx, int on);
 int irt_debug_chain_errors(irt_context *ctx);
 int irt_debug_set_chain_fault(irt_context *ctx, uint32_t spins, int withholdFrame);
diff --git a/profiles/void_share.py b/profiles/void_share.py
--- /dev/null
+++ b/profiles/void_share.py
@@ -0,0 +1,106 @@
+#!/usr/bin/env python3
+import argparse
+import json
+import os
+import sys
+
+ROOT = os.path.dirname(os.path.dirname(os.path.abspath(__file__)))
+sys.path[:0] = [os.path.join(ROOT, "icon-ray-tracing_amd", "python"), ROOT]
+
+import numpy as np
+import torch
+
+import bench
+import irt
+
+
+def void_packets_f64(cam12, W, H, radius):
+    c = np.asarray(cam12, dtype=np.float64)
+    org, d00, du, dv = c[0:3], c[3:6], c[6:9], c[9:12]
+    tx, ty = (W + 63) // 64, (H + 63) // 64
+    p = np.arange(tx * ty * 64)
+    blk, wave = p >> 2, p & 3
+    k, sub = blk >> 4, blk & 15
+    x0 = (k % tx) * 64 + ((sub & 3) << 4) + ((wave & 1) << 3)
+    y0 = (k // tx) * 64 + ((sub >> 2) << 4) + ((wave >> 1) << 3)
+    x1 = np.minimum(x0 + 8, W)
+    y1 = np.minimum(y0 + 8, H)
+    active = (x0 < W) & (y0 < H)
+
+    def unit(a, b):
+        d = d00[None, :] + a[:, None] * du[None, :] + b[:, None] * dv[None, :]
+        return d / np.linalg.norm(d, axis=1, keepdims=True)
+
+    alo, ahi, blo, bhi = x0 + .5, x1 + .5, y0 + .5, y1 + .5
+    cen = unit((alo + ahi) / 2, (blo + bhi) / 2)
+    ext = np.zeros(len(p))
+    for a, b in ((alo, blo), (ahi, blo), (alo, bhi), (ahi, bhi)):
+        ext = np.maximum(ext, np.arccos(np.clip((cen * unit(a, b)).sum(1), -1, 1)))
+    dist = np.linalg.norm(org)
+    if dist <= radius:
+        return np.zeros(len(p), dtype=bool)
+    to_centre = np.arccos(np.clip((cen * (-org / dist)[None, :]).sum(1), -1, 1))
+    return active & (to_centre - ext > np.arcsin(radius / dist))
+
+
+def main():
+    ap = argparse.ArgumentParser()
+    ap.add_argument("--config", default="c3")
+    ap.add_argument("--launches", type=int, default=3)
+    ap.add_argument("--warmup", type=int, default=5)
+    ap.add_argument("--batch", type=int, default=8)
+    args = ap.parse_args()
+    rn, bis, L, W, H, tf, orbit_cfg, desc = bench.CONFIGS[args.config]
+    assert not orbit_cfg, "progressive configs only"
+    dev = torch.device("cuda:0")
+    ctx = irt.Context.synth(rn, bis, L, 0, terrain=bench.TERRAIN.get(args.config, 0.0))
+    setup = irt.setup_frame(None, W, H, camera=bench.FRAMING, info=ctx.info)
+    ctx.set_transfunc(bench.make_lut(tf, setup.lut), setup.value_range)
+    ctx.set_statistics(False)
+    lp = setup.lp
+    fb = torch.zeros(W * H, dtype=torch.int32, device=dev)
+    accum = torch.zeros(W * H * 4, dtype=torch.float32, device=dev)
+    stream = torch.cuda.current_stream(0).cuda_stream
+    ctx.clear(fb.data_ptr(), accum.data_ptr(), W * H, stream)
+    B = args.batch
+
+    def step(s):
+        lp.accumID = s * B
+        ctx.render_accumulate(lp, W, H, B, fb.data_ptr(), accum.data_ptr(), stream)
+
+    for s in range(args.warmup):
+        step(s)
+    nt = irt.num_tiles(W, H)
+    nwg = ctx.launch_workgroups(nt, B)
+    assert nwg == nt * 64 * B, "one-wave workgroups, no split items"
+    bufs = [torch.zeros(nwg * 4, dtype=torch.int32, device=dev) for _ in range(args.launches)]
+    torch.cuda.synchronize()
+    for k in range(args.launches):
+        ctx.set_wg_trace(bufs[k].data_ptr())
+        step(args.warmup + k)
+    ctx.set_wg_trace(0)
+    torch.cuda.synchronize()
+    void = void_packets_f64(lp.camera12(), W, H, ctx.info.sphericalBounds.upper.x)
+    bx = np.arange(nt * 64)
+    pkt = ((((bx >> 5) << 3) | (bx & 7)) << 2) | ((bx >> 3) & 3)
+    wg_void = np.tile(void[pkt], B)
+    frame = np.repeat(np.arange(B), nt * 64)
+    for k in range(args.launches):
+        tr = bufs[k].cpu().numpy().view(np.uint32).reshape(-1, 4)
+        dur = ((tr[:, 1].astype(np.int64) - tr[:, 0].astype(np.int64)) & 0xFFFFFFFF) / 100.0
+        span = ((tr[:, 1].astype(np.int64) - tr[:, 0].astype(np.int64).min()) & 0xFFFFFFFF).max() / 100.0
+        out = {"config": args.config, "launch": k, "frames_per_launch": B, "workgroups": int(nwg),
+               "void_packets_per_frame": int(void.sum()), "packets_per_frame": int(nt * 64),
+               "void_packet_share": round(float(void.mean()), 4),
+               "void_lifetime_share": round(float(dur[wg_void].sum() / dur.sum()), 4),
+               "void_lifetime_share_frames_after_first": round(float(dur[wg_void & (frame > 0)].sum() / dur.sum()), 4),
+               "wg_us_mean_void_first_frame": round(float(dur[wg_void & (frame == 0)].mean()), 3) if void.any() else None,
+               "wg_us_mean_void_later_frames": round(float(dur[wg_void & (frame > 0)].mean()), 3) if void.any() else None,
+               "wg_us_mean_other": round(float(dur[~wg_void].mean()), 3),
+               "span_us": float(span)}
+        print(json.dumps(out), flush=True)
+    ctx.close()
+
+
+if __name__ == "__main__":
+    main()
```

Result: faster. 17990 Mray/s, median of 6 (+4.6%).
